# vaenyr/stable-diffusion-on-device

Measured on AMD Instinct MI355X. Metric: images/sec + per-UNet-step ms, SD v1.4 512x512 20-step PLMS, 1/2/4/8 MI355X, higher is better.
Workload: dtype f16; 1 GPU; SD v1.4 txt2img 512x512, 20-step PLMS (21 UNet evals, batch 2 = cond+uncond per image), CLIP encode + VAE decode + uint8, guidance 7.5; images_per_gpu=1, global_batch=1, parallelism=dp1 (image shards, 1 RCCL broadcast), hip_graph=True, trajectory_graph=True, decode_overlaps_next_sampling=False

## Files before the change

include/sdod_engine.h:

```cpp
#ifndef SDOD_ENGINE_H
#define SDOD_ENGINE_H

#include <stddef.h>
#include <stdint.h>

#ifndef SDOD_API
#define SDOD_API
#endif

#ifdef __cplusplus
extern "C" {
#endif

enum sdod_graph_kind { SDOD_GRAPH_UNET = 0, SDOD_GRAPH_VAE_DECODER = 1, SDOD_GRAPH_TEXT_ENCODER = 2, SDOD_GRAPH_TEMB = 3,
                       SDOD_GRAPH_VAE_ENCODER = 4, SDOD_GRAPH_VAE_ENCODER_MASKED = 5, SDOD_GRAPH_ADAPTER = 6, SDOD_GRAPH_UPSCALER = 7,
                       SDOD_GRAPH_CONTROLNET = 8, SDOD_GRAPH_CONTROL_HINT = 9, SDOD_GRAPH_IMAGE_ENCODER = 10, SDOD_GRAPH_IMAGE_PROJ = 11 };

typedef struct sdod_model_config {
    int latent_channels;
    int latent_h;
    int latent_w;
    int model_channels;
    int context_dim;
    int context_len;
    int num_heads;
    int head_dim;
    int vocab_size;
    int text_layers;
    int text_heads;
    int vae_channels;
    int linear_proj;
    int text_arch;
    int weight_quant;
    int concat_channels;
} sdod_model_config;

SDOD_API void sdod_model_config_sd14(sdod_model_config* cfg);
SDOD_API void sdod_model_config_sd21(sdod_model_config* cfg);

SDOD_API int sdod_graph_create(void** graph, int kind, const sdod_model_config* cfg, int batch);
typedef struct sdod_adapter_config {
    int adapter_reps;
    int adapter_hint_channels;
    int adapter_res_blocks;
} sdod_adapter_config;
SDOD_API int sdod_graph_create_ex(void** graph, int kind, const sdod_model_config* cfg, const sdod_adapter_config* adapter, int batch);
SDOD_API int sdod_graph_create_wrap(void** graph, int kind, const sdod_model_config* cfg, const sdod_adapter_config* adapter, int wrap,
                                    int batch);
typedef struct sdod_upscaler_config {
    int num_blocks;
    int in_h;
    int in_w;
} sdod_upscaler_config;
SDOD_API int sdod_graph_create_upscaler(void** graph, const sdod_upscaler_config* cfg, int batch);
typedef struct sdod_control_config {
    int control_inputs;
    int control_temb;
} sdod_control_config;
SDOD_API int sdod_graph_create_control(void** graph, int kind, const sdod_model_config* cfg, const sdod_control_config* control, int batch);
typedef struct sdod_region_config {
    int regions;
} sdod_region_config;
SDOD_API int sdod_graph_create_regions(void** graph, int kind, const sdod_model_config* cfg, const sdod_region_config* regions, int batch);
typedef struct sdod_ip_config {
    int ip_tokens;
} sdod_ip_config;
SDOD_API int sdod_graph_create_ip(void** graph, int kind, const sdod_model_config* cfg, const sdod_ip_config* ip, int batch);
typedef struct sdod_vision_config {
    int image_size;
    int patch;
    int width;
    int layers;
    int heads;
    int mlp_dim;
    int proj_dim;
    int quick_gelu;
} sdod_vision_config;
SDOD_API int sdod_graph_create_vision(void** graph, int kind, const sdod_model_config* cfg, const sdod_vision_config* vision, const sdod_ip_config* ip,
                                      int batch);
SDOD_API int sdod_graph_bind_output(void* graph, int index, void* device_ptr, size_t bytes);
SDOD_API int sdod_graph_destroy(void* graph);

SDOD_API int sdod_graph_num_params(void* graph);
SDOD_API int sdod_graph_param_info(void* graph, int index, const char** name, int* ndim, int64_t shape[4]);
SDOD_API int sdod_graph_set_param(void* graph, const char* name, const void* data, int dtype, const int64_t* shape, int ndim);
SDOD_API int sdod_graph_param_device(void* graph, const char* name, void** device_ptr, size_t* bytes);
SDOD_API int sdod_graph_load_file(void* graph, const char* path, const char* prefix);
SDOD_API int sdod_graph_finalize(void* graph);
SDOD_API int sdod_graph_io(void* graph, int is_output, int index, void** device_ptr, size_t* bytes);
enum sdod_exec_flags { SDOD_EXEC_HIP_GRAPH = 1, SDOD_EXEC_STATIC_UNCHANGED = 2 };
SDOD_API int sdod_graph_execute(void* graph, void* stream, int flags);
SDOD_API int sdod_graph_check(void* graph);
SDOD_API int sdod_graph_num_ops(void* graph);
SDOD_API int sdod_graph_op_info(void* graph, int index, const char** label, double* flops, double* bytes);
SDOD_API int sdod_graph_op_detail(void* graph, int index, const char** detail);
SDOD_API int sdod_graph_profile(void* graph, void* stream, int iters, float* ms_out, int n);
SDOD_API int sdod_graph_stats(void* graph, size_t* weight_bytes, size_t* arena_bytes, int* num_launches, double* flops);
SDOD_API int sdod_graph_tune_info(void* graph, int* from_table, int* tuned_in_process, char* table_path, int cap);

SDOD_API int sdod_graph_keep_base(void* graph);
SDOD_API int sdod_graph_base_bytes(void* graph, size_t* bytes);
typedef struct {
    const char* name;
    const void* up;
    const void* down;
    int dtype;
    int rank;
    float scale;
} sdod_lora_entry;
SDOD_API int sdod_graph_set_loras(void* graph, const sdod_lora_entry* entries, int count, void* stream);

SDOD_API int sdod_graph_enable_freeu(void* graph);
SDOD_API int sdod_graph_freeu_input(void* graph, int* index);

#ifdef __cplusplus
}
#endif
#endif
```

include/sdod_hip.h:

```cpp
#ifndef SDOD_HIP_H
#define SDOD_HIP_H

#include <stddef.h>
#include <stdint.h>

#ifndef SDOD_API
#define SDOD_API
#endif

#ifdef __cplusplus
extern "C" {
#endif

enum sdod_act { SDOD_ACT_NONE = 0, SDOD_ACT_SILU = 1, SDOD_ACT_GELU = 2, SDOD_ACT_QUICK_GELU = 3, SDOD_ACT_RELU = 4 };
enum sdod_dtype { SDOD_F16 = 0, SDOD_F32 = 1, SDOD_U8Q = 2, SDOD_BF16 = 3  };
enum sdod_a_mode { SDOD_A_ROWS = 0, SDOD_A_CONV3X3 = 1  };

typedef struct sdod_gemm_desc {
    const void* a;
    const void* a2;
    const void* w;
    const void* bias;
    const void* row_bias;
    const void* residual;
// ... 19 lines not shown
    const void* t0;
    const void* t1;
    int tc0, tc1;
    const void* bias2;
    int ln;
    const void* ln_s;
    float ln_eps;
    int phase;
    int wq;
    const void* w_scale;
    const void* w_off;
    void* fix_counters;
    int xcd_panels;
    int w_img_stride;
    int vec_img_stride;
    int softmax_cols;
    int pad_mode;
} sdod_gemm_desc;

SDOD_API int sdod_gemm_f16(const sdod_gemm_desc* d, void* stream);
SDOD_API int sdod_gemm_region_f16(const sdod_gemm_desc* d, const void* region_w, int regions, void* stream);
SDOD_API int sdod_gemm_fixup(const sdod_gemm_desc* d);
SDOD_API size_t sdod_gemm_fixup_counters(void);
SDOD_API size_t sdod_gemm_workspace_bytes(const sdod_gemm_desc* d);
SDOD_API int sdod_gemm_plan(const sdod_gemm_desc* d, int* tile, int* splits);
SDOD_API int sdod_gemm_halo_ok(const sdod_gemm_desc* d, int tile);
SDOD_API int sdod_gemm_panel_ok(const sdod_gemm_desc* d, int tile);
SDOD_API int sdod_gemm_xcd_panels(const sdod_gemm_desc* d);
SDOD_API int sdod_gemm_num_tiles(void);
SDOD_API int sdod_gemm_tile_shape(int tile, int* bm, int* bn, int* lds_dma);
SDOD_API int sdod_gemm_tile_info(int tile, int out[7]);
SDOD_API int sdod_gemm_time(const sdod_gemm_desc* d, void* stream, int iters, float* ms_avg);
SDOD_API int sdod_gemm_time_cold(const sdod_gemm_desc* d, void* stream, int iters, void* scratch, size_t scratch_bytes, float* ms_avg,
                                float* ms_min );

SDOD_API size_t sdod_group_norm_workspace_bytes(int n, int groups);
SDOD_API int sdod_group_norm_layout(int n, int groups, size_t* sync_off, size_t* partial_off, size_t* stats_off, size_t* shift_off,
                                    size_t* end_off);
SDOD_API int sdod_group_norm_status(void);
SDOD_API int sdod_group_norm_clear_error(void);
SDOD_API int sdod_group_norm_launches(int hw, int c, int groups, int dtype);
SDOD_API int sdod_group_norm_path(int n, int hw, int c0, int c1, int groups, int dtype);
SDOD_API int sdod_group_norm_nhwc(const void* x, const void* x2, void* y, const float* weight, const float* bias,
                                  int n, int hw, int c0, int c1, int groups, float eps, int silu, int dtype,
                                  void* workspace, void* stream);

SDOD_API size_t sdod_group_norm_nchw_workspace_bytes(int n, int groups);
SDOD_API int sdod_group_norm_nchw(const void* x, void* y, const float* weight, const float* bias, int n, int c, long long spatial,
                                  int groups, float eps, int silu, int dtype, void* workspace, void* stream);

typedef struct sdod_gn_reduce {
    const void* partial;
    int splits;
    size_t slab_floats;
    const void* bias;
    const void* bias2;
    const void* row_bias;
    int ld_row_bias;
    const void* residual;
    int ldr;
    void* x_out;
    float alpha;
    int act;
    int M, N;
} sdod_gn_reduce;
SDOD_API int sdod_gemm_reduce_info(const sdod_gemm_desc* d, sdod_gn_reduce* out);
SDOD_API int sdod_group_norm_reduce_ok(int hw, int c0, int c1, int groups);
SDOD_API int sdod_group_norm_reduce_nhwc(const sdod_gn_reduce* red, const void* x2, void* y, const float* weight,
                                         const float* bias, int n, int hw, int c0, int c1, int groups, float eps, int silu,
                                         void* stream);

SDOD_API int sdod_ln_fold_f16(void* w, int n, int k, int ldw, const float* gamma, const float* beta, const float* bias_in,
                              float* s_out, float* t_out, void* stream);
SDOD_API int sdod_compose_linear_f16(const void* p, int ldp, const void* w, int ldw, void* c, int ldc, int n_out, int n_mid, int k,
                                     const float* bias_w, const float* bias_p, float* bias_out, void* stream);
SDOD_API int sdod_lora_merge_f16(void* w, int n, int k, int ldw, const void* up, const void* down, int rank, float scale,
                                 int conv_cin, int geglu, void* stream);
SDOD_API int sdod_layer_norm_f16(const void* x, void* y, const float* weight, const float* bias, int m, int c,
                                 float eps, void* stream);

SDOD_API int sdod_attention_f16(const void* q, const void* k, const void* v, void* out, int batch, int heads,
                                int lq, int lk, int d, int ldq, int ldk, int ldv, int ldo, float scale, int causal,
                                void* stream);
SDOD_API int sdod_attention_head_dim_ok(int d);

SDOD_API int sdod_xattn_fold_f16(const void* kv, int ld_kv, int k_off, int v_off, int n_img, int L, const void* wq, int ldq,
                                 const void* sq, const void* tq, const void* wo, int ldwo, int heads, int d, float scale, void* w1,
                                 void* s1, void* t1, void* w2, void* stream);
SDOD_API int sdod_xattn_fold_ok(int heads, int d, int l_keys, int rows_per_image);

SDOD_API int sdod_xattn_fold_regions_f16(const void* kv, int ld_kv, int k_off, int v_off, int n_img, int regions, int L, const void* wq,
                                         int ldq, const void* sq, const void* tq, const void* wo, int ldwo, int heads, int d, float scale,
                                         void* w1, void* s1, void* t1, void* w2, void* stream);

SDOD_API int sdod_xattn_fold_ip_f16(const void* kv, int ld_kv, int k_off, int v_off, const void* kv_ip, int ld_ip, int k_off_ip, int v_off_ip,
                                    int n_img, int L, int T, const void* wq, int ldq, const void* sq, const void* tq, const void* wo, int ldwo,
                                    int heads, int d, float scale, void* w1, void* s1, void* t1, void* w2, void* stream);

SDOD_API int sdod_softmax_rows_f16(const void* x, void* y, int m, int n, void* stream);

SDOD_API int sdod_geglu_f16(const void* x, void* y, int m, int c, void* stream);
SDOD_API int sdod_act_f16(const void* x, void* y, size_t n, int act, void* stream);
SDOD_API int sdod_add_f16(const void* a, const void* b, void* y, size_t n, void* stream);
SDOD_API int sdod_region_weights_f32(const uint8_t* masks, int regions, int h, int w, float* w1, float* w2, float* w4, float* w8, void* stream);
SDOD_API int sdod_region_blend_f16(const void* a, size_t region_stride, const float* w, void* out, int rows, int rows_per_img, int c, int regions,
                                   void* stream);
SDOD_API int sdod_ip_weights_f32(const uint8_t* mask, float scale, int h, int w, float* w1, float* w2, float* w4, float* w8, void* stream);
SDOD_API int sdod_patch_embed_u8_f16(const uint8_t* img, void* out, int n, int image_size, int patch, int kpad, const float* mean3, const float* std3,
                                     void* stream);
SDOD_API int sdod_vit_tokens_f16(const void* patches, const void* class_embedding, const void* position_embedding, const float* ln_weight,
                                 const float* ln_bias, void* out, int n, int num_patches, int width, float eps, void* stream);
SDOD_API int sdod_concat_channels_f16(const void* a, const void* b, void* y, size_t rows, int c0, int c1, void* stream);
SDOD_API int sdod_pixel_unshuffle_u8_f16(const uint8_t* img, void* y, int n, int h, int w, int ch, int factor, void* stream);
SDOD_API int sdod_avg_pool2_f16(const void* x, void* y, int n, int h, int w, int c, void* stream);
SDOD_API int sdod_adapter_stage_f16(const void* src, void* dst, size_t count, float weight, void* stream);
SDOD_API int sdod_add_feature_f16(void* h, const void* f, size_t per_copy, int reps, void* stream);
#define SDOD_CONTROL_MAX_SEGS 16
typedef struct sdod_control_seg {
    void* h;
    const void* r;
    size_t count;
} sdod_control_seg;
SDOD_API int sdod_add_control_f16(const sdod_control_seg* segs, int count, const float* scales, void* stream);
#define SDOD_FREEU_PARAMS 8
SDOD_API int sdod_freeu_f16(void* h, void* skip, int n, int height, int width, int c, const float* params, int stage, float* scratch,
                            int phases, void* stream);
SDOD_API int sdod_im2col3x3_small_f16(const void* x, void* y, int n_img, int h, int w, int c, int kpad, void* stream);
SDOD_API int sdod_im2col3x3_small_wrap_f16(const void* x, void* y, int n_img, int h, int w, int c, int kpad, int wrap, void* stream);
SDOD_API int sdod_latent_im2col_f16(const float* x, void* y, int n_img, int h, int w, int c, int kpad, float scale, void* stream);

SDOD_API int sdod_conv_in_f16(const float* x, const void* w, const float* bias, void* y, int n_img, int h, int wd, int c, int cout,
                              float scale, void* stream);
SDOD_API int sdod_conv_in_wrap_f16(const float* x, const void* w, const float* bias, void* y, int n_img, int h, int wd, int c, int cout,
                                   float scale, int wrap, void* stream);
SDOD_API int sdod_image_conv_in_f16(const uint8_t* img, const void* w, const float* bias, void* y, int n_img, int h, int wd, int cout,
                                    void* stream);
SDOD_API int sdod_conv_in_cat_f16(const float* x, const float* cond, const void* w, const float* bias, void* y, int n_img, int h, int wd,
                                  int c, int c_cond, int cout, void* stream);
SDOD_API int sdod_masked_image_conv_in_f16(const uint8_t* img, const uint8_t* mask, const void* w, const float* bias, void* y, int n_img,
                                           int h, int wd, int cout, void* stream);
SDOD_API int sdod_image_conv_in_unit_f16(const uint8_t* img, const void* w, const float* bias, void* y, void* y2, int ld2, int n_img, int h,
                                         int wd, int cout, void* stream);

typedef struct sdod_dense_conv_desc {
    const void* in;
    const void* w;
    const float* bias;
    void* out;
    const void* res1;
    const void* res2;
    int ld_in, ld_out, ld_res1, ld_res2;
    int out_col;
    int cin, cout;
    int n, h, w_in;
    int upsample;
    float alpha, slope, c1;
} sdod_dense_conv_desc;
SDOD_API int sdod_dense_conv3x3_f16(const sdod_dense_conv_desc* d, void* stream);
SDOD_API int sdod_dense_conv3x3_ok(const sdod_dense_conv_desc* d);

SDOD_API int sdod_inpaint_cond_f32(const float* moments, const uint8_t* mask_u8, const float* n1, float* cond, int n, int c, int h_lat,
                                   int w_lat, int factor, int reps, uint64_t seed, uint64_t image_index0, void* stream);
SDOD_API int sdod_encode_latent_f32(const float* moments, const float* n1, const float* n2, float* x, float* z0, int n, int c, int hw,
                                    float sqrt_at, float sqrt_one_minus_at, uint64_t seed, uint64_t image_index0, void* stream);
SDOD_API int sdod_latent_resize_f32(const float* src, float* dst, int n, int c, int h_in, int w_in, int h_out, int w_out, int mode, float a,
                                    float b, const float* noise, uint64_t seed, uint64_t image_index0, void* stream);
// ... 110 lines not shown
```

stable-diffusion-on-device_amd/csrc/attention.hip:

```cpp
#include "common.h"
#include "sdod_hip.h"
#include "host_util.h"

#include <climits>
#include <cmath>
#include <cstdlib>
#include <type_traits>

namespace {

struct AttnP {
    const f16* q;
    const f16* k;
    const f16* v;
    f16* out;
    int B, H, Lq, Lk;
    int ldq, ldk, ldv, ldo;
    float scale_log2;
    int causal;
};

typedef short short4v __attribute__((__vector_size__(4 * sizeof(short))));
typedef __attribute__((address_space(3))) short4v* lds_short4_ptr;

constexpr int odd16(int dv) {
    int s = (dv + 15) / 16;
    if ((s & 1) == 0) s += 1;
    return s * 16;
}

template <int D, int QT>
constexpr int attn_min_waves() { return (D == 40 || (D == 80 && QT == 1)) ? 3 : 1; }

template <int N, int I = 0, class F>
SDOD_DEVICE void static_for(F&& f) {
    if constexpr (I < N) {
        f(std::integral_constant<int, I>{});
        static_for<N, I + 1>(f);
    }
}

template <int D, int QT, bool TR, int KVS = 1>
__global__ __launch_bounds__(256 * KVS, (attn_min_waves<D, QT>())) void attn_kernel(const AttnP p) {
    constexpr int DP = ((D + 31) / 32) * 32;
    constexpr int KSTEPS = DP / 32;
    constexpr int DV = ((D + 15) / 16) * 16;
    constexpr int NDT = DV / 16;
    constexpr int KSTR = DP + 8;
    constexpr int VSTR = odd16(DV);
    constexpr int KT = 64;
    constexpr int DC = D / 8;
    constexpr int LD_IT = (KT * DC + 255) / 256;
    constexpr int STAGE = KT * (KSTR + VSTR);
    constexpr bool SUM_BY_MFMA = DV > D;
    constexpr bool DEFER = DP > D;
    constexpr int KS_M = D / 32, G_M = (D % 32) / 8;
    constexpr float THR = 8.0f;
    static_assert(D % 8 == 0, "head dim must be a multiple of 8");

    extern __shared__ __attribute__((aligned(16))) char smem_raw[];
    const int grp = KVS > 1 ? (int)(threadIdx.x >> 8) : 0;
    f16* smem = reinterpret_cast<f16*>(smem_raw) + (size_t)grp * 2 * STAGE;

    const int tid = threadIdx.x & 255;
    const int lane = tid & 63;
    const int wave = tid >> 6;
    const int g = lane >> 4;
    const int li = lane & 15;
    const int nqb = (p.Lq + 64 * QT - 1) / (64 * QT);
    const int lid = xcd_remap(blockIdx.x, nqb * p.H * p.B);
    const int bh = lid / nqb;
    const int b = bh / p.H, h = bh - b * p.H;
    const int q_block = (lid - bh * nqb) * (64 * QT);

    const f16* kbase = p.k + (size_t)b * p.Lk * p.ldk + h * D;
    const f16* vbase = p.v + (size_t)b * p.Lk * p.ldv + h * D;

    {
        constexpr int KPADC = (DP - D) / 8, VPADC = (DV - D) / 8;
        for (int st = 0; st < 2; ++st) {
            f16* sK = smem + st * STAGE;
            f16* sV = sK + KT * KSTR;
            if (KPADC > 0)
                for (int idx = tid; idx < KT * KPADC; idx += 256) {
                    const int row = idx / (KPADC > 0 ? KPADC : 1), ch = idx - row * KPADC;
                    f16x8 pad = zero8();
                    if (DEFER && ch == 0) pad[0] = (f16)-1.0f;
                    *reinterpret_cast<f16x8*>(sK + row * KSTR + D + ch * 8) = pad;
                }
            if (VPADC > 0)
                for (int idx = tid; idx < KT * VPADC; idx += 256) {
                    const int row = idx / (VPADC > 0 ? VPADC : 1), ch = idx - row * VPADC;
                    f16x8 pad = zero8();
                    if (ch == 0) pad[0] = (f16)1.0f;
                    *reinterpret_cast<f16x8*>(sV + row * VSTR + D + ch * 8) = pad;
                }
        }
    }

    f16x8 qf[QT][KSTEPS];
    int qrow[QT];
#pragma unroll
// ... 236 lines not shown
    };

    if (grp < NT) {
        load_tile(grp);
        store_tile(0);
    }
    __syncthreads();
    const int NTG = (NT + KVS - 1) / KVS;
    int thr = INT_MIN;
    for (int it = 0; it < NTG; ++it) {
        const int t = it * KVS + grp;
        const int cur = it & 1;
        const bool has_next = t + KVS < NT;
        const f16* sK = smem + cur * STAGE;
        const f16* sV = sK + KT * KSTR;
        if (t >= NT) {
            __syncthreads();
            continue;
        }
        f16x8 kf[HOLD ? KSTEPS : 1][4];
        f16x8 vfr[HOLD ? 2 : 1][HOLD ? NDT : 1];
        read_k(sK, kf);
        read_v(sV, vfr);
        f32x4 s[QT][4];
        qk(sK, kf, s);
        if (has_next && !(abl & 1)) load_tile(t + KVS);
        static_for<QT>([&](auto a_c) { softmax_pv(a_c, t, thr, s[decltype(a_c)::value], vfr, sV); });
        thr = __builtin_bit_cast(int, THR);
        asm volatile("" : "+s"(thr));
        if (has_next) store_tile(cur ^ 1);
        __syncthreads();
    }

    if constexpr (KVS > 1) {
        static_assert(KVS == 2, "the merge below handles two groups");
        float* mrg = reinterpret_cast<float*>(smem_raw);
        constexpr int NV = QT * (2 + NDT * 4);
        static_assert((size_t)NV * 256 * sizeof(float) <= (size_t)KVS * 2 * STAGE * sizeof(f16), "merge buffer fits the staging LDS");
        if (grp == 1) {
#pragma unroll
            for (int a = 0; a < QT; ++a) {
                mrg[(a * (2 + NDT * 4) + 0) * 256 + tid] = m_run[a];
                mrg[(a * (2 + NDT * 4) + 1) * 256 + tid] = l_run[a];
#pragma unroll
                for (int dt = 0; dt < NDT; ++dt)
#pragma unroll
                    for (int r = 0; r < 4; ++r) mrg[(a * (2 + NDT * 4) + 2 + dt * 4 + r) * 256 + tid] = o[a][dt][r];
            }
        }
        __syncthreads();
        if (grp == 1) return;
#pragma unroll
        for (int a = 0; a < QT; ++a) {
            const float m1 = mrg[(a * (2 + NDT * 4) + 0) * 256 + tid], l1 = mrg[(a * (2 + NDT * 4) + 1) * 256 + tid];
            const float m = fmaxf(m_run[a], m1);
            const float a0 = __builtin_amdgcn_exp2f(m_run[a] - m), a1 = __builtin_amdgcn_exp2f(m1 - m);
            l_run[a] = l_run[a] * a0 + l1 * a1;
#pragma unroll
            for (int dt = 0; dt < NDT; ++dt)
#pragma unroll
                for (int r = 0; r < 4; ++r) o[a][dt][r] = o[a][dt][r] * a0 + mrg[(a * (2 + NDT * 4) + 2 + dt * 4 + r) * 256 + tid] * a1;
            m_run[a] = m;
        }
    }
#pragma unroll
    for (int a = 0; a < QT; ++a) {
        float l;
        if (SUM_BY_MFMA) {
            l = __shfl(o[a][D / 16][D % 4], ((D % 16) / 4) * 16 + li);
        } else {
            l = quad_rows_sum(l_run[a]);
        }
        const float inv = l > 0.f ? 1.0f / l : 0.f;
        if (qrow[a] < p.Lq) {
            f16* op = p.out + ((size_t)b * p.Lq + qrow[a]) * p.ldo + h * D;
#pragma unroll
            for (int dt = 0; dt < NDT; ++dt) {
                const int dv0 = dt * 16 + g * 4;
                if (dv0 < D) {
                    f16x4 hv;
#pragma unroll
                    for (int r = 0; r < 4; ++r) hv[r] = (f16)(o[a][dt][r] * inv);
                    *reinterpret_cast<f16x4*>(op + dv0) = hv;
                }
            }
        }
    }
}

template <int D, int QT, bool TR, int KVS = 1>
hipError_t attn_launch(const AttnP& p, hipStream_t st) {
    constexpr int DP = ((D + 31) / 32) * 32;
    constexpr int DV = ((D + 15) / 16) * 16;
    constexpr size_t smem = (size_t)KVS * 2 * 64 * (DP + 8 + odd16(DV)) * sizeof(f16);
    static_assert(smem <= 160 * 1024, "LDS");
    static std::atomic<unsigned long long> attr_devs{0};
    if (sdod::first_use_on_device(attr_devs)) {
        hipError_t e = hipFuncSetAttribute(reinterpret_cast<const void*>(&attn_kernel<D, QT, TR, KVS>),
                                           hipFuncAttributeMaxDynamicSharedMemorySize, (int)smem);
        if (e != hipSuccess) return e;
    }
    dim3 grid(((p.Lq + 64 * QT - 1) / (64 * QT)) * p.H * p.B);
    SDOD_LAUNCH((attn_kernel<D, QT, TR, KVS>), grid, dim3(256 * KVS), smem, st, p);
    return hipGetLastError();
}

template <int D>
hipError_t attn_dispatch(const AttnP& p, bool big, bool tr, hipStream_t st) {
    if (tr) return big ? attn_launch<D, 2, true>(p, st) : attn_launch<D, 1, true>(p, st);
    return big ? attn_launch<D, 2, false>(p, st) : attn_launch<D, 1, false>(p, st);
}

struct FoldP {
    const f16* kv; int ld_kv, k_off, v_off, L, n_img;
    const f16* wq; int ldq;
    const float* sq; const float* tq;
    const f16* wo; int ldwo;
    int heads, d, C;
    float alpha;
    f16* w1; float* s1; float* t1; f16* w2;
    int tiles_c;
    int n_w;
    int regions;
    const f16* kv2; int ld_kv2, k_off2, v_off2, L2;
};
constexpr int kFoldKMax = 160;
struct FoldSeg { const f16* k; const f16* v; int ld, L; };
template <bool TWO_SRC>
__device__ __forceinline__ FoldSeg fold_segment(const FoldP& p, int seg) {
    if constexpr (!TWO_SRC) {
        const f16* base = p.kv + (long long)seg * p.L * p.ld_kv;
        return FoldSeg{base + p.k_off, base + p.v_off, p.ld_kv, p.L};
    }
    const int b = seg >> 1;
    if (seg & 1) {
        const f16* base = p.kv2 + (long long)b * p.L2 * p.ld_kv2;
        return FoldSeg{base + p.k_off2, base + p.v_off2, p.ld_kv2, p.L2};
    }
    const f16* base = p.kv + (long long)b * p.L * p.ld_kv;
    return FoldSeg{base + p.k_off, base + p.v_off, p.ld_kv, p.L};
}
template <bool TWO_SRC>
__global__ __launch_bounds__(256) void xattn_fold_kernel(const FoldP p) {
    __shared__ __attribute__((aligned(16))) f16 sa[80][kFoldKMax + 8], sb[80][kFoldKMax + 8];
    const int tid = threadIdx.x, lane = tid & 63, wave = tid >> 6;
    const int NK = p.heads * 80, d = p.d;
    int item = blockIdx.x;
    if (item >= 2 * p.n_w) {
        const int idx = (item - 2 * p.n_w) * 256 + tid;
        if (idx >= p.n_img * NK) return;
        const int j = idx % 80, bh = idx / 80, h = bh % p.heads, img = bh / p.heads;
        const FoldSeg sg = fold_segment<TWO_SRC>(p, img);
        if (j >= sg.L) {
            p.s1[idx] = 0.f;
            p.t1[idx] = -30000.f;
            return;
        }
        const f16* kr = sg.k + (long long)j * sg.ld + h * d;
        float a = 0.f, b = 0.f;
        for (int dd = 0; dd < d; ++dd) {
            const float kval = (float)kr[dd];
            a = fmaf(kval, p.sq[h * d + dd], a);
            b = fmaf(kval, p.tq[h * d + dd], b);
        }
        p.s1[idx] = p.alpha * a;
        p.t1[idx] = p.alpha * b;
        return;
    }
    const bool second = item >= p.n_w;
    if (second) item -= p.n_w;
    const int tc = item % p.tiles_c, bh = item / p.tiles_c, h = bh % p.heads, img = bh / p.heads;
    const int KP = (d + 31) & ~31, kc = KP / 8;
    const FoldSeg sg = fold_segment<TWO_SRC>(p, img);
    auto stage_rows = [&](f16 (*dst)[kFoldKMax + 8], const f16* base, long long row_stride, int valid_rows) {
        for (int idx = tid; idx < 80 * kc; idx += 256) {
            const int r = idx / kc, ch = idx - r * kc;
            const f16x8 v = (r < valid_rows && ch * 8 < d) ? ldg8(base + (long long)r * row_stride + ch * 8) : zero8();
            *reinterpret_cast<f16x8*>(&dst[r][ch * 8]) = v;
        }
    };
    if (!second) {
        stage_rows(sa, sg.k + h * d, sg.ld, sg.L);
        for (int idx = tid; idx < KP * 10; idx += 256) {
            const int k = idx / 10, ch = idx - k * 10;
            const f16x8 v = k < d ? ldg8(p.wq + (long long)(h * d + k) * p.ldq + tc * 80 + ch * 8) : zero8();
#pragma unroll
            for (int e = 0; e < 8; ++e) sb[ch * 8 + e][k] = v[e];
        }
    } else {
        stage_rows(sa, p.wo + (long long)(tc * 80) * p.ldwo + h * d, p.ldwo, 80);
        stage_rows(sb, sg.v + h * d, sg.ld, sg.L);
    }
    __syncthreads();
    const int fr = lane & 15, fg = lane >> 4;
    for (int rb = wave; rb < 5; rb += 4) {
        f32x4 acc[5];
#pragma unroll
        for (int j = 0; j < 5; ++j) acc[j] = f32x4{0.f, 0.f, 0.f, 0.f};
        for (int ks = 0; ks < KP / 32; ++ks) {
            const f16x8 fa = *reinterpret_cast<const f16x8*>(&sa[rb * 16 + fr][ks * 32 + fg * 8]);
#pragma unroll
            for (int j = 0; j < 5; ++j) {
                const f16x8 fb = *reinterpret_cast<const f16x8*>(&sb[j * 16 + fr][ks * 32 + fg * 8]);
                acc[j] = mfma16(fb, fa, acc[j]);
            }
        }
        const int m = rb * 16 + fr;
        const int wimg = img / p.regions, reg = img - wimg * p.regions;
        f16* row = second ? p.w2 + ((long long)wimg * p.C + tc * 80 + m) * ((long long)p.regions * NK) + reg * NK + h * 80
                          : p.w1 + ((long long)(img * p.heads + h) * 80 + m) * p.C + tc * 80;
        const float al = second ? 1.0f : p.alpha;
#pragma unroll
        for (int j = 0; j < 5; ++j) {
            f16x4 o;
#pragma unroll
            for (int r = 0; r < 4; ++r) o[r] = (f16)(al * acc[j][r]);
            *reinterpret_cast<f16x4*>(row + j * 16 + fg * 4) = o;
        }
    }
}

}

extern "C" int sdod_attention_head_dim_ok(int d) { return d == 40 || d == 64 || d == 80 || d == 160 ? 1 : 0; }

extern "C" int sdod_xattn_fold_ok(int heads, int d, int l_keys, int rows_per_image) {
    if (heads <= 0 || d <= 0 || d > kFoldKMax || d % 8 != 0 || l_keys <= 0 || l_keys > 80) return 0;
    const long long C = (long long)heads * d, NK = (long long)heads * 80;
    if (C % 80 != 0) return 0;
    if (rows_per_image == 0) return 1;
    return rows_per_image > 0 && rows_per_image % 32 == 0 && NK % 320 == 0 && C % 64 == 0 ? 1 : 0;
}

extern "C" int sdod_attention_f16(const void* q, const void* k, const void* v, void* out, int batch, int heads, int lq,
                                  int lk, int d, int ldq, int ldk, int ldv, int ldo, float scale, int causal,
                                  void* stream) {
    SDOD_TRY
    SDOD_REQUIRE(q && k && v && out, "null pointer");
    SDOD_REQUIRE(batch > 0 && heads > 0 && lq > 0 && lk > 0, "bad shape");
    SDOD_REQUIRE(sdod_attention_head_dim_ok(d), "head dim must be one of 40, 64, 80, 160");
    SDOD_REQUIRE(ldq % 8 == 0 && ldk % 8 == 0 && ldv % 8 == 0 && ldo % 4 == 0, "row strides must keep 16-byte alignment");
    SDOD_REQUIRE(ldq >= heads * d && ldk >= heads * d && ldv >= heads * d && ldo >= heads * d, "row stride < heads*d");
    SDOD_REQUIRE((((uintptr_t)q | (uintptr_t)k | (uintptr_t)v) & 15) == 0 && ((uintptr_t)out & 7) == 0, "misaligned pointer");
    SDOD_REQUIRE(std::isfinite(scale) && scale > 0.f, "scale must be finite and > 0");
    AttnP p{};
    p.q = (const f16*)q; p.k = (const f16*)k; p.v = (const f16*)v; p.out = (f16*)out;
    p.B = batch; p.H = heads; p.Lq = lq; p.Lk = lk;
    p.ldq = ldq; p.ldk = ldk; p.ldv = ldv; p.ldo = ldo;
    p.scale_log2 = scale * 1.4426950408889634f;
    p.causal = causal;
    const bool no_tr = std::getenv("SDOD_ATTN_NO_TR") != nullptr;
    const bool tr = !no_tr;
    bool big = lq >= 2048 && d != 160;
    if (const char* e = std::getenv("SDOD_ATTN_QT")) big = e[0] == '2' && d != 160;
    hipStream_t st = (hipStream_t)stream;
    hipError_t e;
    switch (d) {
    case 40: e = attn_dispatch<40>(p, big, tr, st); break;
    case 64: e = attn_dispatch<64>(p, big, tr, st); break;
    case 80: {
        static const bool kvs_off = [] { const char* e2 = std::getenv("SDOD_ATTN_KVS"); return e2 && e2[0] == '0'; }();
        const long long wgs = (long long)((lq + 63) / 64) * heads * batch;
        if (!big && tr && !kvs_off && !causal && wgs <= 512 && lk >= 256) e = attn_launch<80, 1, true, 2>(p, st);
        else e = attn_dispatch<80>(p, big, tr, st);
        break;
    }
    default: e = attn_dispatch<160>(p, false, tr, st); break;
    }
    SDOD_HIP_CHECK(e);
    return 0;
    SDOD_CATCH
}

namespace {
struct FoldSrc2 { const void* kv; int ld, k_off, v_off, L; };
int xattn_fold_launch(const void* kv, int ld_kv, int k_off, int v_off, int n_img, int regions, int L, const void* wq, int ldq, const void* sq,
                      const void* tq, const void* wo, int ldwo, int heads, int d, float scale, void* w1, void* s1, void* t1, void* w2,
                      void* stream, const FoldSrc2& ip = FoldSrc2{nullptr, 0, 0, 0, 0}) {
    SDOD_TRY
    SDOD_REQUIRE(regions >= 1 && regions <= 4, "regions must be in [1, 4]");
    if (ip.kv) {
        SDOD_REQUIRE(regions == 2, "two sources are two segments per image");
        SDOD_REQUIRE(ip.L >= 1 && ip.L <= 16, "image tokens must be in [1, 16]");
        SDOD_REQUIRE(ip.ld % 8 == 0 && ip.k_off % 8 == 0 && ip.v_off % 8 == 0 && ip.k_off >= 0 && ip.v_off >= 0 && ((uintptr_t)ip.kv & 15) == 0,
                     "operands must keep 16-byte alignment");
        SDOD_REQUIRE(heads > 0 && d > 0 && (long long)ip.k_off + (long long)heads * d <= ip.ld && (long long)ip.v_off + (long long)heads * d <= ip.ld,
                     "image K / V offsets + heads * d must fit the image row stride");
    }
    SDOD_REQUIRE(n_img <= (1 << 20), "bad shape (too many images)");
    n_img *= regions;
    SDOD_REQUIRE(kv && wq && sq && tq && wo && w1 && s1 && t1 && w2, "null pointer");
    SDOD_REQUIRE(n_img > 0 && sdod_xattn_fold_ok(heads, d, L, 0), "bad shape (d <= 160, d % 8 == 0, L <= 80, heads * d a multiple of 80)");
    SDOD_REQUIRE((long long)heads * d <= (1 << 24), "bad shape (heads * d too large)");
    const int C = heads * d, NK = heads * 80;
    SDOD_REQUIRE(ldq >= C && ldwo >= C && ld_kv >= C, "row strides >= heads * d");
    SDOD_REQUIRE(ld_kv % 8 == 0 && k_off % 8 == 0 && v_off % 8 == 0 && ldq % 8 == 0 && ldwo % 8 == 0 &&
                     (((uintptr_t)kv | (uintptr_t)wq | (uintptr_t)wo | (uintptr_t)w1 | (uintptr_t)w2) & 15) == 0,
                 "operands must keep 16-byte alignment");
    FoldP p{};
    p.kv = (const f16*)kv; p.ld_kv = ld_kv; p.k_off = k_off; p.v_off = v_off; p.L = L; p.n_img = n_img;
    p.wq = (const f16*)wq; p.ldq = ldq; p.sq = (const float*)sq; p.tq = (const float*)tq;
    p.wo = (const f16*)wo; p.ldwo = ldwo;
    p.heads = heads; p.d = d; p.C = C;
    p.alpha = scale * 1.4426950408889634f;
    p.w1 = (f16*)w1; p.s1 = (float*)s1; p.t1 = (float*)t1; p.w2 = (f16*)w2;
    p.tiles_c = C / 80;
    p.n_w = n_img * heads * p.tiles_c;
    p.regions = regions;
    p.kv2 = (const f16*)ip.kv; p.ld_kv2 = ip.ld; p.k_off2 = ip.k_off; p.v_off2 = ip.v_off; p.L2 = ip.L;
    const int blocks = 2 * p.n_w + (n_img * NK + 255) / 256;
    if (ip.kv) SDOD_LAUNCH(xattn_fold_kernel<true>, dim3(blocks), dim3(256), 0, (hipStream_t)stream, p);
    else SDOD_LAUNCH(xattn_fold_kernel<false>, dim3(blocks), dim3(256), 0, (hipStream_t)stream, p);
    SDOD_HIP_CHECK(hipGetLastError());
    return 0;
    SDOD_CATCH
}
}

extern "C" int sdod_xattn_fold_f16(const void* kv, int ld_kv, int k_off, int v_off, int n_img, int L, const void* wq, int ldq,
                                   const void* sq, const void* tq, const void* wo, int ldwo, int heads, int d, float scale, void* w1,
                                   void* s1, void* t1, void* w2, void* stream) {
    return xattn_fold_launch(kv, ld_kv, k_off, v_off, n_img, 1, L, wq, ldq, sq, tq, wo, ldwo, heads, d, scale, w1, s1, t1, w2, stream);
}

extern "C" int sdod_xattn_fold_regions_f16(const void* kv, int ld_kv, int k_off, int v_off, int n_img, int regions, int L, const void* wq,
                                           int ldq, const void* sq, const void* tq, const void* wo, int ldwo, int heads, int d, float scale,
                                           void* w1, void* s1, void* t1, void* w2, void* stream) {
    return xattn_fold_launch(kv, ld_kv, k_off, v_off, n_img, regions, L, wq, ldq, sq, tq, wo, ldwo, heads, d, scale, w1, s1, t1, w2, stream);
}

extern "C" int sdod_xattn_fold_ip_f16(const void* kv, int ld_kv, int k_off, int v_off, const void* kv_ip, int ld_ip, int k_off_ip, int v_off_ip,
                                      int n_img, int L, int T, const void* wq, int ldq, const void* sq, const void* tq, const void* wo, int ldwo,
                                      int heads, int d, float scale, void* w1, void* s1, void* t1, void* w2, void* stream) {
    SDOD_TRY
    SDOD_REQUIRE(kv_ip, "null pointer");
    SDOD_CATCH
    return xattn_fold_launch(kv, ld_kv, k_off, v_off, n_img, 2, L, wq, ldq, sq, tq, wo, ldwo, heads, d, scale, w1, s1, t1, w2, stream,
                             FoldSrc2{kv_ip, ld_ip, k_off_ip, v_off_ip, T});
}
```

stable-diffusion-on-device_amd/csrc/engine.h:

```cpp
#pragma once
#include <hip/hip_runtime.h>

#include <cstdint>
#include <functional>
#include <map>
#include <string>
#include <unordered_map>
#include <vector>

#include "host_util.h"
#include "sdod_engine.h"
#include "sdod_hip.h"

namespace sdod {

typedef _Float16 f16;

inline void check_rc(int rc) {
    if (rc != 0) throw Error(rc, get_last_error());
}

enum ParamKind {
    PK_CONV3,
    PK_CONV3_SMALL,
    PK_CONV1,
    PK_LINEAR,
    PK_EMBED,
    PK_VEC,
    PK_MAT_F32,
    PK_LINEAR_GEGLU,
    PK_VEC_GEGLU,
};

inline int small_k(int64_t cin) { return 9 * cin <= 64 ? 64 : 128; }

struct Param {
    std::string name;
    std::vector<int64_t> shape;
    ParamKind kind;
    int group = -1;
    int ld = 0;
    int col_off = 0;
    int owner = -1;
    size_t dev_bytes = 0;
    char* dev = nullptr;
    bool set = false;
    bool quant = false;
    size_t qrow = 0;
};

struct Act {
    f16* p = nullptr;
    int n = 0, h = 0, w = 0, c = 0;
    int rows() const { return n * h * w; }
    size_t numel() const { return (size_t)rows() * c; }
};

struct IoSlot {
    void* ptr = nullptr;
    size_t bytes = 0;
    bool owned = true;
};

class Graph {
public:
    Graph(int kind, const sdod_model_config& cfg, int batch, const sdod_adapter_config& acfg = sdod_adapter_config{0, 0, 0}, int wrap = 0,
          const sdod_upscaler_config& ucfg = sdod_upscaler_config{0, 0, 0}, const sdod_control_config* ccfg = nullptr, int regions = 0,
          int ip_tokens = 0, const sdod_vision_config* vcfg = nullptr);
    ~Graph();
    Graph(const Graph&) = delete;

    int num_params() const { return (int)params_.size(); }
    const Param& param(int i) const { return params_.at(i); }
    void set_param(const std::string& name, const void* data, int dtype, const int64_t* shape, int ndim);
    void load_file(const std::string& path, const std::string& prefix);
    void finalize();
    void keep_base();
    size_t base_bytes() const { return base_copy_ ? weight_bytes_ : 0; }
    void set_loras(const sdod_lora_entry* entries, int count, hipStream_t st);
    void enable_freeu();
    int freeu_input() const { return freeu_ ? freeu_input_ : -1; }
    void execute(hipStream_t st, bool use_hip_graph, bool skip_static = false);
    void check_health() const;
    IoSlot io(bool output, int index) const;
    void bind_output(int index, void* ptr, size_t bytes);
    void stats(size_t* wbytes, size_t* abytes, int* launches, double* flops) const;

private:
    enum Mode { DECLARE, DRY, REAL };
    int kind_;
    sdod_model_config cfg_;
    sdod_adapter_config acfg_;
    sdod_upscaler_config ucfg_;
    sdod_control_config ccfg_{0, 0};
    int regions_ = 0;
    const float* region_w_[4] = {};
    sdod_vision_config vcfg_{0, 0, 0, 0, 0, 0, 0, 0};
    int ip_tokens_ = 0;
    const float* ip_w_[4] = {};
    f16* ip_kv_all_ = nullptr;
    bool freeu_ = false;
    int freeu_input_ = -1;
    void freeu_site(const Act& h, const Act& skip, const float* params, int stage);
    bool has_kv() const { return kind_ == SDOD_GRAPH_UNET || kind_ == SDOD_GRAPH_CONTROLNET; }
    int batch_;
    int wrap_ = 0;
    Mode mode_ = DECLARE;
    bool finalized_ = false;

    std::vector<Param> params_;
    std::unordered_map<std::string, int> pindex_;
    std::vector<std::vector<int>> groups_;
    std::unordered_map<std::string, int> gindex_;
    char* weight_base_ = nullptr;
    size_t weight_bytes_ = 0;
    float* qscale_ = nullptr;
    float* qoff_ = nullptr;
    size_t qrows_ = 0;
    bool quant_mode() const { return cfg_.weight_quant != 0 && (kind_ == SDOD_GRAPH_UNET || kind_ == SDOD_GRAPH_TEMB); }
    static constexpr int kQuantAutoMaxRows = 128;
    bool quant_decl_ = false;
    void quant_rows(int rows) { quant_decl_ = quant_mode() && (cfg_.weight_quant == 1 || rows <= kQuantAutoMaxRows); }
    void quant_global() { quant_decl_ = quant_mode(); }
    const float* qscale_of(int w) const { return params_[w].quant ? qscale_ + params_[w].qrow : nullptr; }
    const float* qoff_of(int w) const { return params_[w].quant ? qoff_ + params_[w].qrow : nullptr; }
    int P(const std::string& name, std::vector<int64_t> shape, ParamKind kind, const std::string& group = "");
    int Pc(const std::string& name, std::vector<int64_t> shape, ParamKind kind, int ld, int col_off, int owner);
    template <typename T>
    const T* W(int idx) const { return reinterpret_cast<const T*>(params_[idx].dev); }
    void allocate_weights();

    char* arena_base_ = nullptr;
    size_t arena_cap_ = 0, arena_high_ = 0;
    std::map<size_t, size_t> free_;
    std::map<size_t, size_t> used_;
    void arena_reset();
    f16* alloc(size_t halves);
    void release(const void* p);
    Act act(int n, int h, int w, int c);
    void release(const Act& a) { release(a.p); }

    char* ws_ = nullptr;
    size_t ws_bytes_ = 0, ws_need_ = 0;
    char* gn_ws_ = nullptr;
    size_t gn_ws_bytes_ = 0, gn_ws_need_ = 0;

    std::vector<IoSlot> inputs_, outputs_;
    void* io_alloc(std::vector<IoSlot>& v, size_t bytes);
    std::vector<size_t> out_bytes_;
    std::map<int, void*> bound_out_;

    struct Op {
        std::function<void(hipStream_t)> fn;
        std::string label;
        double flops = 0;
        double bytes = 0;
        std::string detail;
        const void* pf_ptr = nullptr;
        size_t pf_bytes = 0;
    };
    std::vector<Op> ops_;
    std::vector<Op> static_ops_;
    bool to_static_ = false;
    double flops_ = 0;
    hipGraphExec_t graph_exec_ = nullptr;
    hipGraph_t hip_graph_ = nullptr;
    hipStream_t capture_stream_ = nullptr;
    unsigned* fix_counters_ = nullptr;
    hipStream_t side_stream_ = nullptr;
    std::vector<hipEvent_t> pf_events_;
    void run_ops(hipStream_t st);
    int eager_runs_ = 0;
    int tune_hits_ = 0, tune_misses_ = 0;

    void build();
    void build_unet();
    void build_vae();
    void build_vae_encoder(bool masked);
    void build_clip();
    Act clip_block(const std::string& pfx, bool oc, Act x, int heads, int inter, bool causal, int mlp_act);
    void build_image_encoder();
    void build_image_proj();
    void build_temb();
    void build_adapter();
    void build_upscaler();
    void build_controlnet();
    void build_control_hint();

    struct GemmOpt {
        int bias = -1;
        const float* bias_raw = nullptr;
        f16* out = nullptr;
        const f16* row_bias = nullptr;
        int ld_row_bias = 0, rows_per_img = 0;
        const f16* residual = nullptr;
        int act = 0;
        float alpha = 1.0f;
        bool bias_on_m = false;
        int lda = 0, ldo = 0;
        int ldr = 0;
        bool geglu = false;
        const Act* tail0 = nullptr;
        const Act* tail1 = nullptr;
        int bias2 = -1;
        int ln_w = -1, ln_b = -1;
        const float* wq_scale = nullptr;
        const float* wq_off = nullptr;
        const float* ln_s_raw = nullptr;
        int w_img_stride = 0, vec_img_stride = 0;
        int softmax_cols = 0;
        const float* region_w = nullptr;
        int regions = 0;
        int pad_mode = 0;
        int split_k = 0;
    };
    struct LnVecs { float* s; float* t; };
    LnVecs ln_fold_vectors(f16* w, int N, int K, int ldw, int ln_w, int ln_b, const float* bias);
    struct FoldJob {
        f16* w; int n, k, ldw;
        const float *gamma, *beta, *bias_in;
        float *s, *t;
    };
    std::vector<FoldJob> fold_jobs_;
    struct ComposeJob {
        f16* c; const f16* p; int ld, n_out, n_mid, k;
        const float *bias_w, *bias_p;
        float* bias_out;
    };
    std::vector<ComposeJob> compose_jobs_;
    void run_folds(hipStream_t st);
    bool keep_base_ = false;
    char* base_copy_ = nullptr;
    bool static_stale_ = false;
    std::vector<void*> derived_;
    void emit_gemm(sdod_gemm_desc d, const float* region_w = nullptr, int regions = 0);
    void linear(const f16* x, int rows, int K, int w, int N, f16* out, const GemmOpt& o);
    void linear_raw(const f16* x, int rows, int K, const f16* w, int ldw, int N, f16* out, const GemmOpt& o);
    Act conv(const Act& x, const Act* x2, int w, int cout, int ksize, int stride, bool upsample, const GemmOpt& o);
    Act group_norm(const Act& x, const Act* x2, int gw, int gb, float eps, bool silu);
    Act layer_norm(const Act& x, int lw, int lb, float eps);
    void dense_conv(sdod_dense_conv_desc d, int w, int bias);
    void attention(const f16* q, const f16* k, const f16* v, f16* out, int B, int heads, int lq, int lk, int d, int ldq,
                   int ldk, int ldv, int ldo, bool causal);

    Act res_block(const std::string& pfx, const Act& x, const Act* x2, int cout, const f16* emb_all, int emb_ld, int& emb_off);
    std::vector<Op>& sink() { return to_static_ ? static_ops_ : ops_; }
    struct PendingReduce {
        bool active = false;
        sdod_gemm_desc d{};
        double bytes = 0;
        std::string detail;
    } pending_;
    void flush_pending();
    std::vector<const void*> parked_;
    void release_after_consumer(const Act& a) { parked_.push_back(a.p); }
    void drain_parked() {
        for (const void* p : parked_) release(p);
        parked_.clear();
    }
    void settle() {
        flush_pending();
        drain_parked();
    }
    struct HeadGeom { int heads, d; };
    HeadGeom head_geometry(int C) const;
    void check_head_geometry() const;
    Act spatial_transformer(const std::string& pfx, const Act& x, const Act& ctx);
    Act unet_conv_in(const float* x_in, const float* cond_in);
    Act unet_encoder(Act h, const Act& ctx, const f16* emb_all, int emb_ld, int& emb_off, const f16* const* feat_in, std::vector<Act>* hs,
                     const std::function<void(int, const Act&)>& on_skip);
    size_t control_residual_numel(int k) const;
    void kv_all_gemm(const f16* ctx_in);
    void ip_kv_all_gemm(const f16* ip_ctx_in);
    std::vector<std::pair<std::string, int>> temb_blocks() const;
    Act vae_res_block(const std::string& pfx, const Act& x, int cout);
    Act vae_attn_block(const std::string& pfx, const Act& x);
    void vae_res_step(const std::string& pfx, Act& h, int cout);
    void vae_mid(const std::string& pfx, Act& h, int ch);
    int emb_total_ = 0;
    int kv_total_ = 0;
    f16* kv_all_ = nullptr;
    int kv_off_ = 0;
    std::vector<std::pair<std::string, int>> unet_res_blocks() const;
    const char* group_base(const std::string& group) const;
    int group_first(const std::string& group) const;
    void emit(std::function<void(hipStream_t)> fn, std::string label = "elementwise", double flops = 0, double bytes = 0, std::string detail = "") {
        settle();
        if (mode_ != REAL) return;
        flops_ += flops;
        sink().push_back(Op{std::move(fn), std::move(label), flops, bytes, std::move(detail)});
    }

public:
    int tune_hits() const { return tune_hits_; }
    int tune_misses() const { return tune_misses_; }
    int num_ops() const { return (int)ops_.size(); }
    const Op& op(int i) const { return ops_.at(i); }
    void profile(hipStream_t st, int iters, float* ms, int n);
};

}
```

stable-diffusion-on-device_amd/csrc/engine.hip:

```cpp
#include "engine.h"

#include <cstdio>

#include <dlfcn.h>
#include <fcntl.h>
#include <sys/mman.h>
#include <sys/stat.h>
#include <unistd.h>

#include <algorithm>
#include <cstdlib>
#include <cstring>
#include <map>
#include <mutex>
#include <thread>

namespace sdod {

static inline size_t align_up(size_t v, size_t a) { return (v + a - 1) / a * a; }

template <typename F>
static void parallel_for(int64_t n, F&& fn) {
    int nt = (int)std::min<int64_t>(n, std::max(1u, std::min(16u, std::thread::hardware_concurrency())));
    if (nt <= 1) {
        fn(0, n);
        return;
    }
    std::vector<std::thread> th;
    const int64_t per = (n + nt - 1) / nt;
    for (int t = 0; t < nt; ++t) {
        const int64_t b = t * per, e = std::min(n, b + per);
        if (b < e) th.emplace_back([=, &fn]() { fn(b, e); });
    }
    for (auto& t : th) t.join();
}

Graph::Graph(int kind, const sdod_model_config& cfg, int batch, const sdod_adapter_config& acfg, int wrap, const sdod_upscaler_config& ucfg,
             const sdod_control_config* ccfg, int regions, int ip_tokens, const sdod_vision_config* vcfg)
    : kind_(kind), cfg_(cfg), acfg_(acfg), ucfg_(ucfg), regions_(regions), ip_tokens_(ip_tokens), batch_(batch), wrap_(wrap) {
    SDOD_REQUIRE(ip_tokens == 0 || ((kind == SDOD_GRAPH_UNET || kind == SDOD_GRAPH_IMAGE_PROJ) && ip_tokens >= 1 && ip_tokens <= 16 && regions == 0),
                 "ip_tokens: the UNET and IMAGE_PROJ graphs only, 1 .. 16, not with regions");
    const bool vision_kind = kind == SDOD_GRAPH_IMAGE_ENCODER || kind == SDOD_GRAPH_IMAGE_PROJ;
    SDOD_REQUIRE(vision_kind == (vcfg != nullptr), "the IMAGE_ENCODER and IMAGE_PROJ graphs, and only they, are created by sdod_graph_create_vision");
    if (vcfg) {
        vcfg_ = *vcfg;
        cfg_.weight_quant = 0;
        SDOD_REQUIRE(vcfg_.proj_dim >= 64 && vcfg_.proj_dim <= 4096 && vcfg_.proj_dim % 64 == 0, "proj_dim must be a multiple of 64 in [64, 4096]");
        if (kind == SDOD_GRAPH_IMAGE_ENCODER) {
            SDOD_REQUIRE(vcfg_.patch >= 1 && vcfg_.patch <= 64 && vcfg_.image_size >= vcfg_.patch && vcfg_.image_size <= 1024 && vcfg_.image_size % vcfg_.patch == 0,
                         "image_size must be a multiple of patch (patch <= 64, image_size <= 1024)");
            SDOD_REQUIRE(vcfg_.width >= 64 && vcfg_.width <= 3072 && vcfg_.width % 64 == 0 && vcfg_.mlp_dim >= 64 && vcfg_.mlp_dim % 64 == 0 && vcfg_.mlp_dim <= 16384,
                         "width and mlp_dim must be multiples of 64 (width <= 3072, mlp_dim <= 16384)");
            SDOD_REQUIRE(vcfg_.layers >= 1 && vcfg_.layers <= 64 && vcfg_.heads >= 1 && vcfg_.width % vcfg_.heads == 0 &&
                             (vcfg_.width / vcfg_.heads == 64 || vcfg_.width / vcfg_.heads == 80),
                         "layers in [1, 64]; the head dim width / heads must be 64 or 80");
            SDOD_REQUIRE(vcfg_.quick_gelu == 0 || vcfg_.quick_gelu == 1, "quick_gelu must be 0 or 1");
        } else {
            SDOD_REQUIRE(ip_tokens >= 1, "the IMAGE_PROJ graph needs ip_tokens");
        }
    }
    SDOD_REQUIRE(regions == 0 || (kind == SDOD_GRAPH_UNET && regions >= 2 && regions <= 4), "regions: the UNET graph only, 2 .. 4");
    SDOD_REQUIRE(kind >= SDOD_GRAPH_UNET && kind <= SDOD_GRAPH_IMAGE_PROJ, "unknown graph kind");
    const bool control_kind = kind == SDOD_GRAPH_CONTROLNET || kind == SDOD_GRAPH_CONTROL_HINT;
    SDOD_REQUIRE(!control_kind || ccfg, "the CONTROLNET and CONTROL_HINT graphs are created by sdod_graph_create_control");
    if (ccfg) {
        ccfg_ = *ccfg;
        SDOD_REQUIRE((ccfg_.control_inputs == 0 || ccfg_.control_inputs == 1) && (ccfg_.control_temb == 0 || ccfg_.control_temb == 1),
                     "control_inputs and control_temb must be 0 or 1");
        SDOD_REQUIRE(ccfg_.control_inputs == 0 || kind == SDOD_GRAPH_UNET, "control_inputs applies to the UNET graph only");
        SDOD_REQUIRE(ccfg_.control_temb == 0 || kind == SDOD_GRAPH_TEMB, "control_temb applies to the TEMB graph only");
        if (control_kind || ccfg_.control_temb) {
            SDOD_REQUIRE(cfg.concat_channels == 0 && cfg.weight_quant == 0, "a control graph takes no concat_channels and no weight_quant");
            SDOD_REQUIRE(kind != SDOD_GRAPH_CONTROLNET || batch % 2 == 0, "the CONTROLNET graph needs an even batch (the two guidance halves)");
        }
    }
    if (kind == SDOD_GRAPH_UPSCALER) {
        SDOD_REQUIRE(ucfg.num_blocks != 0 || ucfg.in_h != 0 || ucfg.in_w != 0, "the UPSCALER graph is created by sdod_graph_create_upscaler");
        SDOD_REQUIRE(ucfg.num_blocks >= 1 && ucfg.num_blocks <= 23, "num_blocks must be in [1, 23]");
        SDOD_REQUIRE(ucfg.in_h >= 8 && ucfg.in_h <= 1024 && ucfg.in_h % 8 == 0 && ucfg.in_w >= 8 && ucfg.in_w <= 1024 && ucfg.in_w % 8 == 0,
                     "in_h and in_w must be multiples of 8 in [8, 1024]");
        cfg_.weight_quant = 0;
    } else {
        SDOD_REQUIRE(ucfg.num_blocks == 0 && ucfg.in_h == 0 && ucfg.in_w == 0, "an upscaler configuration needs kind SDOD_GRAPH_UPSCALER");
    }
    SDOD_REQUIRE(batch > 0 && batch <= 64, "batch must be in [1, 64]");
    SDOD_REQUIRE(cfg.model_channels > 0 && cfg.model_channels % 64 == 0, "model_channels must be a multiple of 64");
    SDOD_REQUIRE(cfg.context_dim % 64 == 0, "context_dim must be a multiple of 64");
    if (kind == SDOD_GRAPH_UNET || kind == SDOD_GRAPH_CONTROLNET) check_head_geometry();
    SDOD_REQUIRE(cfg.context_len >= 1 && cfg.context_len <= 4096, "context_len must be in [1, 4096]");
    SDOD_REQUIRE(cfg.concat_channels >= 0, "concat_channels must not be negative");
    SDOD_REQUIRE(acfg.adapter_reps >= 0 && acfg.adapter_reps <= 2, "adapter_reps must be 0, 1 or 2");
    SDOD_REQUIRE(wrap >= 0 && wrap <= 3, "wrap must be 0 .. 3 (bit 0 = x, bit 1 = y)");
    if (wrap != 0)
        SDOD_REQUIRE((kind == SDOD_GRAPH_UNET || kind == SDOD_GRAPH_VAE_DECODER) && cfg.concat_channels == 0,
                     "wrap applies to the UNET (without concat_channels) and VAE_DECODER graphs only");
    if (kind == SDOD_GRAPH_UNET && acfg.adapter_reps > 0)
        SDOD_REQUIRE(batch % acfg.adapter_reps == 0, "adapter_reps must divide the batch");
    if (kind == SDOD_GRAPH_ADAPTER) {
        SDOD_REQUIRE(acfg.adapter_hint_channels == 1 || acfg.adapter_hint_channels == 3, "adapter_hint_channels must be 1 or 3");
        SDOD_REQUIRE(acfg.adapter_res_blocks >= 0 && acfg.adapter_res_blocks <= 8, "adapter_res_blocks must be in [1, 8] (0 = 2)");
        cfg_.weight_quant = 0;
    }
    mode_ = DECLARE;
    arena_reset();
    build();
}

Graph::~Graph() {
    if (graph_exec_) (void)hipGraphExecDestroy(graph_exec_);
    if (capture_stream_) (void)hipStreamDestroy(capture_stream_);
    if (side_stream_) (void)hipStreamDestroy(side_stream_);
    (void)hipFree(fix_counters_);
    for (hipEvent_t e : pf_events_) (void)hipEventDestroy(e);
    if (hip_graph_) (void)hipGraphDestroy(hip_graph_);
    for (auto& s : inputs_) (void)hipFree(s.ptr);
    for (auto& s : outputs_)
        if (s.owned) (void)hipFree(s.ptr);
    (void)hipFree(weight_base_);
    (void)hipFree(base_copy_);
    (void)hipFree(qscale_);
    (void)hipFree(qoff_);
    (void)hipFree(arena_base_);
    (void)hipFree(ws_);
    (void)hipFree(gn_ws_);
    (void)hipFree(kv_all_);
    (void)hipFree(ip_kv_all_);
    for (void* d : derived_) (void)hipFree(d);
}

static size_t param_dev_bytes(const Param& p) {
    const auto& s = p.shape;
    if (p.quant) return (size_t)s[0] * s[1] * (p.kind == PK_CONV3 ? 9 : 1);
    switch (p.kind) {
    case PK_CONV3: return (size_t)s[0] * s[1] * 9 * sizeof(f16);
    case PK_CONV3_SMALL: return (size_t)s[0] * small_k(s[1]) * sizeof(f16);
    case PK_CONV1:
    case PK_LINEAR:
    case PK_LINEAR_GEGLU:
    case PK_EMBED: return (size_t)s[0] * s[1] * sizeof(f16);
    case PK_VEC:
    case PK_VEC_GEGLU: return (size_t)s[0] * sizeof(float);
    case PK_MAT_F32: {
        size_t n = 1;
        for (auto d : s) n *= (size_t)d;
        return n * sizeof(float);
    }
    }
    return 0;
}

int Graph::P(const std::string& name, std::vector<int64_t> shape, ParamKind kind, const std::string& group) {
    if (mode_ != DECLARE) {
        auto it = pindex_.find(name);
        if (it == pindex_.end()) throw Error(INTERNAL_ERROR, "parameter not declared: " + name);
        return it->second;
    }
    if (pindex_.count(name)) throw Error(INTERNAL_ERROR, "duplicate parameter: " + name);
    Param p;
    p.name = name;
    p.shape = std::move(shape);
    p.kind = kind;
    p.quant = quant_decl_ && (kind == PK_CONV3 || kind == PK_CONV1 || kind == PK_LINEAR || kind == PK_LINEAR_GEGLU);
    p.dev_bytes = param_dev_bytes(p);
    if (!group.empty()) {
        auto it = gindex_.find(group);
        if (it == gindex_.end()) {
            gindex_[group] = (int)groups_.size();
            groups_.emplace_back();
            it = gindex_.find(group);
        }
        p.group = it->second;
// ... 432 lines not shown
            for (int i = 0; i < ShapeKey::kFields; ++i) k.v[i] = (int)val[i];
            v = (int)val[ShapeKey::kFields];
        } else if (n == 13) {
            for (int i = 0; i < 12; ++i) k.v[i] = (int)val[i];
            k.v[12] = k.v[13] = 0;
            if (k.v[0] == SDOD_A_CONV3X3 && k.v[9] > 0) {
                const int ups = k.v[7] ? 1 : 0, stride = k.v[6] > 0 ? k.v[6] : 1;
                const int ho = (k.v[9] << ups) / stride;
                k.v[12] = k.v[9];
                k.v[13] = ho > 0 ? k.v[1] / (ho * ho) : 0;
            }
            v = (int)val[12];
        } else {
            continue;
        }
        const int tile = v % 1000, split = v / 1000;
        if (!(tile >= 1 && tile <= sdod_gemm_num_tiles() && split >= 1 && split <= 64)) continue;
        if (keep_existing) c.emplace(k, TuneEntry{v, true});
        else c[k] = TuneEntry{v, true};
    }
    std::fclose(f);
}
TuneCache& tune_cache() {
    static TuneCache c;
    std::lock_guard<std::mutex> lk(c.mu);
    if (!c.loaded) {
        c.loaded = true;
        const std::string shipped = shipped_tune_path();
        if (!shipped.empty()) tune_cache_read(shipped.c_str(), c.map);
        if (!shipped.empty()) tune_cache_read(control_tune_path().c_str(), c.map, true);
        if (!shipped.empty()) tune_cache_read(regions_tune_path().c_str(), c.map, true);
        if (!shipped.empty()) tune_cache_read(ip_tune_path().c_str(), c.map, true);
        if (const char* path = tune_cache_path()) tune_cache_read(path, c.map);
    }
    return c;
}
void tune_cache_append(const ShapeKey& k, int v) {
    const char* path = tune_cache_path();
    if (!path) return;
    if (FILE* f = std::fopen(path, "a")) {
        for (int i = 0; i < ShapeKey::kFields; ++i) std::fprintf(f, "%d ", k.v[i]);
        std::fprintf(f, "%d\n", v);
        std::fclose(f);
    }
}
bool autotune_enabled() {
    const char* e = std::getenv("SDOD_AUTOTUNE");
    return !(e && e[0] == '0');
}
bool autotune_cold() {
    const char* e = std::getenv("SDOD_AUTOTUNE");
    return !(e && e[0] == 'h');
}
constexpr size_t kSweepBytes = (size_t)384 << 20;
void*& tune_scratch() {
    static void* p = nullptr;
    return p;
}
ShapeKey key_of(const sdod_gemm_desc& d) {
    return ShapeKey{{d.a_mode, d.M, d.N, d.K, d.c0, d.c1, d.stride, d.upsample, d.ksize, d.h_in,
                     (d.residual ? 1 : 0) + (d.geglu ? 2 : 0) + 4 * d.tc0 + 16384 * d.tc1 + (d.ln ? (1 << 30) : 0) + (d.wq ? (1 << 29) : 0) + (d.softmax_cols ? (1 << 28) : 0) + (d.w_img_stride ? (1 << 27) : 0) +
                         (d.pad_mode == 1 ? (1 << 26) : 0) , d.lda,
                     d.a_mode == SDOD_A_CONV3X3 ? d.w_in : 0, d.a_mode == SDOD_A_CONV3X3 ? d.n_img : 0}};
}
bool pick_runs(const sdod_gemm_desc& d, int v) {
    sdod_gemm_desc c = d;
    c.tile = v % 1000;
    c.split_k = v / 1000;
    int info[7] = {0};
    if (sdod_gemm_tile_info(c.tile, info) != 0) return false;
    if (info[5] == 2) return sdod_gemm_halo_ok(&c, c.tile) != 0;
    if (info[5] == 3) return sdod_gemm_panel_ok(&c, c.tile) != 0;
    return true;
}
}

void Graph::flush_pending() {
    if (!pending_.active) return;
    pending_.active = false;
    const sdod_gemm_desc d2 = pending_.d;
    sink().push_back(Op{[d2](hipStream_t st) { check_rc(sdod_gemm_f16(&d2, st)); }, "splitk_reduce", 0.0, pending_.bytes, pending_.detail});
}

void Graph::emit_gemm(sdod_gemm_desc d, const float* region_w, int regions) {
    settle();
    if (mode_ == DECLARE) return;
    const bool tune = autotune_enabled() && (d.N > 16 || (d.a_mode == SDOD_A_CONV3X3 && d.ksize != 1 && d.N % 4 == 0));
    if (tune) {
        for (int t : kCandidates) {
            sdod_gemm_desc c = d;
            c.tile = t;
            c.split_k = 0;
            int tt = 0, sp = 1;
            (void)sdod_gemm_plan(&c, &tt, &sp);
            c.split_k = sp > 1 ? std::min(64, sp * 2) : 1;
            if (c.split_k > 1 && d.N % 4 == 0) ws_need_ = std::max(ws_need_, sdod_gemm_workspace_bytes(&c));
        }
    }
    ws_need_ = std::max(ws_need_, sdod_gemm_workspace_bytes(&d));
    if (mode_ != REAL) return;
    if (tune) {
        d.workspace = ws_;
        d.workspace_bytes = ws_bytes_;
        d.fix_counters = std::getenv("SDOD_GEMM_FIXUP") && std::getenv("SDOD_GEMM_FIXUP")[0] == '1' ? fix_counters_ : nullptr;
        const ShapeKey key = key_of(d);
        TuneCache& tc = tune_cache();
        int pick = 0;
        bool from_file = false;
        {
            std::lock_guard<std::mutex> lk(tc.mu);
            auto it = tc.map.find(key);
            if (it != tc.map.end() && pick_runs(d, it->second.v)) {
                pick = it->second.v;
                from_file = it->second.from_file;
            }
        }
        if (pick && from_file) ++tune_hits_;
        else ++tune_misses_;
        if (!pick) {
            int best = 0;
            float best_ms = 1e30f;
            const int KT = d.K / 64;
            for (int t : kCandidates) {
                sdod_gemm_desc h = d;
                h.tile = t;
                h.split_k = 0;
                int tt = 0, sp = 1;
                (void)sdod_gemm_plan(&h, &tt, &sp);
                if (tt != t) continue;
                int tried[4] = {sp, 1, sp / 2, sp > 1 ? sp * 2 : 0};
                for (int k = 0; k < 4; ++k) {
                    const int want = tried[k];
                    bool dup = want < 1 || want > 64 || (want > 1 && KT / want < 2) || (want > 1 && d.N % 4 != 0);
                    for (int j = 0; j < k && !dup; ++j) dup = tried[j] == want;
                    if (dup) continue;
                    sdod_gemm_desc c = d;
                    c.tile = t;
                    c.split_k = want;
                    if (sdod_gemm_workspace_bytes(&c) > ws_bytes_) continue;
                    float ms = 0.f;
                    if (autotune_cold()) {
                        if (!tune_scratch()) {
                            SDOD_HIP_CHECK(hipMalloc(&tune_scratch(), kSweepBytes));
                            SDOD_HIP_CHECK(hipMemset(tune_scratch(), 0, kSweepBytes));
                        }
                        float avg = 0.f;
                        if (sdod_gemm_time_cold(&c, nullptr, 4, tune_scratch(), kSweepBytes, &avg, &ms) != 0) continue;
                    } else if (sdod_gemm_time(&c, nullptr, 4, &ms) != 0) {
                        continue;
                    }
                    if (ms < best_ms) {
                        best_ms = ms;
                        best = t + 1000 * want;
                    }
                }
            }
            {
                std::lock_guard<std::mutex> lk(tc.mu);
                tc.map[key] = TuneEntry{best, false};
                tune_cache_append(key, best);
            }
            pick = best;
        }
        d.tile = pick % 1000;
        d.split_k = pick / 1000;
    }
    const double fl = 2.0 * d.M * d.N * d.K;
    flops_ += fl;
    d.workspace = ws_;
    d.workspace_bytes = ws_bytes_;
    d.fix_counters = fix_counters_;
    int tile = 0, splits = 1;
    (void)sdod_gemm_plan(&d, &tile, &splits);
    std::string label = "gemm_t" + std::to_string(tile);
    double a_bytes = d.a_mode == SDOD_A_ROWS ? (double)d.M * d.K * 2
                                             : (double)d.n_img * d.h_in * d.w_in * (d.c0 + d.c1) * 2;
    double by = a_bytes + (double)d.N * d.K * 2 + (double)d.M * d.N * 2 * (d.residual ? 2 : 1);
    std::string detail = (d.a_mode == SDOD_A_ROWS ? std::string("rows") : "conv" + std::to_string(d.ksize) + (d.upsample ? "u" : "") +
                                                                          (d.stride == 2 ? "s2" : "") + (d.c1 ? "+cat" : "")) +
                         " M" + std::to_string(d.M) + " N" + std::to_string(d.N) + " K" + std::to_string(d.K) + " x" + std::to_string(splits);
    static const bool fixup_on = [] { const char* e = std::getenv("SDOD_GEMM_FIXUP"); return e && e[0] == '1'; }();
    if (!fixup_on) d.fix_counters = nullptr;
    static const bool fuse_reduce_gn = [] { const char* e = std::getenv("SDOD_GN_REDUCE"); return e && e[0] == '1'; }();
    if (regions > 0) {
        if (splits > 1) throw Error(INTERNAL_ERROR, "a region-weighted GEMM planned split-K");
        sink().push_back(Op{[d, region_w, regions](hipStream_t st) { check_rc(sdod_gemm_region_f16(&d, region_w, regions, st)); }, label, fl, by, detail});
        return;
    }
    if (splits > 1 && !fuse_reduce_gn && sdod_gemm_fixup(&d)) {
        const double part = (double)splits * d.M * d.N * 4;
        sink().push_back(Op{[d](hipStream_t st) { check_rc(sdod_gemm_f16(&d, st)); }, label, fl, by + part, detail});
        return;
    }
    if (splits > 1) {
        sdod_gemm_desc d1 = d, d2 = d;
        d1.phase = 1;
        d2.phase = 2;
        const double part = (double)splits * d.M * d.N * 4;
        sink().push_back(Op{[d1](hipStream_t st) { check_rc(sdod_gemm_f16(&d1, st)); }, label, fl, by + part, detail});
        if ((size_t)d.N * d.ldw * (d.wq ? 1 : 2) >= kPrefetchMinBytes) {
            sink().back().pf_ptr = d.w;
            sink().back().pf_bytes = (size_t)d.N * d.ldw * (d.wq ? 1 : 2);
        }
        pending_.active = true;
        pending_.d = d2;
        pending_.bytes = part + (double)d.M * d.N * 2 * (d.residual ? 2 : 1);
        pending_.detail = detail;
        static const bool fuse_reduce = [] { const char* e = std::getenv("SDOD_GN_REDUCE"); return e && e[0] == '1'; }();
        if (to_static_ || !fuse_reduce) flush_pending();
        return;
    }
    sink().push_back(Op{[d](hipStream_t st) { check_rc(sdod_gemm_f16(&d, st)); }, label, fl, by, detail});
    if ((size_t)d.N * d.ldw * (d.wq ? 1 : 2) >= kPrefetchMinBytes) {
        sink().back().pf_ptr = d.w;
        sink().back().pf_bytes = (size_t)d.N * d.ldw * (d.wq ? 1 : 2);
    }
}

void Graph::linear_raw(const f16* x, int rows, int K, const f16* w, int ldw, int N, f16* out, const GemmOpt& o) {
    sdod_gemm_desc d{};
    d.a = x; d.w = w; d.out = out;
    d.M = rows; d.N = N; d.K = K;
    d.lda = o.lda ? o.lda : K;
    d.ldw = ldw;
    d.ldo = o.ldo ? o.ldo : N;
    d.a_mode = SDOD_A_ROWS;
    if (o.bias >= 0) d.bias = params_[o.bias].dev;
    if (o.bias_raw) d.bias = o.bias_raw;
    d.bias_on_m = o.bias_on_m ? 1 : 0;
    d.row_bias = o.row_bias; d.ld_row_bias = o.ld_row_bias; d.rows_per_img = o.rows_per_img;
    d.residual = o.residual; d.ldr = o.ldr ? o.ldr : d.ldo;
    d.act = o.act; d.alpha = o.alpha;
    if (o.geglu) {
        d.geglu = 1;
        if (!o.ldo) d.ldo = N / 2;
        d.ldr = d.ldo;
    }
    if (o.wq_scale) {
        d.wq = 1;
        d.w_scale = o.wq_scale;
        d.w_off = o.wq_off;
    }
    if (o.ln_w >= 0) {
        if (d.wq) throw Error(INTERNAL_ERROR, "LayerNorm fold with uint8 weights");
        d.ln = 1;
        d.ln_eps = 1e-5f;
        if (mode_ == REAL) {
            const LnVecs v = ln_fold_vectors(const_cast<f16*>(w), N, K, ldw, o.ln_w, o.ln_b, reinterpret_cast<const float*>(d.bias));
            d.ln_s = v.s;
            d.bias = v.t;
        } else {
            d.ln_s = d.w;
            d.bias = d.w;
        }
    }
    if (o.ln_s_raw) {
        d.ln = 1;
        d.ln_eps = 1e-5f;
        d.ln_s = o.ln_s_raw;
    }
    d.w_img_stride = o.w_img_stride; d.vec_img_stride = o.vec_img_stride; d.softmax_cols = o.softmax_cols;
    emit_gemm(d, o.region_w, o.regions);
}

Graph::LnVecs Graph::ln_fold_vectors(f16* w, int N, int K, int ldw, int ln_w, int ln_b, const float* bias) {
    float *sv = nullptr, *tv = nullptr;
    SDOD_HIP_CHECK(hipMalloc((void**)&sv, (size_t)N * sizeof(float)));
    SDOD_HIP_CHECK(hipMalloc((void**)&tv, (size_t)N * sizeof(float)));
    derived_.push_back(sv);
    derived_.push_back(tv);
    fold_jobs_.push_back(FoldJob{w, N, K, ldw, W<float>(ln_w), W<float>(ln_b), bias, sv, tv});
    return LnVecs{sv, tv};
}

void Graph::linear(const f16* x, int rows, int K, int w, int N, f16* out, const GemmOpt& o) {
    const Param& p = params_[w];
    const int ldw = p.ld > 0 ? p.ld : p.kind == PK_CONV3_SMALL ? small_k(p.shape[1]) : (int)(p.kind == PK_CONV3 ? p.shape[1] * 9 : p.shape[1]);
    if (p.quant) {
        GemmOpt oq = o;
        oq.wq_scale = qscale_of(w);
        oq.wq_off = qoff_of(w);
        linear_raw(x, rows, K, reinterpret_cast<const f16*>(p.dev), ldw, N, out, oq);
        return;
    }
    linear_raw(x, rows, K, reinterpret_cast<const f16*>(p.dev), ldw, N, out, o);
}

Act Graph::conv(const Act& x, const Act* x2, int w, int cout, int ksize, int stride, bool upsample, const GemmOpt& o) {
    const int ups = upsample ? 1 : 0;
    const int hup = x.h << ups, wup = x.w << ups;
    const int pad_mode = o.pad_mode == 0 && ksize == 3 && wrap_ != 0 ? (wrap_ == 3 ? 2 : wrap_ == 1 ? 3 : 4) : o.pad_mode;
    const int pad_sum = pad_mode == 1 ? 1 : 2 * (ksize / 2);
    const int ho = (hup + pad_sum - ksize) / stride + 1, wo = (wup + pad_sum - ksize) / stride + 1;
    Act y;
    y.n = x.n; y.h = ho; y.w = wo; y.c = cout;
    y.p = o.out ? o.out : alloc(y.numel());
    sdod_gemm_desc d{};
    d.a = x.p; d.a2 = x2 ? x2->p : nullptr;
    d.w = params_[w].dev; d.out = y.p;
    const int cin = x.c + (x2 ? x2->c : 0);
    d.M = y.rows(); d.N = cout; d.K = ksize * ksize * cin;
    if (o.tail0) {
        d.k_tail = d.K;
        d.t0 = o.tail0->p; d.tc0 = o.tail0->c;
        d.t1 = o.tail1 ? o.tail1->p : nullptr; d.tc1 = o.tail1 ? o.tail1->c : 0;
        d.K += d.tc0 + d.tc1;
        if (o.bias2 >= 0) d.bias2 = params_[o.bias2].dev;
    }
    d.ldw = params_[w].ld > 0 ? params_[w].ld : d.K; d.ldo = cout;
    d.a_mode = SDOD_A_CONV3X3;
    d.n_img = x.n; d.h_in = x.h; d.w_in = x.w; d.c0 = x.c; d.c1 = x2 ? x2->c : 0;
    d.stride = stride; d.upsample = ups; d.ksize = ksize; d.pad_mode = pad_mode;
    if (o.bias >= 0) d.bias = params_[o.bias].dev;
    else if (o.bias_raw) d.bias = o.bias_raw;
    d.row_bias = o.row_bias; d.ld_row_bias = o.ld_row_bias; d.rows_per_img = o.rows_per_img;
    d.residual = o.residual; d.ldr = cout;
    d.act = o.act; d.alpha = o.alpha;
    d.split_k = o.split_k;
    if (params_[w].quant) {
        if (o.tail0) throw Error(INTERNAL_ERROR, "tail segment with uint8 weights");
        d.wq = 1;
        d.w_scale = qscale_of(w);
        d.w_off = qoff_of(w);
    }
    emit_gemm(d);
    return y;
}

Act Graph::group_norm(const Act& x, const Act* x2, int gw, int gb, float eps, bool silu) {
    Act y = act(x.n, x.h, x.w, x.c + (x2 ? x2->c : 0));
    if (mode_ != DECLARE) gn_ws_need_ = std::max(gn_ws_need_, sdod_group_norm_workspace_bytes(x.n, 32));
    if (mode_ == REAL) {
        const void* xp = x.p; const void* x2p = x2 ? x2->p : nullptr; void* yp = y.p;
        const float* wp = W<float>(gw); const float* bp = W<float>(gb);
        const int n = x.n, hw = x.h * x.w, c0 = x.c, c1 = x2 ? x2->c : 0, si = silu ? 1 : 0;
        const std::string shape = "n" + std::to_string(n) + " hw" + std::to_string(hw) + " c" + std::to_string(c0 + c1);
        if (pending_.active && pending_.d.out == x.p && pending_.d.M == x.rows() && pending_.d.N == c0 &&
            (!pending_.d.row_bias || pending_.d.rows_per_img == hw) && sdod_group_norm_reduce_ok(hw, c0, c1, 32)) {
            sdod_gn_reduce red{};
            check_rc(sdod_gemm_reduce_info(&pending_.d, &red));
            pending_.active = false;
            ops_.push_back(Op{[=](hipStream_t st) {
                check_rc(sdod_group_norm_reduce_nhwc(&red, x2p, yp, wp, bp, n, hw, c0, c1, 32, eps, si, st));
            }, "gn_group_red", 0, pending_.bytes + 2.0 * n * hw * (c0 + c1) * 2, shape + " x" + std::to_string(red.splits)});
        } else {
            flush_pending();
            void* ws = gn_ws_;
            ops_.push_back(Op{[=](hipStream_t st) {
                check_rc(sdod_group_norm_nhwc(xp, x2p, yp, wp, bp, n, hw, c0, c1, 32, eps, si, SDOD_F16, ws, st));
            }, [&] {
                switch (sdod_group_norm_path(n, hw, c0, c1, 32, SDOD_F16)) {
                case 0: return "gn_grid";
                case 1: return "gn_group";
                case 2: return "gn_small";
                default: return "gn_stats_apply";
                }
            }(), 0, 2.0 * n * hw * (c0 + c1) * 2, shape});
        }
    }
    drain_parked();
    return y;
}

Act Graph::layer_norm(const Act& x, int lw, int lb, float eps) {
    Act y = act(x.n, x.h, x.w, x.c);
    const void* xp = x.p; void* yp = y.p;
    const float* wp = W<float>(lw); const float* bp = W<float>(lb);
    const int m = x.rows(), c = x.c;
    emit([=](hipStream_t st) { check_rc(sdod_layer_norm_f16(xp, yp, wp, bp, m, c, eps, st)); }, "layer_norm", 0, 2.0 * m * c * 2,
         "m" + std::to_string(m) + " c" + std::to_string(c));
    return y;
}

void Graph::attention(const f16* q, const f16* k, const f16* v, f16* out, int B, int heads, int lq, int lk, int d, int ldq,
                      int ldk, int ldv, int ldo, bool causal) {
    const float scale = 1.0f / sqrtf((float)d);
    const int ca = causal ? 1 : 0;
    emit([=](hipStream_t st) { check_rc(sdod_attention_f16(q, k, v, out, B, heads, lq, lk, d, ldq, ldk, ldv, ldo, scale, ca, st)); },
         "attn_d" + std::to_string(d), 4.0 * B * heads * (double)lq * lk * d, 2.0 * B * heads * d * (2.0 * lq + 2.0 * lk),
         "B" + std::to_string(B) + " h" + std::to_string(heads) + " lq" + std::to_string(lq) + " lk" + std::to_string(lk));
}

void Graph::build() {
    quant_global();
    switch (kind_) {
    case SDOD_GRAPH_UNET: build_unet(); break;
    case SDOD_GRAPH_VAE_DECODER: build_vae(); break;
    case SDOD_GRAPH_TEXT_ENCODER: build_clip(); break;
    case SDOD_GRAPH_VAE_ENCODER: build_vae_encoder(false); break;
    case SDOD_GRAPH_VAE_ENCODER_MASKED: build_vae_encoder(true); break;
    case SDOD_GRAPH_ADAPTER: build_adapter(); break;
    case SDOD_GRAPH_UPSCALER: build_upscaler(); break;
    case SDOD_GRAPH_IMAGE_ENCODER: build_image_encoder(); break;
    case SDOD_GRAPH_IMAGE_PROJ: build_image_proj(); break;
    case SDOD_GRAPH_CONTROLNET: build_controlnet(); break;
    case SDOD_GRAPH_CONTROL_HINT: build_control_hint(); break;
    default: build_temb(); break;
    }
    settle();
}

void Graph::finalize() {
    allocate_weights();
    SDOD_REQUIRE(!finalized_, "graph already finalized");
    std::string missing;
    int nmiss = 0;
    for (auto& p : params_)
        if (!p.set) {
            if (nmiss < 5) missing += (nmiss ? ", " : "") + p.name;
            ++nmiss;
        }
    SDOD_REQUIRE(nmiss == 0, std::to_string(nmiss) + " parameter(s) not set: " + missing + (nmiss > 5 ? ", ..." : ""));
    mode_ = DRY;
    arena_reset();
    ws_need_ = gn_ws_need_ = 0;
    build();
    arena_cap_ = align_up(arena_high_, 256) + 256;
    ws_bytes_ = align_up(ws_need_, 256) + 256;
    gn_ws_bytes_ = align_up(gn_ws_need_, 256) + 256;
    SDOD_HIP_CHECK(hipMalloc((void**)&arena_base_, arena_cap_));
    SDOD_HIP_CHECK(hipMalloc((void**)&ws_, ws_bytes_));
    SDOD_HIP_CHECK(hipMalloc((void**)&gn_ws_, gn_ws_bytes_));
    SDOD_HIP_CHECK(hipMemset(gn_ws_, 0, gn_ws_bytes_));
    SDOD_HIP_CHECK(hipMalloc((void**)&fix_counters_, sdod_gemm_fixup_counters() * sizeof(unsigned)));
    SDOD_HIP_CHECK(hipMemset(fix_counters_, 0, sdod_gemm_fixup_counters() * sizeof(unsigned)));
    if (has_kv() && kv_total_ > 0)
        SDOD_HIP_CHECK(hipMalloc((void**)&kv_all_, (size_t)batch_ * cfg_.context_len * kv_total_ * sizeof(f16)));
    if (ip_tokens_ > 0 && kv_total_ > 0)
        SDOD_HIP_CHECK(hipMalloc((void**)&ip_kv_all_, (size_t)batch_ * ip_tokens_ * kv_total_ * sizeof(f16)));
    mode_ = REAL;
    arena_reset();
    ops_.clear();
    static_ops_.clear();
    fold_jobs_.clear();
    compose_jobs_.clear();
    flops_ = 0;
    build();
    if (keep_base_) {
        SDOD_HIP_CHECK(hipMalloc((void**)&base_copy_, weight_bytes_));
        SDOD_HIP_CHECK(hipMemcpy(base_copy_, weight_base_, weight_bytes_, hipMemcpyDeviceToDevice));
    }
    run_folds(nullptr);
    SDOD_HIP_CHECK(hipDeviceSynchronize());
    if (tune_scratch()) {
        (void)hipFree(tune_scratch());
        tune_scratch() = nullptr;
    }
    finalized_ = true;
}

void Graph::run_folds(hipStream_t st) {
    for (const FoldJob& j : fold_jobs_)
        check_rc(sdod_ln_fold_f16(j.w, j.n, j.k, j.ldw, j.gamma, j.beta, j.bias_in, j.s, j.t, st));
    for (const ComposeJob& j : compose_jobs_) {
        f16* tmp = nullptr;
        SDOD_HIP_CHECK(hipMalloc((void**)&tmp, (size_t)j.n_mid * j.k * sizeof(f16)));
        int rc = 0;
        hipError_t e = hipMemcpy2DAsync(tmp, (size_t)j.k * sizeof(f16), j.c, (size_t)j.ld * sizeof(f16), (size_t)j.k * sizeof(f16), (size_t)j.n_mid,
                                        hipMemcpyDeviceToDevice, st);
        if (e == hipSuccess) rc = sdod_compose_linear_f16(j.p, j.ld, tmp, j.k, j.c, j.ld, j.n_out, j.n_mid, j.k, j.bias_w, j.bias_p, j.bias_out, st);
        const hipError_t e2 = hipStreamSynchronize(st);
        (void)hipFree(tmp);
        SDOD_HIP_CHECK(e);
        SDOD_HIP_CHECK(e2);
        check_rc(rc);
    }
}

void Graph::keep_base() {
    SDOD_REQUIRE(!finalized_, "keep_base() must be called before finalize()");
    keep_base_ = true;
}

void Graph::enable_freeu() {
    SDOD_REQUIRE(kind_ == SDOD_GRAPH_UNET, "FreeU applies to the UNET graph only");
    SDOD_REQUIRE(!finalized_, "enable_freeu() must be called before finalize()");
    SDOD_REQUIRE(cfg_.latent_h <= 2048 && cfg_.latent_w <= 2048, "FreeU needs latent_h and latent_w <= 2048 (sdod_freeu_f16 takes sides up to 1024)");
    freeu_ = true;
}

void Graph::set_loras(const sdod_lora_entry* entries, int count, hipStream_t st) {
    SDOD_REQUIRE(count >= 0 && (count == 0 || entries != nullptr), "bad entry list");
    SDOD_REQUIRE(finalized_, "graph not finalized");
    SDOD_REQUIRE(base_copy_ != nullptr, "the graph was finalized without keep_base(): merge on the host and rebuild it");
    SDOD_REQUIRE(cfg_.weight_quant == 0, "LoRA adapters need fp16 weights (weight_quant = 0): integer codes cannot take a delta");
    struct Merge {
        f16* w;
        int n, k, ldw, cin, geglu, rank;
        size_t up_off, down_off;
        float scale;
    };
    std::vector<Merge> merges;
    size_t halves = 0;
    for (int i = 0; i < count; ++i) {
        const sdod_lora_entry& e = entries[i];
        SDOD_REQUIRE(e.name != nullptr, "entry " + std::to_string(i) + ": null name");
        const std::string name = e.name;
        auto it = pindex_.find(name);
        SDOD_REQUIRE(it != pindex_.end(), "unknown parameter '" + name + "'");
        const Param& p = params_[it->second];
        SDOD_REQUIRE(p.kind == PK_LINEAR || p.kind == PK_CONV1 || p.kind == PK_LINEAR_GEGLU || p.kind == PK_CONV3,
                     "'" + name + "' is not a LoRA target (3x3 / 1x1 convolution, Linear or GEGLU projection weights only)");
        SDOD_REQUIRE(!p.quant, "'" + name + "' is kept as uint8 codes");
        SDOD_REQUIRE(e.dtype == SDOD_F16 || e.dtype == SDOD_F32, "'" + name + "': dtype must be SDOD_F16 or SDOD_F32");
        SDOD_REQUIRE(e.up != nullptr && e.down != nullptr, "'" + name + "': null factor");
        SDOD_REQUIRE(e.rank >= 1 && e.rank <= 128, "'" + name + "': rank must be in [1, 128]");
        Merge m{};
        m.w = reinterpret_cast<f16*>(p.dev);
        m.n = (int)p.shape[0];
        m.cin = p.kind == PK_CONV3 ? (int)p.shape[1] : 0;
        m.k = p.kind == PK_CONV3 ? 9 * (int)p.shape[1] : (int)p.shape[1];
        m.ldw = p.ld > 0 ? p.ld : m.k;
        m.geglu = p.kind == PK_LINEAR_GEGLU ? 1 : 0;
        m.rank = e.rank;
        m.scale = e.scale;
        m.up_off = halves;
        halves += align_up((size_t)m.n * m.rank, 8);
        m.down_off = halves;
        halves += align_up((size_t)m.rank * m.k, 8);
        try {
            lora_merge_require(m.w, m.n, m.k, m.ldw, e.up, e.down, m.rank, m.scale, m.cin, m.geglu);
        } catch (const Error& err) {
            throw Error(err.code, "'" + name + "': " + err.what());
        }
        merges.push_back(m);
    }
    std::vector<f16> host(halves, (f16)0.0f);
    for (int i = 0; i < count; ++i) {
        const Merge& m = merges[i];
        auto put = [&](const void* src, size_t off, size_t cnt) {
            f16* dst = host.data() + off;
            if (entries[i].dtype == SDOD_F16) std::memcpy(dst, src, cnt * sizeof(f16));
            else
                for (size_t j = 0; j < cnt; ++j) dst[j] = (f16) static_cast<const float*>(src)[j];
        };
        put(entries[i].up, m.up_off, (size_t)m.n * m.rank);
        put(entries[i].down, m.down_off, (size_t)m.rank * m.k);
    }
    struct Staging {
        f16* p = nullptr;
        ~Staging() { (void)hipFree(p); }
    } dev;
    if (halves) {
        SDOD_HIP_CHECK(hipMalloc((void**)&dev.p, halves * sizeof(f16)));
        SDOD_HIP_CHECK(hipMemcpy(dev.p, host.data(), halves * sizeof(f16), hipMemcpyHostToDevice));
    }
    SDOD_HIP_CHECK(hipMemcpyAsync(weight_base_, base_copy_, weight_bytes_, hipMemcpyDeviceToDevice, st));
    static_stale_ = true;
    for (const Merge& m : merges)
        check_rc(sdod_lora_merge_f16(m.w, m.n, m.k, m.ldw, dev.p + m.up_off, dev.p + m.down_off, m.rank, m.scale, m.cin, m.geglu, st));
    run_folds(st);
    SDOD_HIP_CHECK(hipStreamSynchronize(st));
}

namespace {
constexpr int kPrefetchLookahead = 3;
bool prefetch_enabled() {
    static const bool on = [] { const char* e = std::getenv("SDOD_PREFETCH"); return e && e[0] == '1'; }();
    return on;
// ... 140 lines not shown
    cfg->text_layers = 12;
    cfg->text_heads = 12;
    cfg->vae_channels = 128;
    cfg->linear_proj = 0;
    cfg->text_arch = 0;
    cfg->concat_channels = 0;
}

extern "C" void sdod_model_config_sd21(sdod_model_config* cfg) {
    if (!cfg) return;
    sdod_model_config_sd14(cfg);
    cfg->latent_h = cfg->latent_w = 96;
    cfg->context_dim = 1024;
    cfg->num_heads = 0;
    cfg->head_dim = 64;
    cfg->linear_proj = 1;
    cfg->text_arch = 1;
    cfg->text_layers = 23;
    cfg->text_heads = 16;
}

extern "C" int sdod_graph_create(void** graph, int kind, const sdod_model_config* cfg, int batch) {
    SDOD_TRY
    SDOD_REQUIRE(graph != nullptr && cfg != nullptr, "null argument");
    *graph = nullptr;
    *graph = new Graph(kind, *cfg, batch);
    return 0;
    SDOD_CATCH
}

extern "C" int sdod_graph_create_ex(void** graph, int kind, const sdod_model_config* cfg, const sdod_adapter_config* adapter, int batch) {
    SDOD_TRY
    SDOD_REQUIRE(graph != nullptr && cfg != nullptr, "null argument");
    *graph = nullptr;
    *graph = new Graph(kind, *cfg, batch, adapter ? *adapter : sdod_adapter_config{0, 0, 0});
    return 0;
    SDOD_CATCH
}

extern "C" int sdod_graph_create_wrap(void** graph, int kind, const sdod_model_config* cfg, const sdod_adapter_config* adapter, int wrap,
                                      int batch) {
    SDOD_TRY
    SDOD_REQUIRE(graph != nullptr && cfg != nullptr, "null argument");
    *graph = nullptr;
    *graph = new Graph(kind, *cfg, batch, adapter ? *adapter : sdod_adapter_config{0, 0, 0}, wrap);
    return 0;
    SDOD_CATCH
}

extern "C" int sdod_graph_create_upscaler(void** graph, const sdod_upscaler_config* ucfg, int batch) {
    SDOD_TRY
    SDOD_REQUIRE(graph != nullptr, "null argument");
    *graph = nullptr;
    SDOD_REQUIRE(ucfg != nullptr, "null upscaler configuration");
    sdod_model_config cfg{};
    sdod_model_config_sd14(&cfg);
    *graph = new Graph(SDOD_GRAPH_UPSCALER, cfg, batch, sdod_adapter_config{0, 0, 0}, 0, *ucfg);
    return 0;
    SDOD_CATCH
}

extern "C" int sdod_graph_create_control(void** graph, int kind, const sdod_model_config* cfg, const sdod_control_config* control, int batch) {
    SDOD_TRY
    SDOD_REQUIRE(graph && cfg, "null argument");
    SDOD_REQUIRE(kind != SDOD_GRAPH_UPSCALER && kind != SDOD_GRAPH_ADAPTER, "this kind has a create function of its own");
    const sdod_control_config none{0, 0};
    *graph = new Graph(kind, *cfg, batch, sdod_adapter_config{0, 0, 0}, 0, sdod_upscaler_config{0, 0, 0}, control ? control : &none);
    return 0;
    SDOD_CATCH
}

extern "C" int sdod_graph_create_regions(void** graph, int kind, const sdod_model_config* cfg, const sdod_region_config* regions, int batch) {
    SDOD_TRY
    SDOD_REQUIRE(graph && cfg, "null argument");
    *graph = nullptr;
    SDOD_REQUIRE(regions != nullptr && kind == SDOD_GRAPH_UNET, "regional prompts: a region configuration and kind SDOD_GRAPH_UNET");
    SDOD_REQUIRE(regions->regions >= 2 && regions->regions <= 4, "regions must be in [2, 4]");
    SDOD_REQUIRE(cfg->context_len == 77 * regions->regions, "regional prompts: context_len must be 77 * regions");
    *graph = new Graph(kind, *cfg, batch, sdod_adapter_config{0, 0, 0}, 0, sdod_upscaler_config{0, 0, 0}, nullptr, regions->regions);
    return 0;
    SDOD_CATCH
}

extern "C" int sdod_graph_create_ip(void** graph, int kind, const sdod_model_config* cfg, const sdod_ip_config* ip, int batch) {
    SDOD_TRY
    SDOD_REQUIRE(graph && cfg, "null argument");
    *graph = nullptr;
    SDOD_REQUIRE(kind != SDOD_GRAPH_UPSCALER && kind != SDOD_GRAPH_ADAPTER && kind != SDOD_GRAPH_CONTROLNET && kind != SDOD_GRAPH_CONTROL_HINT,
                 "this graph kind has a create function of its own");
    const int T = ip ? ip->ip_tokens : 0;
    if (T != 0) {
        SDOD_REQUIRE(kind == SDOD_GRAPH_UNET, "image prompts: kind SDOD_GRAPH_UNET");
        SDOD_REQUIRE(T >= 1 && T <= 16, "ip_tokens must be in [1, 16]");
        SDOD_REQUIRE(cfg->weight_quant == 0 && cfg->concat_channels == 0, "image prompts take no weight_quant and no concat_channels");
        SDOD_REQUIRE(cfg->context_len <= 80, "image prompts: context_len must be <= 80");
    }
    *graph = new Graph(kind, *cfg, batch, sdod_adapter_config{0, 0, 0}, 0, sdod_upscaler_config{0, 0, 0}, nullptr, 0, T);
    return 0;
    SDOD_CATCH
}

extern "C" int sdod_graph_create_vision(void** graph, int kind, const sdod_model_config* cfg, const sdod_vision_config* vision, const sdod_ip_config* ip,
                                        int batch) {
    SDOD_TRY
    SDOD_REQUIRE(graph, "null argument");
    *graph = nullptr;
    SDOD_REQUIRE(vision && (kind == SDOD_GRAPH_IMAGE_ENCODER || kind == SDOD_GRAPH_IMAGE_PROJ),
                 "a vision configuration and kind SDOD_GRAPH_IMAGE_ENCODER or SDOD_GRAPH_IMAGE_PROJ");
    SDOD_REQUIRE(kind == SDOD_GRAPH_IMAGE_ENCODER || (cfg && ip), "the IMAGE_PROJ graph needs the model configuration (context_dim) and ip_tokens");
    sdod_model_config base;
    sdod_model_config_sd14(&base);
    if (cfg) base = *cfg;
    *graph = new Graph(kind, base, batch, sdod_adapter_config{0, 0, 0}, 0, sdod_upscaler_config{0, 0, 0}, nullptr, 0,
                       kind == SDOD_GRAPH_IMAGE_PROJ ? ip->ip_tokens : 0, vision);
    return 0;
    SDOD_CATCH
}

extern "C" int sdod_graph_bind_output(void* graph, int index, void* device_ptr, size_t bytes) {
    SDOD_TRY
    SDOD_REQUIRE(graph, "null argument");
    static_cast<Graph*>(graph)->bind_output(index, device_ptr, bytes);
    return 0;
    SDOD_CATCH
}

extern "C" int sdod_graph_destroy(void* graph) {
    SDOD_TRY
    delete static_cast<Graph*>(graph);
    return 0;
    SDOD_CATCH
}

extern "C" int sdod_graph_num_params(void* graph) { return graph ? static_cast<Graph*>(graph)->num_params() : 0; }

extern "C" int sdod_graph_param_info(void* graph, int index, const char** name, int* ndim, int64_t shape[4]) {
    SDOD_TRY
    SDOD_REQUIRE(graph != nullptr, "null graph");
    auto* g = static_cast<Graph*>(graph);
    SDOD_REQUIRE(index >= 0 && index < g->num_params(), "parameter index out of range");
    const sdod::Param& p = g->param(index);
    if (name) *name = p.name.c_str();
    if (ndim) *ndim = (int)p.shape.size();
    if (shape)
        for (size_t i = 0; i < 4; ++i) shape[i] = i < p.shape.size() ? p.shape[i] : 1;
    return 0;
    SDOD_CATCH
}

extern "C" int sdod_graph_set_param(void* graph, const char* name, const void* data, int dtype, const int64_t* shape, int ndim) {
    SDOD_TRY
    SDOD_REQUIRE(graph && name && shape, "null argument");
    static_cast<Graph*>(graph)->set_param(name, data, dtype, shape, ndim);
    return 0;
    SDOD_CATCH
}

extern "C" int sdod_graph_load_file(void* graph, const char* path, const char* prefix) {
    SDOD_TRY
    SDOD_REQUIRE(graph && path, "null argument");
    static_cast<Graph*>(graph)->load_file(path, prefix ? prefix : "");
    return 0;
    SDOD_CATCH
}

extern "C" int sdod_graph_finalize(void* graph) {
// ... 147 lines not shown
```

stable-diffusion-on-device_amd/csrc/graphs.hip:

```cpp
#include "engine.h"

namespace sdod {

static const int kChMult[4] = {1, 2, 4, 4};

int Graph::group_first(const std::string& group) const {
    auto it = gindex_.find(group);
    if (it == gindex_.end()) throw Error(INTERNAL_ERROR, "unknown parameter group " + group);
    return groups_[it->second].front();
}

const char* Graph::group_base(const std::string& group) const {
    auto it = gindex_.find(group);
    if (it == gindex_.end()) throw Error(INTERNAL_ERROR, "unknown parameter group " + group);
    return params_[groups_[it->second].front()].dev;
}

Act Graph::res_block(const std::string& pfx, const Act& x, const Act* x2, int cout, const f16* emb_all, int emb_ld, int& emb_off) {
    const int cin = x.c + (x2 ? x2->c : 0);
    quant_rows(x.rows());
    const int n1w = P(pfx + ".in_layers.0.weight", {cin}, PK_VEC), n1b = P(pfx + ".in_layers.0.bias", {cin}, PK_VEC);
    const int c1w = P(pfx + ".in_layers.2.weight", {cout, cin, 3, 3}, PK_CONV3), c1b = P(pfx + ".in_layers.2.bias", {cout}, PK_VEC);
    const int n2w = P(pfx + ".out_layers.0.weight", {cout}, PK_VEC), n2b = P(pfx + ".out_layers.0.bias", {cout}, PK_VEC);
    int c2w, skw = -1, skb = -1;
// ... 54 lines not shown
    HeadGeom g;
    if (nh > 0) {
        SDOD_REQUIRE(C % nh == 0, "num_heads must divide the channels of every transformer" + at);
        g.heads = nh;
        g.d = C / nh;
        SDOD_REQUIRE(sdod_attention_head_dim_ok(g.d), "num_heads gives head dim " + std::to_string(g.d) + ", which no attention kernel takes (40, 64, 80, 160)" + at);
    } else {
        SDOD_REQUIRE(hd > 0, "head_dim must be positive when num_heads is 0 (one of num_heads / head_dim decides the head geometry)");
        SDOD_REQUIRE(C % hd == 0, "head_dim must divide the channels of every transformer" + at);
        SDOD_REQUIRE(sdod_attention_head_dim_ok(hd), "head_dim must be one the attention kernel takes (40, 64, 80, 160)");
        g.heads = C / hd;
        g.d = hd;
    }
    return g;
}

void Graph::check_head_geometry() const {
    for (int m : {1, 2, 4}) (void)head_geometry(m * cfg_.model_channels);
}

Act Graph::spatial_transformer(const std::string& pfx, const Act& x, const Act& ctx) {
    const int C = x.c, cd = ctx.c;
    const HeadGeom hg = head_geometry(C);
    const int heads = hg.heads, d = hg.d;
    const int rows = x.rows(), L = x.h * x.w, B = x.n;
    const std::string tb = pfx + ".transformer_blocks.0";
    quant_rows(rows);
    const bool quant_block = quant_decl_;
    const int nw = P(pfx + ".norm.weight", {C}, PK_VEC), nb = P(pfx + ".norm.bias", {C}, PK_VEC);
    const bool lin = cfg_.linear_proj != 0;
    const int piw = lin ? P(pfx + ".proj_in.weight", {C, C}, PK_LINEAR) : P(pfx + ".proj_in.weight", {C, C, 1, 1}, PK_CONV1);
    const int pib = P(pfx + ".proj_in.bias", {C}, PK_VEC);
    const int l1w = P(tb + ".norm1.weight", {C}, PK_VEC), l1b = P(tb + ".norm1.bias", {C}, PK_VEC);
    const std::string gq = tb + ".attn1.qkv";
    P(tb + ".attn1.to_q.weight", {C, C}, PK_LINEAR, gq);
    P(tb + ".attn1.to_k.weight", {C, C}, PK_LINEAR, gq);
    P(tb + ".attn1.to_v.weight", {C, C}, PK_LINEAR, gq);
    const int o1w = P(tb + ".attn1.to_out.0.weight", {C, C}, PK_LINEAR), o1b = P(tb + ".attn1.to_out.0.bias", {C}, PK_VEC);
    const int l2w = P(tb + ".norm2.weight", {C}, PK_VEC), l2b = P(tb + ".norm2.bias", {C}, PK_VEC);
    const int q2w = P(tb + ".attn2.to_q.weight", {C, C}, PK_LINEAR);
    quant_global();
    P(tb + ".attn2.to_k.weight", {C, cd}, PK_LINEAR, "attn2_kv_all");
    P(tb + ".attn2.to_v.weight", {C, cd}, PK_LINEAR, "attn2_kv_all");
    if (ip_tokens_ > 0) {
        P(tb + ".attn2.to_k_ip.weight", {C, cd}, PK_LINEAR, "attn2_kv_ip_all");
        P(tb + ".attn2.to_v_ip.weight", {C, cd}, PK_LINEAR, "attn2_kv_ip_all");
    }
    quant_decl_ = quant_block;
    const int my_kv = kv_off_;
    kv_off_ += 2 * C;
    const int o2w = P(tb + ".attn2.to_out.0.weight", {C, C}, PK_LINEAR), o2b = P(tb + ".attn2.to_out.0.bias", {C}, PK_VEC);
    const int l3w = P(tb + ".norm3.weight", {C}, PK_VEC), l3b = P(tb + ".norm3.bias", {C}, PK_VEC);
    const int f1w = P(tb + ".ff.net.0.proj.weight", {8 * C, C}, PK_LINEAR_GEGLU), f1b = P(tb + ".ff.net.0.proj.bias", {8 * C}, PK_VEC_GEGLU);
    static const bool compose_on = [] { const char* e = std::getenv("SDOD_COMPOSE"); return !(e && e[0] == '0'); }();
    const bool compose = compose_on && !quant_block;
    int f2w, pow_;
    if (compose) {
        f2w = Pc(tb + ".ff.net.2.weight", {C, 4 * C}, PK_LINEAR, 5 * C, 0, -1);
        pow_ = lin ? Pc(pfx + ".proj_out.weight", {C, C}, PK_LINEAR, 5 * C, 4 * C, f2w)
                   : Pc(pfx + ".proj_out.weight", {C, C, 1, 1}, PK_CONV1, 5 * C, 4 * C, f2w);
    } else {
        f2w = P(tb + ".ff.net.2.weight", {C, 4 * C}, PK_LINEAR);
        pow_ = lin ? P(pfx + ".proj_out.weight", {C, C}, PK_LINEAR) : P(pfx + ".proj_out.weight", {C, C, 1, 1}, PK_CONV1);
    }
    const int f2b = P(tb + ".ff.net.2.bias", {C}, PK_VEC);
    const int pob = P(pfx + ".proj_out.bias", {C}, PK_VEC);
    if (mode_ == DECLARE) return act(x.n, x.h, x.w, C);

    Act g = group_norm(x, nullptr, nw, nb, 1e-6f, false);
    Act t0 = act(B, 1, L, C);
    { GemmOpt o; o.bias = pib; linear(g.p, rows, C, piw, C, t0.p, o); }
    release(g);
    const bool fold = !quant_block;
    auto behind_ln = [&](const Act& src, int lw, int lb, GemmOpt o, auto gemm) {
        if (fold) {
            o.ln_w = lw; o.ln_b = lb;
            gemm(src.p, o);
        } else {
            Act nrm = layer_norm(src, lw, lb, 1e-5f);
            gemm(nrm.p, o);
            release(nrm);
        }
    };
    f16* qkv = alloc((size_t)rows * 3 * C);
    { GemmOpt o; o.wq_scale = qscale_of(group_first(gq)); o.wq_off = qoff_of(group_first(gq));
      behind_ln(t0, l1w, l1b, o, [&](const f16* a, const GemmOpt& og) {
          linear_raw(a, rows, C, reinterpret_cast<const f16*>(group_base(gq)), C, 3 * C, qkv, og); }); }
    f16* a1 = alloc((size_t)rows * C);
    attention(qkv, qkv + C, qkv + 2 * C, a1, B, heads, L, L, d, 3 * C, 3 * C, 3 * C, C, false);
    release(qkv);
    Act t1 = act(B, 1, L, C);
    { GemmOpt o; o.bias = o1b; o.residual = t0.p; linear(a1, rows, C, o1w, C, t1.p, o); }
    release(a1); release(t0);
    static const bool xfold_on = [] { const char* e = std::getenv("SDOD_XATTN_FOLD"); return !(e && e[0] == '0'); }();
    const int IPT = ip_tokens_;
    const int RG = IPT > 0 ? 2 : regions_, NR = RG > 0 ? RG : 1;
    const int Lkeys = IPT > 0 ? ctx.w : ctx.w / NR;
    const float* rgw = nullptr;
    if (RG > 0) {
        int lvl = 0;
        while (lvl < 4 && (cfg_.latent_h >> lvl) != x.h) ++lvl;
        if (lvl == 4 || (cfg_.latent_w >> lvl) != x.w) throw Error(INTERNAL_ERROR, "regional prompts: a transformer off the four UNet levels");
        rgw = IPT > 0 ? ip_w_[lvl] : region_w_[lvl];
    }
    const int NK = heads * 80;
    const bool xfold = xfold_on && fold && sdod_xattn_fold_ok(heads, d, Lkeys, L) != 0;
    struct { f16* a; int K; const f16* w; GemmOpt o; } xo;
    xo.o.bias = o2b; xo.o.residual = t1.p;
    if (xfold) {
        f16 *w1 = nullptr, *w2 = nullptr;
        float *s1 = nullptr, *t1v = nullptr;
        f16* wq = reinterpret_cast<f16*>(params_[q2w].dev);
        const f16* wo = reinterpret_cast<const f16*>(params_[o2w].dev);
        if (mode_ == REAL) {
            SDOD_HIP_CHECK(hipMalloc((void**)&w1, (size_t)B * NR * NK * C * sizeof(f16)));
            SDOD_HIP_CHECK(hipMalloc((void**)&w2, (size_t)B * NR * NK * C * sizeof(f16)));
            SDOD_HIP_CHECK(hipMalloc((void**)&s1, (size_t)B * NR * NK * sizeof(float)));
            SDOD_HIP_CHECK(hipMalloc((void**)&t1v, (size_t)B * NR * NK * sizeof(float)));
            derived_.push_back(w1); derived_.push_back(w2); derived_.push_back(s1); derived_.push_back(t1v);
            const LnVecs qv = ln_fold_vectors(wq, C, C, C, l2w, l2b, nullptr);
            const f16* kvp = kv_all_;
            const int ldkv = kv_total_, koff = my_kv, Lk = Lkeys, hh = heads, dd = d;
            const float scale = 1.0f / sqrtf((float)d);
            to_static_ = true;
            const f16* ipkv = ip_kv_all_;
            if (IPT > 0)
                sink().push_back(Op{[=](hipStream_t st) {
                    check_rc(sdod_xattn_fold_ip_f16(kvp, ldkv, koff, koff + C, ipkv, ldkv, koff, koff + C, B, Lk, IPT, wq, C, qv.s, qv.t, wo, C, hh, dd, scale,
                                                    w1, s1, t1v, w2, st));
                }, "xattn_fold", 4.0 * B * RG * NK * (double)C * d, 4.0 * B * RG * NK * C * 2,
                   "C" + std::to_string(C) + " d" + std::to_string(d) + " ip" + std::to_string(IPT)});
            else if (RG > 0)
                sink().push_back(Op{[=](hipStream_t st) {
                    check_rc(sdod_xattn_fold_regions_f16(kvp, ldkv, koff, koff + C, B, RG, Lk, wq, C, qv.s, qv.t, wo, C, hh, dd, scale, w1, s1, t1v, w2, st));
                }, "xattn_fold", 4.0 * B * RG * NK * (double)C * d, 4.0 * B * RG * NK * C * 2,
                   "C" + std::to_string(C) + " d" + std::to_string(d) + " regions" + std::to_string(RG)});
            else
            sink().push_back(Op{[=](hipStream_t st) {
                check_rc(sdod_xattn_fold_f16(kvp, ldkv, koff, koff + C, B, Lk, wq, C, qv.s, qv.t, wo, C, hh, dd, scale, w1, s1, t1v, w2, st));
            }, "xattn_fold", 4.0 * B * NK * (double)C * d, 4.0 * B * NK * C * 2, "C" + std::to_string(C) + " d" + std::to_string(d)});
            to_static_ = false;
        }
        const f16* w1p = mode_ == REAL ? w1 : wq;
        const f16* w2p = mode_ == REAL ? w2 : wq;
        const int NKR = NR * NK;
        f16* pb = alloc((size_t)rows * NKR);
        { GemmOpt o; o.ln_s_raw = mode_ == REAL ? s1 : reinterpret_cast<const float*>(wq); o.bias_raw = mode_ == REAL ? t1v : reinterpret_cast<const float*>(wq);
          o.w_img_stride = NKR * C; o.vec_img_stride = NKR; o.softmax_cols = 80; o.rows_per_img = L;
          o.region_w = rgw; o.regions = RG;
          linear_raw(t1.p, rows, C, w1p, C, NKR, pb, o); }
        xo.a = pb; xo.K = NKR; xo.w = w2p;
        xo.o.w_img_stride = C * NKR; xo.o.rows_per_img = L;
    } else if (RG > 0) {
        f16* q2 = alloc((size_t)rows * C);
        behind_ln(t1, l2w, l2b, GemmOpt{}, [&](const f16* a, const GemmOpt& og) { linear(a, rows, C, q2w, C, q2, og); });
        f16* ar = alloc((size_t)RG * rows * C);
        for (int b = 0; b < B; ++b)
            for (int r = 0; r < RG; ++r) {
                const bool img_seg = IPT > 0 && r == 1;
                const f16* kv = img_seg     ? ip_kv_all_ + (size_t)b * IPT * kv_total_ + my_kv
                                : IPT > 0   ? kv_all_ + (size_t)b * Lkeys * kv_total_ + my_kv
                                            : kv_all_ + (size_t)(b * RG + r) * Lkeys * kv_total_ + my_kv;
                attention(q2 + (size_t)b * L * C, kv, kv + C, ar + ((size_t)r * rows + (size_t)b * L) * C, 1, heads, L, img_seg ? IPT : Lkeys, d, C, kv_total_,
                          kv_total_, C, false);
            }
        release(q2);
        { const int rr = rows, LL = L, CC2 = C;
          emit([=](hipStream_t st) { check_rc(sdod_region_blend_f16(ar, (size_t)rr * CC2, rgw, ar, rr, LL, CC2, RG, st)); }, "region_blend", 2.0 * RG * rows * C,
               (double)(RG + 1) * rows * C * 2, "rows" + std::to_string(rows) + " C" + std::to_string(C) + " regions" + std::to_string(RG)); }
        xo.a = ar; xo.K = C; xo.w = W<f16>(o2w);
    } else {
        f16* q2 = alloc((size_t)rows * C);
// ... 882 lines not shown
```

stable-diffusion-on-device_amd/sdod/amd/_lib.py:

```python
import ctypes
import os

_HERE = os.path.dirname(os.path.abspath(__file__))
LIB_DIR = os.path.normpath(os.path.join(_HERE, '..', '..', 'lib'))

_cache = {}


def load(name):
    if name in _cache:
        return _cache[name]
    path = os.path.join(LIB_DIR, os.environ.get('SDOD_LIBSDOD', name) if name == 'libsdod.so' else name)
    if not os.path.exists(path):
        raise ImportError(
            f'{path} not found: build the MI355X extension first '
            f'(python -c "import __graft_entry__ as g; g.build()" or make -C stable-diffusion-on-device_amd). '
            f'There is no CPU fallback for the HIP path.')
    lib = ctypes.CDLL(path, mode=ctypes.RTLD_GLOBAL)
    _cache[name] = lib
    return lib


class SdodError(RuntimeError):
    def __init__(self, code, msg):
# ... 37 lines not shown
                                              'known_sa', 'known_s1a')]


class KStepArgs(ctypes.Structure):
    _fields_ = [(k, ctypes.c_void_p) for k in ('eps_nhwc', 'x', 'den_prev', 'noise', 'x_stage', 'temb_row', 'temb_dst')] + \
               [('seed', ctypes.c_uint64), ('image_index0', ctypes.c_uint64)] + \
               [(k, ctypes.c_int) for k in ('n', 'c', 'hw', 'uncond_first', 'mode', 'noise_level', 'stage_reps', 'temb_width', 'temb_reps')] + \
               [(k, ctypes.c_float) for k in ('guidance', 'd0', 'd1', 'a', 'b', 'cprev', 'u', 'stage_scale')]


PANO_MAX_AXIS = 32


class KStepWindowsArgs(ctypes.Structure):
    _fields_ = [(k, ctypes.c_void_p) for k in ('eps', 'x', 'den_prev', 'noise', 'wgt', 'wsum', 'x_stage', 'temb_row', 'temb_dst')] + \
               [('seed', ctypes.c_uint64), ('image_index0', ctypes.c_uint64)] + \
               [(k, ctypes.c_int) for k in ('c', 'H', 'W', 'wh', 'ww', 'ny', 'nx', 'wrap_x', 'n', 'chunks', 'mode', 'noise_level',
                                            'temb_width', 'temb_reps')] + \
               [('oy', ctypes.c_int * PANO_MAX_AXIS), ('ox', ctypes.c_int * PANO_MAX_AXIS)] + \
               [(k, ctypes.c_float) for k in ('guidance', 'd0', 'd1', 'a', 'b', 'cprev', 'u', 'stage_scale')]


class GemmDesc(ctypes.Structure):
    _fields_ = [
        ('a', c_void_p), ('a2', c_void_p), ('w', c_void_p), ('bias', c_void_p), ('row_bias', c_void_p),
        ('residual', c_void_p), ('out', c_void_p), ('workspace', c_void_p), ('workspace_bytes', c_size_t),
        ('M', c_int), ('N', c_int), ('K', c_int),
        ('lda', c_int), ('ldw', c_int), ('ldo', c_int), ('ldr', c_int),
        ('a_mode', c_int),
        ('n_img', c_int), ('h_in', c_int), ('w_in', c_int), ('c0', c_int), ('c1', c_int),
        ('stride', c_int), ('upsample', c_int), ('ksize', c_int), ('rows_per_img', c_int), ('ld_row_bias', c_int),
        ('act', c_int), ('alpha', c_float), ('bias_on_m', c_int), ('split_k', c_int), ('tile', c_int),
        ('geglu', c_int), ('k_tail', c_int), ('t0', c_void_p), ('t1', c_void_p), ('tc0', c_int), ('tc1', c_int),
        ('bias2', c_void_p), ('ln', c_int), ('ln_s', c_void_p), ('ln_eps', c_float), ('phase', c_int),
        ('wq', c_int), ('w_scale', c_void_p), ('w_off', c_void_p), ('fix_counters', c_void_p), ('xcd_panels', c_int),
        ('w_img_stride', c_int), ('vec_img_stride', c_int), ('softmax_cols', c_int), ('pad_mode', c_int),
    ]


class DenseConvDesc(ctypes.Structure):
    _fields_ = [(k, c_void_p) for k in ('inp', 'w', 'bias', 'out', 'res1', 'res2')] + \
               [(k, c_int) for k in ('ld_in', 'ld_out', 'ld_res1', 'ld_res2', 'out_col', 'cin', 'cout', 'n', 'h', 'w_in', 'upsample')] + \
               [(k, c_float) for k in ('alpha', 'slope', 'c1')]


class ControlSeg(ctypes.Structure):
    _fields_ = [('h', c_void_p), ('r', c_void_p), ('count', c_size_t)]


def _declare(lib):
    P = c_void_p
    sig = {
        'sdod_gemm_f16': (c_int, [ctypes.POINTER(GemmDesc), P]),
        'sdod_gemm_region_f16': (c_int, [ctypes.POINTER(GemmDesc), P, c_int, P]),
        'sdod_gemm_fixup': (c_int, [P]),
        'sdod_gemm_fixup_counters': (c_size_t, []),
        'sdod_gemm_workspace_bytes': (c_size_t, [ctypes.POINTER(GemmDesc)]),
        'sdod_gemm_plan': (c_int, [ctypes.POINTER(GemmDesc), ctypes.POINTER(c_int), ctypes.POINTER(c_int)]),
        'sdod_gemm_halo_ok': (c_int, [ctypes.POINTER(GemmDesc), c_int]),
        'sdod_gemm_panel_ok': (c_int, [ctypes.POINTER(GemmDesc), c_int]),
        'sdod_gemm_xcd_panels': (c_int, [ctypes.POINTER(GemmDesc)]),
        'sdod_gemm_time': (c_int, [ctypes.POINTER(GemmDesc), P, c_int, ctypes.POINTER(c_float)]),
        'sdod_gemm_time_cold': (c_int, [ctypes.POINTER(GemmDesc), P, c_int, P, c_size_t, ctypes.POINTER(c_float), ctypes.POINTER(c_float)]),
        'sdod_gemm_num_tiles': (c_int, []),
        'sdod_gemm_tile_info': (c_int, [c_int, ctypes.POINTER(c_int)]),
        'sdod_gemm_tile_shape': (c_int, [c_int, ctypes.POINTER(c_int), ctypes.POINTER(c_int), ctypes.POINTER(c_int)]),
        'sdod_gemm_reduce_info': (c_int, [ctypes.POINTER(GemmDesc), P]),
        'sdod_group_norm_reduce_ok': (c_int, [c_int, c_int, c_int, c_int]),
        'sdod_group_norm_reduce_nhwc': (c_int, [P, P, P, P, P, c_int, c_int, c_int, c_int, c_int, c_float, c_int, P]),
        'sdod_group_norm_launches': (c_int, [c_int, c_int, c_int, c_int]),
        'sdod_group_norm_workspace_bytes': (c_size_t, [c_int, c_int]),
        'sdod_group_norm_layout': (c_int, [c_int, c_int] + [ctypes.POINTER(c_size_t)] * 5),
        'sdod_group_norm_status': (c_int, []),
        'sdod_group_norm_clear_error': (c_int, []),
        'sdod_group_norm_path': (c_int, [c_int, c_int, c_int, c_int, c_int, c_int]),
        'sdod_group_norm_nchw_workspace_bytes': (c_size_t, [c_int, c_int]),
        'sdod_group_norm_nchw': (c_int, [P, P, P, P, c_int, c_int, ctypes.c_longlong, c_int, c_float, c_int, c_int, P, P]),
        'sdod_group_norm_nhwc': (c_int, [P, P, P, P, P, c_int, c_int, c_int, c_int, c_int, c_float, c_int, c_int, P, P]),
        'sdod_layer_norm_f16': (c_int, [P, P, P, P, c_int, c_int, c_float, P]),
        'sdod_ln_fold_f16': (c_int, [P, c_int, c_int, c_int, P, P, P, P, P, P]),
        'sdod_compose_linear_f16': (c_int, [P, c_int, P, c_int, P, c_int, c_int, c_int, c_int, P, P, P, P]),
        'sdod_lora_merge_f16': (c_int, [P, c_int, c_int, c_int, P, P, c_int, c_float, c_int, c_int, P]),
        'sdod_attention_f16': (c_int, [P, P, P, P, c_int, c_int, c_int, c_int, c_int, c_int, c_int, c_int, c_int, c_float, c_int, P]),
        'sdod_attention_head_dim_ok': (c_int, [c_int]),
        'sdod_xattn_fold_ok': (c_int, [c_int, c_int, c_int, c_int]),
        'sdod_xattn_fold_f16': (c_int, [P, c_int, c_int, c_int, c_int, c_int, P, c_int, P, P, P, c_int, c_int, c_int, c_float, P, P, P, P, P]),
        'sdod_xattn_fold_regions_f16': (c_int, [P, c_int, c_int, c_int, c_int, c_int, c_int, P, c_int, P, P, P, c_int, c_int, c_int, c_float, P, P, P, P, P]),
        'sdod_region_weights_f32': (c_int, [P, c_int, c_int, c_int, P, P, P, P, P]),
        'sdod_xattn_fold_ip_f16': (c_int, [P, c_int, c_int, c_int, P, c_int, c_int, c_int, c_int, c_int, c_int, P, c_int, P, P, P, c_int, c_int, c_int, c_float,
                                           P, P, P, P, P]),
        'sdod_ip_weights_f32': (c_int, [P, c_float, c_int, c_int, P, P, P, P, P]),
        'sdod_patch_embed_u8_f16': (c_int, [P, P, c_int, c_int, c_int, c_int, P, P, P]),
        'sdod_vit_tokens_f16': (c_int, [P, P, P, P, P, P, c_int, c_int, c_int, c_float, P]),
        'sdod_region_blend_f16': (c_int, [P, c_size_t, P, P, c_int, c_int, c_int, c_int, P]),
        'sdod_softmax_rows_f16': (c_int, [P, P, c_int, c_int, P]),
        'sdod_geglu_f16': (c_int, [P, P, c_int, c_int, P]),
        'sdod_act_f16': (c_int, [P, P, c_size_t, c_int, P]),
        'sdod_add_f16': (c_int, [P, P, P, c_size_t, P]),
        'sdod_concat_channels_f16': (c_int, [P, P, P, c_size_t, c_int, c_int, P]),
        'sdod_pixel_unshuffle_u8_f16': (c_int, [P, P, c_int, c_int, c_int, c_int, c_int, P]),
        'sdod_avg_pool2_f16': (c_int, [P, P, c_int, c_int, c_int, c_int, P]),
        'sdod_adapter_stage_f16': (c_int, [P, P, c_size_t, c_float, P]),
        'sdod_add_feature_f16': (c_int, [P, P, c_size_t, c_int, P]),
        'sdod_add_control_f16': (c_int, [ctypes.POINTER(ControlSeg), c_int, P, P]),
        'sdod_freeu_f16': (c_int, [P, P, c_int, c_int, c_int, c_int, P, c_int, P, c_int, P]),
        'sdod_im2col3x3_small_f16': (c_int, [P, P, c_int, c_int, c_int, c_int, c_int, P]),
        'sdod_im2col3x3_small_wrap_f16': (c_int, [P, P, c_int, c_int, c_int, c_int, c_int, c_int, P]),
        'sdod_latent_im2col_f16': (c_int, [P, P, c_int, c_int, c_int, c_int, c_int, c_float, P]),
        'sdod_conv_in_f16': (c_int, [P, P, P, P, c_int, c_int, c_int, c_int, c_int, c_float, P]),
        'sdod_conv_in_wrap_f16': (c_int, [P, P, P, P, c_int, c_int, c_int, c_int, c_int, c_float, c_int, P]),
        'sdod_image_conv_in_f16': (c_int, [P, P, P, P, c_int, c_int, c_int, c_int, P]),
        'sdod_image_conv_in_unit_f16': (c_int, [P, P, P, P, P, c_int, c_int, c_int, c_int, c_int, P]),
        'sdod_dense_conv3x3_f16': (c_int, [ctypes.POINTER(DenseConvDesc), P]),
        'sdod_dense_conv3x3_ok': (c_int, [ctypes.POINTER(DenseConvDesc)]),
        'sdod_conv_in_cat_f16': (c_int, [P, P, P, P, P, c_int, c_int, c_int, c_int, c_int, c_int, P]),
        'sdod_masked_image_conv_in_f16': (c_int, [P, P, P, P, P, c_int, c_int, c_int, c_int, P]),
        'sdod_inpaint_cond_f32': (c_int, [P, P, P, P, c_int, c_int, c_int, c_int, c_int, c_int, ctypes.c_uint64, ctypes.c_uint64, P]),
        'sdod_encode_latent_f32': (c_int, [P, P, P, P, P, c_int, c_int, c_int, c_float, c_float, ctypes.c_uint64, ctypes.c_uint64, P]),
        'sdod_latent_resize_f32': (c_int, [P, P, c_int, c_int, c_int, c_int, c_int, c_int, c_int, c_float, c_float, P, ctypes.c_uint64, ctypes.c_uint64, P]),
        'sdod_latent_resize_taps': (c_int, [c_int, c_int, c_int, P, P]),
        'sdod_plms_update': (c_int, [ctypes.POINTER(PlmsUpdateArgs), P]),
        'sdod_dpm_step': (c_int, [ctypes.POINTER(DpmStepArgs), P]),
        'sdod_ddim_inpaint_step': (c_int, [ctypes.POINTER(DdimInpaintStepArgs), P]),
        'sdod_k_step': (c_int, [ctypes.POINTER(KStepArgs), P]),
        'sdod_k_step_windows': (c_int, [ctypes.POINTER(KStepWindowsArgs), P]),
        'sdod_mask_to_latent_f32': (c_int, [P, P, c_int, c_int, c_int, c_int, P]),
        'sdod_image_composite_u8': (c_int, [P, P, P, P, c_int, c_size_t, c_float, c_float, c_int, P]),
        'sdod_nchw_f32_to_nhwc_f16': (c_int, [P, P, c_int, c_int, c_int, c_float, P]),
        'sdod_nhwc_f16_to_nchw_f32': (c_int, [P, P, c_int, c_int, c_int, P]),
        'sdod_latent_prep_f16': (c_int, [P, P, P, P, c_int, c_int, c_int, c_float, P]),
        'sdod_embedding_f16': (c_int, [P, P, P, P, c_int, c_int, c_int, P]),
        'sdod_context_assemble_f16': (c_int, [P, P, P, c_int, c_int, c_int, c_int, P]),
        'sdod_timestep_features_f16': (c_int, [P, P, c_int, c_int, P]),
        'sdod_stage_unet_inputs': (c_int, [P, P, c_size_t, c_int, P, P, c_size_t, c_int, P]),
        'sdod_randn_f32': (c_int, [P, P, c_size_t, ctypes.c_uint64, ctypes.c_uint64, P]),
        'sdod_cfg_combine': (c_int, [P, P, c_int, c_int, c_int, c_float, c_int, c_int, P]),
        'sdod_dpm_update': (c_int, [P, P, P, c_size_t, c_int, c_float, c_float, c_float, c_float, c_float, P]),
        'sdod_ddim_step_f32': (c_int, [P, P, c_size_t, c_float, c_float, c_float, c_float, P]),
        'sdod_lincomb4_f32': (c_int, [P, P, P, P, P, c_float, c_float, c_float, c_float, c_float, c_size_t, P]),
        'sdod_image_to_u8': (c_int, [P, P, c_size_t, c_float, c_float, c_int, P]),
        'sdod_hip_last_error': (c_char_p, []),
        'sdod_hip_device_info': (c_int, [ctypes.POINTER(c_int), ctypes.POINTER(c_size_t), c_char_p, c_int]),
    }
    for name, (res, args) in sig.items():
        fn = getattr(lib, name)
        fn.restype = res
        fn.argtypes = args


HIP_SYMBOLS = [
    'sdod_gemm_f16', 'sdod_gemm_fixup', 'sdod_gemm_fixup_counters', 'sdod_gemm_workspace_bytes', 'sdod_gemm_plan', 'sdod_gemm_halo_ok', 'sdod_gemm_panel_ok', 'sdod_gemm_xcd_panels', 'sdod_gemm_num_tiles', 'sdod_gemm_tile_shape', 'sdod_gemm_tile_info', 'sdod_gemm_time', 'sdod_gemm_time_cold', 'sdod_group_norm_workspace_bytes', 'sdod_group_norm_layout', 'sdod_group_norm_status', 'sdod_group_norm_clear_error', 'sdod_l2_prefetch', 'sdod_group_norm_launches', 'sdod_group_norm_path', 'sdod_group_norm_nhwc', 'sdod_group_norm_nchw', 'sdod_group_norm_nchw_workspace_bytes', 'sdod_gemm_reduce_info', 'sdod_group_norm_reduce_ok', 'sdod_group_norm_reduce_nhwc',
    'sdod_layer_norm_f16', 'sdod_ln_fold_f16', 'sdod_compose_linear_f16', 'sdod_lora_merge_f16', 'sdod_attention_f16', 'sdod_xattn_fold_f16', 'sdod_softmax_rows_f16', 'sdod_geglu_f16', 'sdod_act_f16',
    'sdod_add_f16', 'sdod_concat_channels_f16', 'sdod_pixel_unshuffle_u8_f16', 'sdod_avg_pool2_f16', 'sdod_adapter_stage_f16', 'sdod_add_feature_f16', 'sdod_im2col3x3_small_f16', 'sdod_im2col3x3_small_wrap_f16', 'sdod_latent_im2col_f16', 'sdod_conv_in_f16', 'sdod_conv_in_wrap_f16', 'sdod_image_conv_in_f16', 'sdod_conv_in_cat_f16', 'sdod_masked_image_conv_in_f16', 'sdod_inpaint_cond_f32', 'sdod_encode_latent_f32', 'sdod_latent_resize_f32', 'sdod_latent_resize_taps', 'sdod_plms_update', 'sdod_dpm_step', 'sdod_ddim_inpaint_step', 'sdod_k_step', 'sdod_mask_to_latent_f32', 'sdod_image_composite_u8', 'sdod_nchw_f32_to_nhwc_f16',
    'sdod_nhwc_f16_to_nchw_f32', 'sdod_latent_prep_f16', 'sdod_embedding_f16', 'sdod_context_assemble_f16', 'sdod_timestep_features_f16', 'sdod_cfg_combine', 'sdod_stage_unet_inputs', 'sdod_randn_f32',
    'sdod_dpm_update', 'sdod_ddim_step_f32', 'sdod_lincomb4_f32', 'sdod_image_to_u8', 'sdod_hip_last_error',
    'sdod_hip_device_info', 'sdod_image_conv_in_unit_f16', 'sdod_dense_conv3x3_f16', 'sdod_dense_conv3x3_ok',
    'sdod_add_control_f16',
    'sdod_gemm_region_f16', 'sdod_xattn_fold_regions_f16', 'sdod_region_weights_f32', 'sdod_region_blend_f16',
    'sdod_xattn_fold_ip_f16', 'sdod_ip_weights_f32', 'sdod_patch_embed_u8_f16', 'sdod_vit_tokens_f16',
    'sdod_attention_head_dim_ok', 'sdod_xattn_fold_ok',
    'sdod_k_step_windows',
    'sdod_freeu_f16',
]


def check(code):
    if code != 0:
        msg = hip().sdod_hip_last_error()
        raise SdodError(code, msg.decode() if msg else 'unknown error')
```

stable-diffusion-on-device_amd/sdod/amd/engine.py:

```python
import contextlib
import ctypes

import numpy as np
import torch

from . import _lib
from ._lib import check

UNET, VAE_DECODER, TEXT_ENCODER, TEMB, VAE_ENCODER, VAE_ENCODER_MASKED, ADAPTER, UPSCALER, CONTROLNET, CONTROL_HINT = 0, 1, 2, 3, 4, 5, 6, 7, 8, 9
IMAGE_ENCODER, IMAGE_PROJ = 10, 11


class ModelConfig(ctypes.Structure):
    _fields_ = [(n, ctypes.c_int) for n in (
        'latent_channels', 'latent_h', 'latent_w', 'model_channels', 'context_dim', 'context_len', 'num_heads',
        'head_dim', 'vocab_size', 'text_layers', 'text_heads', 'vae_channels', 'linear_proj', 'text_arch', 'weight_quant',
        'concat_channels')]
    adapter_reps = 0
    adapter_hint_channels = 0
    adapter_res_blocks = 0
    tiling = 0
    control_inputs = 0
    control_temb = 0
    regions = 0
    ip_tokens = 0
    freeu = 0
    _ADAPTER_FIELDS = ('adapter_reps', 'adapter_hint_channels', 'adapter_res_blocks', 'tiling', 'control_inputs', 'control_temb', 'regions',
                       'ip_tokens', 'freeu')

    @classmethod
    def from_buffer_copy(cls, source, offset=0):
        out = type(ctypes.Structure).from_buffer_copy(cls, source, offset)
        for n in cls._ADAPTER_FIELDS:
            v = int(getattr(source, n, 0))
            if v:
                setattr(out, n, v)
        return out


class AdapterConfig(ctypes.Structure):
    _fields_ = [(n, ctypes.c_int) for n in ('adapter_reps', 'adapter_hint_channels', 'adapter_res_blocks')]


class ControlConfig(ctypes.Structure):
    _fields_ = [(n, ctypes.c_int) for n in ('control_inputs', 'control_temb')]


class RegionConfig(ctypes.Structure):
    _fields_ = [('regions', ctypes.c_int)]


class IpConfig(ctypes.Structure):
    _fields_ = [('ip_tokens', ctypes.c_int)]


class VisionConfig(ctypes.Structure):
    _fields_ = [(n, ctypes.c_int) for n in ('image_size', 'patch', 'width', 'layers', 'heads', 'mlp_dim', 'proj_dim', 'quick_gelu')]


def vit_h14_config():
    return VisionConfig(224, 14, 1280, 32, 16, 5120, 1024, 0)


class UpscalerConfig(ctypes.Structure):
    _fields_ = [(n, ctypes.c_int) for n in ('num_blocks', 'in_h', 'in_w')]


TILING_WRAP = {False: 0, True: 3, 'xy': 3, 'x': 1, 'y': 2}


def tiling_wrap(tiling):
    if isinstance(tiling, (bool, str)) and tiling in TILING_WRAP:
        return TILING_WRAP[tiling]
    raise ValueError(f"tiling must be False, True, 'xy', 'x' or 'y', not {tiling!r}")


def copy_config(cfg):
    return ModelConfig.from_buffer_copy(cfg)


class LoraEntry(ctypes.Structure):
    _fields_ = [('name', ctypes.c_char_p), ('up', ctypes.c_void_p), ('down', ctypes.c_void_p), ('dtype', ctypes.c_int),
                ('rank', ctypes.c_int), ('scale', ctypes.c_float)]


ENGINE_SYMBOLS = [
    'sdod_model_config_sd14', 'sdod_model_config_sd21', 'sdod_graph_create', 'sdod_graph_create_ex', 'sdod_graph_create_wrap', 'sdod_graph_destroy', 'sdod_graph_num_params', 'sdod_graph_param_info',
    'sdod_graph_set_param', 'sdod_graph_param_device', 'sdod_graph_load_file', 'sdod_graph_finalize', 'sdod_graph_io', 'sdod_graph_execute', 'sdod_graph_check',
    'sdod_graph_stats', 'sdod_graph_tune_info', 'sdod_graph_num_ops', 'sdod_graph_op_info', 'sdod_graph_op_detail', 'sdod_graph_profile',
    'sdod_graph_keep_base', 'sdod_graph_base_bytes', 'sdod_graph_set_loras', 'sdod_graph_create_upscaler',
    'sdod_graph_create_control', 'sdod_graph_bind_output', 'sdod_graph_create_regions',
    'sdod_graph_create_ip', 'sdod_graph_create_vision',
    'sdod_graph_enable_freeu', 'sdod_graph_freeu_input',
]


def _engine():
    lib = _lib.hip()
    if not getattr(lib, '_sdod_engine_typed', False):
        P, I = ctypes.c_void_p, ctypes.c_int
        lib.sdod_model_config_sd14.argtypes = [ctypes.POINTER(ModelConfig)]
        lib.sdod_model_config_sd14.restype = None
        lib.sdod_model_config_sd21.argtypes = [ctypes.POINTER(ModelConfig)]
        lib.sdod_model_config_sd21.restype = None
        lib.sdod_graph_create.argtypes = [ctypes.POINTER(P), I, ctypes.POINTER(ModelConfig), I]
        lib.sdod_graph_create_ex.argtypes = [ctypes.POINTER(P), I, ctypes.POINTER(ModelConfig), ctypes.POINTER(AdapterConfig), I]
        lib.sdod_graph_create_wrap.argtypes = [ctypes.POINTER(P), I, ctypes.POINTER(ModelConfig), ctypes.POINTER(AdapterConfig), I, I]
        lib.sdod_graph_create_upscaler.argtypes = [ctypes.POINTER(P), ctypes.POINTER(UpscalerConfig), I]
        lib.sdod_graph_create_control.argtypes = [ctypes.POINTER(P), I, ctypes.POINTER(ModelConfig), ctypes.POINTER(ControlConfig), I]
        lib.sdod_graph_create_regions.argtypes = [ctypes.POINTER(P), I, ctypes.POINTER(ModelConfig), ctypes.POINTER(RegionConfig), I]
        lib.sdod_graph_create_ip.argtypes = [ctypes.POINTER(P), I, ctypes.POINTER(ModelConfig), ctypes.POINTER(IpConfig), I]
        lib.sdod_graph_create_vision.argtypes = [ctypes.POINTER(P), I, ctypes.POINTER(ModelConfig), ctypes.POINTER(VisionConfig), ctypes.POINTER(IpConfig), I]
        lib.sdod_graph_bind_output.argtypes = [P, I, P, ctypes.c_size_t]
        lib.sdod_graph_destroy.argtypes = [P]
        lib.sdod_graph_num_params.argtypes = [P]
        lib.sdod_graph_param_info.argtypes = [P, I, ctypes.POINTER(ctypes.c_char_p), ctypes.POINTER(I), ctypes.POINTER(ctypes.c_int64)]
        lib.sdod_graph_set_param.argtypes = [P, ctypes.c_char_p, P, I, ctypes.POINTER(ctypes.c_int64), I]
        lib.sdod_graph_load_file.argtypes = [P, ctypes.c_char_p, ctypes.c_char_p]
        lib.sdod_graph_param_device.argtypes = [P, ctypes.c_char_p, ctypes.POINTER(P), ctypes.POINTER(ctypes.c_size_t)]
        lib.sdod_graph_finalize.argtypes = [P]
        lib.sdod_graph_io.argtypes = [P, I, I, ctypes.POINTER(P), ctypes.POINTER(ctypes.c_size_t)]
        lib.sdod_graph_execute.argtypes = [P, P, I]
        lib.sdod_graph_check.argtypes = [P]
        lib.sdod_graph_stats.argtypes = [P, ctypes.POINTER(ctypes.c_size_t), ctypes.POINTER(ctypes.c_size_t), ctypes.POINTER(I),
                                         ctypes.POINTER(ctypes.c_double)]
        lib.sdod_graph_tune_info.argtypes = [P, ctypes.POINTER(I), ctypes.POINTER(I), ctypes.c_char_p, I]
        lib.sdod_graph_num_ops.argtypes = [P]
        lib.sdod_graph_op_info.argtypes = [P, I, ctypes.POINTER(ctypes.c_char_p), ctypes.POINTER(ctypes.c_double), ctypes.POINTER(ctypes.c_double)]
        lib.sdod_graph_profile.argtypes = [P, P, I, P, I]
        lib.sdod_graph_op_detail.argtypes = [P, I, ctypes.POINTER(ctypes.c_char_p)]
        lib.sdod_graph_keep_base.argtypes = [P]
        lib.sdod_graph_base_bytes.argtypes = [P, ctypes.POINTER(ctypes.c_size_t)]
        lib.sdod_graph_set_loras.argtypes = [P, ctypes.POINTER(LoraEntry), I, P]
        lib.sdod_graph_enable_freeu.argtypes = [P]
        lib.sdod_graph_freeu_input.argtypes = [P, ctypes.POINTER(I)]
        lib._sdod_engine_typed = True
    return lib


def sd14_config(latent_h=64, latent_w=64, concat_channels=0, adapter_reps=0, adapter_hint_channels=0, adapter_res_blocks=0):
    cfg = ModelConfig()
    _engine().sdod_model_config_sd14(ctypes.byref(cfg))
    cfg.latent_h, cfg.latent_w, cfg.concat_channels = latent_h, latent_w, concat_channels
    cfg.adapter_reps, cfg.adapter_hint_channels, cfg.adapter_res_blocks = int(adapter_reps), int(adapter_hint_channels), int(adapter_res_blocks)
    return cfg


def sd21_config(latent_h=96, latent_w=96, concat_channels=0):
    cfg = ModelConfig()
    _engine().sdod_model_config_sd21(ctypes.byref(cfg))
    cfg.latent_h, cfg.latent_w, cfg.concat_channels = latent_h, latent_w, concat_channels
    return cfg


class _DevView:

    def __init__(self, ptr, shape, typestr):
        self.__cuda_array_interface__ = {'shape': tuple(shape), 'typestr': typestr, 'data': (int(ptr), False), 'version': 2}


def device_view(ptr, shape, dtype, device):
    typestr = {torch.float16: '<f2', torch.float32: '<f4', torch.int32: '<i4', torch.uint8: '|u1'}[dtype]
    return torch.as_tensor(_DevView(ptr, shape, typestr), device=device)


class Graph:

    def __init__(self, kind, cfg, batch, device='cuda:0', wrap=None):
        self._lib = _engine()
        self._h = ctypes.c_void_p()
        self.kind, self.cfg, self.batch = kind, cfg, batch
        self.device = torch.device(device)
        acfg = AdapterConfig(*(int(getattr(cfg, n, 0)) for n, _ in AdapterConfig._fields_))
        ccfg = ControlConfig(int(getattr(cfg, 'control_inputs', 0)) if kind == UNET else 0, int(getattr(cfg, 'control_temb', 0)) if kind == TEMB else 0)
        control = kind in (CONTROLNET, CONTROL_HINT) or ccfg.control_inputs or ccfg.control_temb
        if control and (wrap or any(getattr(acfg, n) for n, _ in AdapterConfig._fields_)):
            raise ValueError('a ControlNet graph, or a UNet with control inputs, takes neither tiling nor a T2I-Adapter configuration')
        regions = int(getattr(cfg, 'regions', 0)) if kind == UNET else 0
        if regions and (control or wrap or any(getattr(acfg, n) for n, _ in AdapterConfig._fields_)):
            raise ValueError('a UNet with regions takes no control inputs, no tiling and no T2I-Adapter configuration')
        ip_tokens = int(getattr(cfg, 'ip_tokens', 0)) if kind == UNET else 0
        if ip_tokens and (regions or control or wrap or any(getattr(acfg, n) for n, _ in AdapterConfig._fields_)):
            raise ValueError('a UNet with an image prompt takes no regions, no control inputs, no tiling and no T2I-Adapter configuration')
        with self._on_device():
            if kind in (IMAGE_ENCODER, IMAGE_PROJ):
                icfg = IpConfig(int(getattr(cfg, 'ip_tokens', 0)))
                check(self._lib.sdod_graph_create_vision(ctypes.byref(self._h), kind, ctypes.byref(cfg), ctypes.byref(cfg.vision), ctypes.byref(icfg), batch))
            elif ip_tokens:
                icfg = IpConfig(ip_tokens)
                check(self._lib.sdod_graph_create_ip(ctypes.byref(self._h), kind, ctypes.byref(cfg), ctypes.byref(icfg), batch))
            elif regions:
                rcfg = RegionConfig(regions)
                check(self._lib.sdod_graph_create_regions(ctypes.byref(self._h), kind, ctypes.byref(cfg), ctypes.byref(rcfg), batch))
            elif control:
                check(self._lib.sdod_graph_create_control(ctypes.byref(self._h), kind, ctypes.byref(cfg), ctypes.byref(ccfg), batch))
            elif kind == UPSCALER:
                check(self._lib.sdod_graph_create_upscaler(ctypes.byref(self._h), ctypes.byref(cfg), batch))
            elif wrap is not None:
                check(self._lib.sdod_graph_create_wrap(ctypes.byref(self._h), kind, ctypes.byref(cfg), ctypes.byref(acfg), int(wrap), batch))
            elif kind == ADAPTER or any(getattr(acfg, n) for n, _ in AdapterConfig._fields_):
                check(self._lib.sdod_graph_create_ex(ctypes.byref(self._h), kind, ctypes.byref(cfg), ctypes.byref(acfg), batch))
            else:
                check(self._lib.sdod_graph_create(ctypes.byref(self._h), kind, ctypes.byref(cfg), batch))
            if kind == UNET and int(getattr(cfg, 'freeu', 0)):
                self.enable_freeu()
        self.finalized = False

    def _on_device(self):
        return torch.cuda.device(self.device) if torch.cuda.is_available() else contextlib.nullcontext()

    def __del__(self):
        h = getattr(self, '_h', None)
        if h:
            self._lib.sdod_graph_destroy(h)
            self._h = None

    def param_table(self):
        out = []
        n = self._lib.sdod_graph_num_params(self._h)
        name = ctypes.c_char_p(); nd = ctypes.c_int(); shape = (ctypes.c_int64 * 4)()
        for i in range(n):
            check(self._lib.sdod_graph_param_info(self._h, i, ctypes.byref(name), ctypes.byref(nd), shape))
            out.append((name.value.decode(), tuple(shape[:nd.value])))
        return out

    def set_param(self, name, tensor):
        if hasattr(tensor, 'payload'):
            buf = tensor.payload()
            shape = (ctypes.c_int64 * max(len(tensor.shape), 1))(*tensor.shape)
            check(self._lib.sdod_graph_set_param(self._h, name.encode(), ctypes.cast(ctypes.c_char_p(buf), ctypes.c_void_p), 2, shape,
                                                 len(tensor.shape)))
            return
        t = tensor.detach().cpu().contiguous()
        if t.dtype not in (torch.float32, torch.float16):
            t = t.float()
        shape = (ctypes.c_int64 * max(t.dim(), 1))(*t.shape)
        check(self._lib.sdod_graph_set_param(self._h, name.encode(), ctypes.c_void_p(t.data_ptr()),
                                             1 if t.dtype == torch.float32 else 0, shape, t.dim()))

    def packed_param(self, name, dtype=torch.float16):
        p = ctypes.c_void_p(); n = ctypes.c_size_t()
        check(self._lib.sdod_graph_param_device(self._h, name.encode(), ctypes.byref(p), ctypes.byref(n)))
        return device_view(p.value, (n.value // torch.empty((), dtype=dtype).element_size(),), dtype, self.device)

    def load_state_dict(self, sd, prefix=''):
        with torch.cuda.device(self.device):
            for name, _ in self.param_table():
                key = prefix + name
                if key not in sd:
                    raise KeyError(f'missing parameter {key}')
                self.set_param(name, sd[key])

    def load_file(self, path, prefix=''):
        with self._on_device():
            check(self._lib.sdod_graph_load_file(self._h, path.encode(), prefix.encode()))

    def finalize(self):
        with torch.cuda.device(self.device):
            check(self._lib.sdod_graph_finalize(self._h))
        self.finalized = True
        return self

    def keep_base(self):
        check(self._lib.sdod_graph_keep_base(self._h))
        return self

    def enable_freeu(self):
        check(self._lib.sdod_graph_enable_freeu(self._h))
# ... 342 lines not shown
```

stable-diffusion-on-device_amd/sdod/amd/ops.py:

```python
import ctypes

import torch

from . import _lib
from ._lib import GemmDesc, check

ACT = {None: 0, 'none': 0, 'silu': 1, 'gelu': 2, 'quick_gelu': 3, 'relu': 4}


def _stream():
    return ctypes.c_void_p(torch.cuda.current_stream().cuda_stream)


def _p(t):
    return None if t is None else ctypes.c_void_p(t.data_ptr())


def _req(t, dtype=None, name='tensor'):
    if not t.is_cuda:
        raise ValueError(f'{name} must live on the GPU')
    if not t.is_contiguous():
        raise ValueError(f'{name} must be contiguous')
    if dtype is not None and t.dtype != dtype:
        raise ValueError(f'{name} must be {dtype}, got {t.dtype}')
# ... 253 lines not shown
    _req(up, torch.float16, 'up'); _req(down, torch.float16, 'down')
    if up.dim() != 2 or w.stride(-1) != 1:
        raise ValueError('up must be [n, rank] and the columns of w contiguous')
    n, rank = up.shape
    k = down.numel() // rank if rank else (down.shape[-1] if down.dim() > 1 else 0)
    if ld is None:
        ld = w.stride(0) if w.dim() == 2 and w.shape[0] > 1 else k
    check(lib.sdod_lora_merge_f16(_p(w), n, k, int(ld), _p(up), _p(down), rank, float(scale), int(conv_cin or 0), 1 if geglu else 0,
                                  _stream()))
    return w


def layer_norm(x, weight, bias, eps=1e-5, out=None):
    lib = _lib.hip()
    _req(x, torch.float16, 'x')
    c = x.shape[-1]; m = x.numel() // c
    if out is None:
        out = torch.empty_like(x)
    check(lib.sdod_layer_norm_f16(_p(x), _p(out), _p(weight), _p(bias), m, c, eps, _stream()))
    return out


def attention(q, k, v, heads, scale=None, causal=False, out=None):
    lib = _lib.hip()
    for t, nme in ((q, 'q'), (k, 'k'), (v, 'v')):
        _req(t, torch.float16, nme)
    b, lq, c = q.shape
    lk = k.shape[1]
    d = c // heads
    if scale is None:
        scale = d ** -0.5
    if out is None:
        out = torch.empty_like(q)
    check(lib.sdod_attention_f16(_p(q), _p(k), _p(v), _p(out), b, heads, lq, lk, d, q.shape[2], k.shape[2], v.shape[2],
                                 out.shape[2], scale, 1 if causal else 0, _stream()))
    return out


def xattn_fold(kv, k_off, v_off, n_img, L, wq, sq, tq, wo, heads, scale=None, regions=None):
    lib = _lib.hip()
    _req(kv, torch.float16, 'kv'); _req(wq, torch.float16, 'wq'); _req(wo, torch.float16, 'wo')
    _req(sq, torch.float32, 'sq'); _req(tq, torch.float32, 'tq')
    c = wq.shape[0]; d = c // heads
    if scale is None:
        scale = d ** -0.5
    nk = heads * 80 * (1 if regions is None else int(regions))
    w1 = torch.empty(n_img, nk, c, dtype=torch.float16, device=kv.device)
    w2 = torch.empty(n_img, c, nk, dtype=torch.float16, device=kv.device)
    s1 = torch.empty(n_img, nk, dtype=torch.float32, device=kv.device); t1 = torch.empty_like(s1)
    if regions is not None:
        check(lib.sdod_xattn_fold_regions_f16(_p(kv), kv.shape[-1], k_off, v_off, n_img, int(regions), L, _p(wq), wq.shape[1], _p(sq), _p(tq),
                                              _p(wo), wo.shape[1], heads, d, scale, _p(w1), _p(s1), _p(t1), _p(w2), _stream()))
        return w1, s1, t1, w2
    check(lib.sdod_xattn_fold_f16(_p(kv), kv.shape[-1], k_off, v_off, n_img, L, _p(wq), wq.shape[1], _p(sq), _p(tq), _p(wo), wo.shape[1],
                                  heads, d, scale, _p(w1), _p(s1), _p(t1), _p(w2), _stream()))
    return w1, s1, t1, w2


def xattn_fold_ip(kv, k_off, v_off, kv_ip, k_off_ip, v_off_ip, n_img, L, T, wq, sq, tq, wo, heads, scale=None):
    lib = _lib.hip()
    _req(kv, torch.float16, 'kv'); _req(kv_ip, torch.float16, 'kv_ip'); _req(wq, torch.float16, 'wq'); _req(wo, torch.float16, 'wo')
    _req(sq, torch.float32, 'sq'); _req(tq, torch.float32, 'tq')
    c = wq.shape[0]; d = c // heads
    if kv.shape[0] < n_img * L or kv_ip.shape[0] < n_img * T:
        raise ValueError(f'kv needs {n_img * L} rows and kv_ip {n_img * T}, got {kv.shape[0]} and {kv_ip.shape[0]}')
    if scale is None:
        scale = d ** -0.5
    nk = heads * 80 * 2
    w1 = torch.empty(n_img, nk, c, dtype=torch.float16, device=kv.device)
    w2 = torch.empty(n_img, c, nk, dtype=torch.float16, device=kv.device)
    s1 = torch.empty(n_img, nk, dtype=torch.float32, device=kv.device); t1 = torch.empty_like(s1)
    check(lib.sdod_xattn_fold_ip_f16(_p(kv), kv.shape[-1], k_off, v_off, _p(kv_ip), kv_ip.shape[-1], k_off_ip, v_off_ip, n_img, L, T,
                                     _p(wq), wq.shape[1], _p(sq), _p(tq), _p(wo), wo.shape[1], heads, d, scale, _p(w1), _p(s1), _p(t1), _p(w2),
                                     _stream()))
    return w1, s1, t1, w2


def attention_strided(q, k, v, out, batch, heads, lq, lk, d, ldq, ldk, ldv, ldo, scale, causal=False):
    lib = _lib.hip()
    check(lib.sdod_attention_f16(q, k, v, out, batch, heads, lq, lk, d, ldq, ldk, ldv, ldo, scale, 1 if causal else 0,
                                 _stream()))


def softmax_rows(x, out=None):
    if out is not None:
        _req_out(out, x, x.numel())
    _req(x, torch.float16, 'x')
    lib = _lib.hip()
    n = x.shape[-1]; m = x.numel() // n
    if out is None:
        out = torch.empty_like(x)
    check(lib.sdod_softmax_rows_f16(_p(x), _p(out), m, n, _stream()))
    return out


def geglu(x, out=None):
    if out is not None:
        _req_out(out, x, x.numel() // 2)
    _req(x, torch.float16, 'x')
    lib = _lib.hip()
    c = x.shape[-1] // 2; m = x.numel() // (2 * c)
    if out is None:
        out = torch.empty(x.shape[:-1] + (c,), dtype=torch.float16, device=x.device)
    check(lib.sdod_geglu_f16(_p(x), _p(out), m, c, _stream()))
    return out


def activation(x, act, out=None):
    if out is not None:
        _req_out(out, x, x.numel())
    _req(x, torch.float16, 'x')
    lib = _lib.hip()
    if out is None:
        out = torch.empty_like(x)
    check(lib.sdod_act_f16(_p(x), _p(out), x.numel(), ACT[act], _stream()))
    return out


def add(a, b, out=None):
    _req_out(b, a, a.numel(), 'b')
    if out is not None:
        _req_out(out, a, a.numel())
    _req(a, torch.float16, 'a')
    lib = _lib.hip()
    if out is None:
        out = torch.empty_like(a)
    check(lib.sdod_add_f16(_p(a), _p(b), _p(out), a.numel(), _stream()))
    return out


def pixel_unshuffle_u8(img_u8, factor=8, out=None):
    lib = _lib.hip()
    _req(img_u8, torch.uint8, 'img')
    n, ih, iw, ch = img_u8.shape
    h, w = ih // factor, iw // factor
    assert ih == h * factor and iw == w * factor, img_u8.shape
    if out is None:
        out = torch.empty((n, h, w, ch * factor * factor), dtype=torch.float16, device=img_u8.device)
    else:
        _req(out, torch.float16, 'out')
        assert out.numel() == img_u8.numel(), (out.shape, img_u8.shape)
    check(lib.sdod_pixel_unshuffle_u8_f16(_p(img_u8), _p(out), n, h, w, ch, factor, _stream()))
    return out


def avg_pool2(x, out=None):
    lib = _lib.hip()
    _req(x, torch.float16, 'x')
    n, h, w, c = x.shape
    if out is None:
        out = torch.empty((n, h // 2, w // 2, c), dtype=torch.float16, device=x.device)
    else:
        _req(out, torch.float16, 'out')
        assert out.numel() * 4 == x.numel(), (out.shape, x.shape)
    check(lib.sdod_avg_pool2_f16(_p(x), _p(out), n, h, w, c, _stream()))
    return out


def adapter_stage(src, dst, weight=1.0):
    lib = _lib.hip()
    _req(src, torch.float16, 'src'); _req(dst, torch.float16, 'dst')
    assert dst.numel() == src.numel(), (dst.shape, src.shape)
    check(lib.sdod_adapter_stage_f16(_p(src), _p(dst), src.numel(), float(weight), _stream()))
    return dst


# ... 612 lines not shown
```

stable-diffusion-on-device_amd/sdod/amd/pipeline.py:

```python
import os

import numpy as np
import torch

from . import engine as E
from . import ops
from . import prompts as PR
from . import regions as RG
from . import ip_adapter as IP
from . import freeu as FU
from . import upscale as UP
from . import panorama as PN
from .host import DpmSolver
from .samplers import K_SAMPLERS, K_SCHEDULES, PLMS_ORDERS, KSchedule, PlmsSchedule


class Txt2Img:
    inpaint_unet = False
    _cond_staged = False
    encoder = None
    masked_encoder = None
    _traj = None
    prompt_chunks = 1
    model = 'sd14'
# ... 17 lines not shown
    regions = 0
    canvas_hw = None
    canvas_wrap = False
    canvas_vae = None
    freeu = False
    _pano = None

    def __init__(self, state_dicts=None, models_dir=None, images_per_gpu=1, latent_hw=64, device='cuda:0', use_hip_graph=True,
                 tokenizer=None, with_text_encoder=True, model='sd14', with_vae=True, cfg_split=False, weight_quant=None,
                 with_vae_encoder=False, inpaint_unet=False, prompt_chunks=1, *, loras=False, hires_hw=None, adapter=False,
                 adapter_channels=3, tiling=False, upscaler=False, controlnet=False, regions=False, ip_adapter=False, canvas_hw=None,
                 canvas_wrap=False, freeu=False):
        self.freeu = FU.freeu_check_build(freeu)
        self.prompt_chunks = check_prompt_chunks(prompt_chunks)
        latent_h, latent_w = check_latent_hw(latent_hw)
        self.canvas_hw = PN.panorama_check_build(canvas_hw, canvas_wrap, (latent_h, latent_w), cfg_split, inpaint_unet, hires_hw, adapter,
                                                 controlnet, regions, ip_adapter, tiling, upscaler)
        self.canvas_wrap = bool(canvas_wrap)
        adapter_check_build(adapter, adapter_channels, cfg_split, hires_hw, inpaint_unet, model)
        control_check_build(controlnet, cfg_split, hires_hw, inpaint_unet, adapter, tiling, model)
        self.tiling = tiling_check_build(tiling, with_vae_encoder, inpaint_unet, hires_hw, adapter)
        quant_asked = bool(regions) and (weight_quant or (weight_quant is None and state_dicts is not None and any(
            hasattr(v, 'payload') and len(v.shape) >= 2 for v in state_dicts.get('unet', {}).values())))
        self.regions = RG.regions_check_build(regions, self.prompt_chunks, cfg_split, hires_hw, controlnet, adapter, tiling, inpaint_unet,
                                              model, quant_asked)
        quant_ip = bool(ip_adapter) and (weight_quant or (weight_quant is None and state_dicts is not None and any(
            hasattr(v, 'payload') and len(v.shape) >= 2 for v in state_dicts.get('unet', {}).values())))
        if IP.ip_check_build(ip_adapter, regions, self.prompt_chunks, cfg_split, hires_hw, controlnet, adapter, tiling, inpaint_unet, model, quant_ip):
            self.ip_tokens, self.ip_proj_dim, ip_vision = IP.ip_sources(state_dicts, models_dir)
        up_args = upscaler_check_build(upscaler, tiling, hires_hw if hires_hw is not None else latent_hw, state_dicts, models_dir)
        if hires_hw is not None:
            check_latent_hw(hires_hw, 'hires_hw')
            if cfg_split or inpaint_unet:
                raise ValueError('hires_hw cannot be combined with cfg_split or inpaint_unet')
        self.device = torch.device(device)
        torch.cuda.set_device(self.device)
        self.n = images_per_gpu
        self.model = model
        self.v_prediction = model == 'sd21'
        self.cfg = E.sd21_config(latent_h, latent_w) if model == 'sd21' else E.sd14_config(latent_h, latent_w)
        self.inpaint_unet = bool(inpaint_unet)
        if self.inpaint_unet:
            self.cfg.concat_channels = 5
        self._cond_staged = False
        if weight_quant is None:
            weight_quant = state_dicts is not None and any(hasattr(v, 'payload') and len(v.shape) >= 2 for v in state_dicts['unet'].values())
        self.cfg.weight_quant = 2 if weight_quant in ('auto', 2) else 1 if weight_quant else 0
        self.cfg_split = bool(cfg_split)
        self._pair = None
        if self.cfg_split:
            import torch.distributed as dist
            if not (dist.is_available() and dist.is_initialized() and dist.get_world_size() % 2 == 0):
                raise RuntimeError('cfg_split needs torch.distributed initialised with an even world size')
            rank = dist.get_rank()
            self._half = rank % 2
            for a in range(0, dist.get_world_size(), 2):
                grp = dist.new_group([a, a + 1])
                if a == rank - self._half:
                    self._pair = grp
            self._pair_staged = dist.get_backend() == 'gloo'
        self.use_hip_graph = use_hip_graph
        self.tokenizer = tokenizer
        unet_cfg = self.cfg
        if self.prompt_chunks > 1:
            unet_cfg = E.copy_config(self.cfg)
            unet_cfg.context_len = PR.CHUNK_LEN * self.prompt_chunks
        if adapter:
            unet_cfg = E.copy_config(unet_cfg)
            unet_cfg.adapter_reps = 2
            self.adapter_channels = int(adapter_channels)
        if controlnet:
            unet_cfg = E.copy_config(unet_cfg)
            unet_cfg.control_inputs = 1
        if self.regions:
            unet_cfg = E.copy_config(unet_cfg)
            unet_cfg.context_len = PR.CHUNK_LEN * self.regions
            unet_cfg.regions = self.regions
        if self.ip_tokens:
            unet_cfg = E.copy_config(unet_cfg)
            unet_cfg.ip_tokens = self.ip_tokens
        if self.freeu:
            unet_cfg = E.copy_config(unet_cfg)
            unet_cfg.freeu = 1
        vae_cfg = self.cfg
        if self.tiling:
            unet_cfg, vae_cfg = E.copy_config(unet_cfg), E.copy_config(self.cfg)
            unet_cfg.tiling = vae_cfg.tiling = self.tiling
        self.unet = E.UNet(unet_cfg, self.n if cfg_split else 2 * self.n, device)
        self.vae = E.VaeDecoder(vae_cfg, 1, device) if with_vae else None
        self.text = E.TextEncoder(self.cfg, 2 * (self.regions or self.prompt_chunks), device) if with_text_encoder else None
        self.encoder = E.VaeEncoder(self.cfg, 1, device) if with_vae_encoder else None
        self.masked_encoder = E.MaskedVaeEncoder(self.cfg, 1, device) if self.inpaint_unet else None
        if adapter:
            acfg = E.copy_config(self.cfg)
            acfg.adapter_hint_channels = self.adapter_channels
            self.adapter = E.Adapter(acfg, 1, device)
        if self.canvas_hw is not None:
            ccfg = E.sd21_config(*self.canvas_hw) if model == 'sd21' else E.sd14_config(*self.canvas_hw)
            if self.canvas_wrap:
                ccfg.tiling = 1
            self.canvas_vae = E.VaeDecoder(ccfg, 1, device) if with_vae else None
        self._temb_graphs = {}
        self._sd = state_dicts
        self._dir = models_dir
        for g, key, stem in ((self.unet, 'unet', 'unet'), (self.vae, 'vae', 'vae_decoder'), (self.text, 'text', 'text_encoder'),
                             (self.encoder, 'vae_enc', 'vae_encoder'), (self.masked_encoder, 'vae_enc', 'vae_encoder'),
                             (self.adapter, 'adapter', 'adapter'), (self.canvas_vae, 'vae', 'vae_decoder')):
            if g is None:
                continue
            self._load(g, key, stem)
            if loras and (g is self.unet or g is self.text):
                g.keep_base()
            g.finalize()
        if controlnet:
            ccfg = E.copy_config(unet_cfg)
            ccfg.control_inputs, ccfg.weight_quant = 0, 0
            self.controlnet = E.ControlNet(ccfg, 2 * self.n, device)
            self.control_hint = E.ControlHint(ccfg, 1, device)
            for g in (self.controlnet, self.control_hint):
                self._load(g, 'controlnet', 'controlnet')
            for k, slot in enumerate(self.unet.control_res):
                self.controlnet.bind_output(k, slot)
            self.controlnet.finalize()
            self.control_hint.finalize()
            self._temb_stage = torch.zeros((self.unet.batch, self.unet.temb_width + self.controlnet.temb_width), dtype=torch.float16,
                                           device=self.device)
        if self.ip_tokens:
            self.image_proj = E.ImageProj(self.cfg, self.ip_proj_dim, self.ip_tokens, 2 * self.n, device)
            self._load(self.image_proj, 'ip_adapter', 'ip_adapter')
            self.image_proj.bind_output(0, self.unet.ip_ctx)
            self.image_proj.finalize()
            if ip_vision is not None:
                self.image_encoder = E.ImageEncoder(E.VisionConfig(*ip_vision), self.n, device)
                self._load(self.image_encoder, 'image_encoder', 'image_encoder')
                self.image_encoder.finalize()
                self.ip_image_size = int(ip_vision[0])
        if up_args is not None:
            self.upscaler = UP.Upscaler(device=device, use_hip_graph=use_hip_graph, **up_args)
        self._loras = bool(loras)
        self._temb_cache = {}
        self._ctx_fresh = True
        if hires_hw is not None:
            self.hires = Txt2Img(state_dicts=state_dicts, models_dir=models_dir, images_per_gpu=images_per_gpu, latent_hw=hires_hw,
                                 device=device, use_hip_graph=use_hip_graph, tokenizer=None, with_text_encoder=False, model=model,
                                 with_vae=with_vae, cfg_split=False, weight_quant=weight_quant, with_vae_encoder=False, inpaint_unet=False,
                                 prompt_chunks=prompt_chunks, loras=loras, freeu=freeu)

    def _load(self, g, key, stem):
        ip_unet = g is self.unet and self.ip_tokens
        if self._sd is not None:
            g.load_state_dict({**self._sd[key], **self._sd['ip_adapter']} if ip_unet else self._sd[key])
        else:
            g.load_file(f'{self._dir}/{stem}.sdodw')
            if ip_unet:
                g.load_file(f'{self._dir}/ip_adapter.sdodw')

    def set_loras(self, adapters, strict=True):
        from . import lora as L
        if not self._loras:
            raise RuntimeError('this pipeline was built without loras=True: merge on the host (lora.merged_state_dict) and build a new one')
        parsed = []
        for a in adapters:
            if not isinstance(a, (tuple, list)) or len(a) not in (2, 3):
                raise ValueError('an adapter is (path_or_dict, strength) or (path_or_dict, strength_unet, strength_text)')
            strengths = [a[1], a[1] if len(a) == 2 else a[2]]
            for v in strengths:
# ... 1032 lines not shown
```

Measured before the change: 10.67 images/s.

## Compute first self-attention once for identical guidance halves and mirror output

In the first transformer block (input_blocks.1.1), the cond and uncond halves of the batch are identical up to that point: same latent, same timestep, no text context yet. A new pair_shared UNet mode runs the QKV GEMM and self-attention only on the first half. The attention kernel then writes each output tile a second time at a mirror row offset, so the second half is filled without being computed. The GEMM tile plan is still chosen at the full row count, and a check verifies it carries over to the half-size launch. The mode is turned on by default for plain SD1.x txt2img, guarded against configurations where the halves could differ, and adds an extra output write plus new API surface.

```diff
diff --git a/include/sdod_engine.h b/include/sdod_engine.h
--- a/include/sdod_engine.h
+++ b/include/sdod_engine.h
@@ -66,6 +66,11 @@
     int ip_tokens;
 } sdod_ip_config;
 SDOD_API int sdod_graph_create_ip(void** graph, int kind, const sdod_model_config* cfg, const sdod_ip_config* ip, int batch);
+typedef struct sdod_pair_config {
+    int pair_shared;
+} sdod_pair_config;
+SDOD_API int sdod_graph_create_pair(void** graph, int kind, const sdod_model_config* cfg, const sdod_pair_config* pair,
+                                    const sdod_adapter_config* adapter, const sdod_region_config* regions, int batch);
 typedef struct sdod_vision_config {
     int image_size;
     int patch;
diff --git a/include/sdod_hip.h b/include/sdod_hip.h
--- a/include/sdod_hip.h
+++ b/include/sdod_hip.h
@@ -125,6 +125,9 @@
 SDOD_API int sdod_attention_f16(const void* q, const void* k, const void* v, void* out, int batch, int heads,
                                 int lq, int lk, int d, int ldq, int ldk, int ldv, int ldo, float scale, int causal,
                                 void* stream);
+SDOD_API int sdod_attention_mirror_f16(const void* q, const void* k, const void* v, void* out, int batch, int heads,
+                                       int lq, int lk, int d, int ldq, int ldk, int ldv, int ldo, float scale, int causal,
+                                       long long mirror_rows, int variant_batch, void* stream);
 SDOD_API int sdod_attention_head_dim_ok(int d);
 
 SDOD_API int sdod_xattn_fold_f16(const void* kv, int ld_kv, int k_off, int v_off, int n_img, int L, const void* wq, int ldq,
diff --git a/stable-diffusion-on-device_amd/csrc/attention.hip b/stable-diffusion-on-device_amd/csrc/attention.hip
--- a/stable-diffusion-on-device_amd/csrc/attention.hip
+++ b/stable-diffusion-on-device_amd/csrc/attention.hip
@@ -18,6 +18,7 @@
     int ldq, ldk, ldv, ldo;
     float scale_log2;
     int causal;
+    int mirror_rows;
 };
 
 typedef short short4v __attribute__((__vector_size__(4 * sizeof(short))));
@@ -420,6 +421,7 @@
 #pragma unroll
                     for (int r = 0; r < 4; ++r) hv[r] = (f16)(o[a][dt][r] * inv);
                     *reinterpret_cast<f16x4*>(op + dv0) = hv;
+                    if (p.mirror_rows > 0) *reinterpret_cast<f16x4*>(op + (size_t)p.mirror_rows * p.ldo + dv0) = hv;
                 }
             }
         }
@@ -570,12 +572,14 @@
     return rows_per_image > 0 && rows_per_image % 32 == 0 && NK % 320 == 0 && C % 64 == 0 ? 1 : 0;
 }
 
-extern "C" int sdod_attention_f16(const void* q, const void* k, const void* v, void* out, int batch, int heads, int lq,
-                                  int lk, int d, int ldq, int ldk, int ldv, int ldo, float scale, int causal,
-                                  void* stream) {
+namespace {
+int attention_launch(const void* q, const void* k, const void* v, void* out, int batch, int heads, int lq, int lk, int d, int ldq, int ldk,
+                     int ldv, int ldo, float scale, int causal, long long mirror_rows, int variant_batch, void* stream) {
     SDOD_TRY
     SDOD_REQUIRE(q && k && v && out, "null pointer");
     SDOD_REQUIRE(batch > 0 && heads > 0 && lq > 0 && lk > 0, "bad shape");
+    SDOD_REQUIRE(variant_batch >= batch, "variant_batch must be at least batch");
+    SDOD_REQUIRE(mirror_rows == 0 || (mirror_rows >= (long long)batch * lq && mirror_rows <= INT_MAX), "mirror_rows must be 0 or in [batch * lq, 2^31)");
     SDOD_REQUIRE(sdod_attention_head_dim_ok(d), "head dim must be one of 40, 64, 80, 160");
     SDOD_REQUIRE(ldq % 8 == 0 && ldk % 8 == 0 && ldv % 8 == 0 && ldo % 4 == 0, "row strides must keep 16-byte alignment");
     SDOD_REQUIRE(ldq >= heads * d && ldk >= heads * d && ldv >= heads * d && ldo >= heads * d, "row stride < heads*d");
@@ -587,6 +591,7 @@
     p.ldq = ldq; p.ldk = ldk; p.ldv = ldv; p.ldo = ldo;
     p.scale_log2 = scale * 1.4426950408889634f;
     p.causal = causal;
+    p.mirror_rows = (int)mirror_rows;
     const bool no_tr = std::getenv("SDOD_ATTN_NO_TR") != nullptr;
     const bool tr = !no_tr;
     bool big = lq >= 2048 && d != 160;
@@ -598,7 +603,7 @@
     case 64: e = attn_dispatch<64>(p, big, tr, st); break;
     case 80: {
         static const bool kvs_off = [] { const char* e2 = std::getenv("SDOD_ATTN_KVS"); return e2 && e2[0] == '0'; }();
-        const long long wgs = (long long)((lq + 63) / 64) * heads * batch;
+        const long long wgs = (long long)((lq + 63) / 64) * heads * variant_batch;
         if (!big && tr && !kvs_off && !causal && wgs <= 512 && lk >= 256) e = attn_launch<80, 1, true, 2>(p, st);
         else e = attn_dispatch<80>(p, big, tr, st);
         break;
@@ -608,6 +613,19 @@
     SDOD_HIP_CHECK(e);
     return 0;
     SDOD_CATCH
+}
+}
+
+extern "C" int sdod_attention_f16(const void* q, const void* k, const void* v, void* out, int batch, int heads, int lq,
+                                  int lk, int d, int ldq, int ldk, int ldv, int ldo, float scale, int causal,
+                                  void* stream) {
+    return attention_launch(q, k, v, out, batch, heads, lq, lk, d, ldq, ldk, ldv, ldo, scale, causal, 0, batch, stream);
+}
+
+extern "C" int sdod_attention_mirror_f16(const void* q, const void* k, const void* v, void* out, int batch, int heads, int lq,
+                                         int lk, int d, int ldq, int ldk, int ldv, int ldo, float scale, int causal,
+                                         long long mirror_rows, int variant_batch, void* stream) {
+    return attention_launch(q, k, v, out, batch, heads, lq, lk, d, ldq, ldk, ldv, ldo, scale, causal, mirror_rows, variant_batch, stream);
 }
 
 namespace {
diff --git a/stable-diffusion-on-device_amd/csrc/engine.h b/stable-diffusion-on-device_amd/csrc/engine.h
--- a/stable-diffusion-on-device_amd/csrc/engine.h
+++ b/stable-diffusion-on-device_amd/csrc/engine.h
@@ -66,7 +66,7 @@
 public:
     Graph(int kind, const sdod_model_config& cfg, int batch, const sdod_adapter_config& acfg = sdod_adapter_config{0, 0, 0}, int wrap = 0,
           const sdod_upscaler_config& ucfg = sdod_upscaler_config{0, 0, 0}, const sdod_control_config* ccfg = nullptr, int regions = 0,
-          int ip_tokens = 0, const sdod_vision_config* vcfg = nullptr);
+          int ip_tokens = 0, const sdod_vision_config* vcfg = nullptr, int pair_shared = 0);
     ~Graph();
     Graph(const Graph&) = delete;
 
@@ -99,6 +99,7 @@
     int ip_tokens_ = 0;
     const float* ip_w_[4] = {};
     f16* ip_kv_all_ = nullptr;
+    bool pair_shared_ = false;
     bool freeu_ = false;
     int freeu_input_ = -1;
     void freeu_site(const Act& h, const Act& skip, const float* params, int stage);
@@ -213,6 +214,7 @@
         int regions = 0;
         int pad_mode = 0;
         int split_k = 0;
+        int plan_rows = 0;
     };
     struct LnVecs { float* s; float* t; };
     LnVecs ln_fold_vectors(f16* w, int N, int K, int ldw, int ln_w, int ln_b, const float* bias);
@@ -233,7 +235,7 @@
     char* base_copy_ = nullptr;
     bool static_stale_ = false;
     std::vector<void*> derived_;
-    void emit_gemm(sdod_gemm_desc d, const float* region_w = nullptr, int regions = 0);
+    void emit_gemm(sdod_gemm_desc d, const float* region_w = nullptr, int regions = 0, int plan_M = 0);
     void linear(const f16* x, int rows, int K, int w, int N, f16* out, const GemmOpt& o);
     void linear_raw(const f16* x, int rows, int K, const f16* w, int ldw, int N, f16* out, const GemmOpt& o);
     Act conv(const Act& x, const Act* x2, int w, int cout, int ksize, int stride, bool upsample, const GemmOpt& o);
@@ -241,7 +243,7 @@
     Act layer_norm(const Act& x, int lw, int lb, float eps);
     void dense_conv(sdod_dense_conv_desc d, int w, int bias);
     void attention(const f16* q, const f16* k, const f16* v, f16* out, int B, int heads, int lq, int lk, int d, int ldq,
-                   int ldk, int ldv, int ldo, bool causal);
+                   int ldk, int ldv, int ldo, bool causal, int mirror_rows = 0, int variant_B = 0);
 
     Act res_block(const std::string& pfx, const Act& x, const Act* x2, int cout, const f16* emb_all, int emb_ld, int& emb_off);
     std::vector<Op>& sink() { return to_static_ ? static_ops_ : ops_; }
diff --git a/stable-diffusion-on-device_amd/csrc/engine.hip b/stable-diffusion-on-device_amd/csrc/engine.hip
--- a/stable-diffusion-on-device_amd/csrc/engine.hip
+++ b/stable-diffusion-on-device_amd/csrc/engine.hip
@@ -36,8 +36,16 @@
 }
 
 Graph::Graph(int kind, const sdod_model_config& cfg, int batch, const sdod_adapter_config& acfg, int wrap, const sdod_upscaler_config& ucfg,
-             const sdod_control_config* ccfg, int regions, int ip_tokens, const sdod_vision_config* vcfg)
-    : kind_(kind), cfg_(cfg), acfg_(acfg), ucfg_(ucfg), regions_(regions), ip_tokens_(ip_tokens), batch_(batch), wrap_(wrap) {
+             const sdod_control_config* ccfg, int regions, int ip_tokens, const sdod_vision_config* vcfg, int pair_shared)
+    : kind_(kind), cfg_(cfg), acfg_(acfg), ucfg_(ucfg), regions_(regions), ip_tokens_(ip_tokens), pair_shared_(pair_shared != 0), batch_(batch),
+      wrap_(wrap) {
+    SDOD_REQUIRE(pair_shared == 0 || pair_shared == 1, "pair_shared must be 0 or 1");
+    if (pair_shared_) {
+        SDOD_REQUIRE(kind == SDOD_GRAPH_UNET, "pair_shared applies to the UNET graph only");
+        SDOD_REQUIRE(batch % 2 == 0, "pair_shared needs an even batch (the two guidance halves)");
+        SDOD_REQUIRE(cfg.weight_quant == 0 && cfg.concat_channels == 0 && wrap == 0 && ip_tokens == 0 && (!ccfg || ccfg->control_inputs == 0),
+                     "pair_shared excludes weight_quant, concat_channels, wrap, image prompts and control inputs");
+    }
     SDOD_REQUIRE(ip_tokens == 0 || ((kind == SDOD_GRAPH_UNET || kind == SDOD_GRAPH_IMAGE_PROJ) && ip_tokens >= 1 && ip_tokens <= 16 && regions == 0),
                  "ip_tokens: the UNET and IMAGE_PROJ graphs only, 1 .. 16, not with regions");
     const bool vision_kind = kind == SDOD_GRAPH_IMAGE_ENCODER || kind == SDOD_GRAPH_IMAGE_PROJ;
@@ -87,6 +95,9 @@
     SDOD_REQUIRE(cfg.model_channels > 0 && cfg.model_channels % 64 == 0, "model_channels must be a multiple of 64");
     SDOD_REQUIRE(cfg.context_dim % 64 == 0, "context_dim must be a multiple of 64");
     if (kind == SDOD_GRAPH_UNET || kind == SDOD_GRAPH_CONTROLNET) check_head_geometry();
+    if (pair_shared_)
+        SDOD_REQUIRE(cfg.model_channels == 320 && head_geometry(320).d == 40,
+                     "pair_shared needs model_channels 320 and 40-wide heads at the first level (the SD 1.x geometry)");
     SDOD_REQUIRE(cfg.context_len >= 1 && cfg.context_len <= 4096, "context_len must be in [1, 4096]");
     SDOD_REQUIRE(cfg.concat_channels >= 0, "concat_channels must not be negative");
     SDOD_REQUIRE(acfg.adapter_reps >= 0 && acfg.adapter_reps <= 2, "adapter_reps must be 0, 1 or 2");
@@ -685,9 +696,14 @@
     sink().push_back(Op{[d2](hipStream_t st) { check_rc(sdod_gemm_f16(&d2, st)); }, "splitk_reduce", 0.0, pending_.bytes, pending_.detail});
 }
 
-void Graph::emit_gemm(sdod_gemm_desc d, const float* region_w, int regions) {
+void Graph::emit_gemm(sdod_gemm_desc d, const float* region_w, int regions, int plan_M) {
     settle();
     if (mode_ == DECLARE) return;
+    const int run_M = d.M;
+    if (plan_M > run_M) {
+        if (d.a_mode != SDOD_A_ROWS) throw Error(INTERNAL_ERROR, "a GEMM planned at another row count must be a rows GEMM");
+        d.M = plan_M;
+    }
     const bool tune = autotune_enabled() && (d.N > 16 || (d.a_mode == SDOD_A_CONV3X3 && d.ksize != 1 && d.N % 4 == 0));
     if (tune) {
         for (int t : kCandidates) {
@@ -768,6 +784,16 @@
         d.tile = pick % 1000;
         d.split_k = pick / 1000;
     }
+    if (d.M != run_M) {
+        int t_full = 0, s_full = 1, t_run = 0, s_run = 1;
+        (void)sdod_gemm_plan(&d, &t_full, &s_full);
+        d.M = run_M;
+        d.tile = t_full;
+        (void)sdod_gemm_plan(&d, &t_run, &s_run);
+        if (t_run != t_full || s_run != s_full || !pick_runs(d, t_full + 1000 * d.split_k))
+            throw Error(INTERNAL_ERROR, "the full-batch GEMM plan (tile " + std::to_string(t_full) + " x" + std::to_string(s_full) +
+                                            ") does not carry over to the half-batch launch");
+    }
     const double fl = 2.0 * d.M * d.N * d.K;
     flops_ += fl;
     d.workspace = ws_;
@@ -863,7 +889,7 @@
         d.ln_s = o.ln_s_raw;
     }
     d.w_img_stride = o.w_img_stride; d.vec_img_stride = o.vec_img_stride; d.softmax_cols = o.softmax_cols;
-    emit_gemm(d, o.region_w, o.regions);
+    emit_gemm(d, o.region_w, o.regions, o.plan_rows);
 }
 
 Graph::LnVecs Graph::ln_fold_vectors(f16* w, int N, int K, int ldw, int ln_w, int ln_b, const float* bias) {
@@ -976,12 +1002,14 @@
 }
 
 void Graph::attention(const f16* q, const f16* k, const f16* v, f16* out, int B, int heads, int lq, int lk, int d, int ldq,
-                      int ldk, int ldv, int ldo, bool causal) {
+                      int ldk, int ldv, int ldo, bool causal, int mirror_rows, int variant_B) {
     const float scale = 1.0f / sqrtf((float)d);
     const int ca = causal ? 1 : 0;
-    emit([=](hipStream_t st) { check_rc(sdod_attention_f16(q, k, v, out, B, heads, lq, lk, d, ldq, ldk, ldv, ldo, scale, ca, st)); },
-         "attn_d" + std::to_string(d), 4.0 * B * heads * (double)lq * lk * d, 2.0 * B * heads * d * (2.0 * lq + 2.0 * lk),
-         "B" + std::to_string(B) + " h" + std::to_string(heads) + " lq" + std::to_string(lq) + " lk" + std::to_string(lk));
+    const int vb = variant_B > 0 ? variant_B : B;
+    emit([=](hipStream_t st) { check_rc(sdod_attention_mirror_f16(q, k, v, out, B, heads, lq, lk, d, ldq, ldk, ldv, ldo, scale, ca, mirror_rows, vb, st)); },
+         "attn_d" + std::to_string(d), 4.0 * B * heads * (double)lq * lk * d, 2.0 * B * heads * d * ((mirror_rows > 0 ? 3.0 : 2.0) * lq + 2.0 * lk),
+         "B" + std::to_string(B) + " h" + std::to_string(heads) + " lq" + std::to_string(lq) + " lk" + std::to_string(lk) +
+             (mirror_rows > 0 ? " mirror" : ""));
 }
 
 void Graph::build() {
@@ -1078,6 +1106,7 @@
 void Graph::enable_freeu() {
     SDOD_REQUIRE(kind_ == SDOD_GRAPH_UNET, "FreeU applies to the UNET graph only");
     SDOD_REQUIRE(!finalized_, "enable_freeu() must be called before finalize()");
+    SDOD_REQUIRE(!pair_shared_, "FreeU is not among the configurations a pair_shared graph is proven bit-equal for: create the graph without the flag");
     SDOD_REQUIRE(cfg_.latent_h <= 2048 && cfg_.latent_w <= 2048, "FreeU needs latent_h and latent_w <= 2048 (sdod_freeu_f16 takes sides up to 1024)");
     freeu_ = true;
 }
@@ -1384,6 +1413,25 @@
     SDOD_CATCH
 }
 
+extern "C" int sdod_graph_create_pair(void** graph, int kind, const sdod_model_config* cfg, const sdod_pair_config* pair,
+                                      const sdod_adapter_config* adapter, const sdod_region_config* regions, int batch) {
+    SDOD_TRY
+    SDOD_REQUIRE(graph && cfg, "null argument");
+    *graph = nullptr;
+    SDOD_REQUIRE(kind != SDOD_GRAPH_UPSCALER && kind != SDOD_GRAPH_ADAPTER && kind != SDOD_GRAPH_CONTROLNET && kind != SDOD_GRAPH_CONTROL_HINT,
+                 "this graph kind has a create function of its own");
+    const int R = regions ? regions->regions : 0;
+    if (R != 0) {
+        SDOD_REQUIRE(kind == SDOD_GRAPH_UNET, "regional prompts: kind SDOD_GRAPH_UNET");
+        SDOD_REQUIRE(R >= 2 && R <= 4, "regions must be in [2, 4]");
+        SDOD_REQUIRE(cfg->context_len == 77 * R, "regional prompts: context_len must be 77 * regions");
+    }
+    *graph = new Graph(kind, *cfg, batch, adapter ? *adapter : sdod_adapter_config{0, 0, 0}, 0, sdod_upscaler_config{0, 0, 0}, nullptr, R, 0, nullptr,
+                       pair ? pair->pair_shared : 0);
+    return 0;
+    SDOD_CATCH
+}
+
 extern "C" int sdod_graph_create_ip(void** graph, int kind, const sdod_model_config* cfg, const sdod_ip_config* ip, int batch) {
     SDOD_TRY
     SDOD_REQUIRE(graph && cfg, "null argument");
diff --git a/stable-diffusion-on-device_amd/csrc/graphs.hip b/stable-diffusion-on-device_amd/csrc/graphs.hip
--- a/stable-diffusion-on-device_amd/csrc/graphs.hip
+++ b/stable-diffusion-on-device_amd/csrc/graphs.hip
@@ -160,12 +160,15 @@
             release(nrm);
         }
     };
+    const bool pair = pair_shared_ && fold && pfx == "input_blocks.1.1";
+    const int srows = pair ? rows / 2 : rows, sB = pair ? B / 2 : B;
     f16* qkv = alloc((size_t)rows * 3 * C);
     { GemmOpt o; o.wq_scale = qscale_of(group_first(gq)); o.wq_off = qoff_of(group_first(gq));
+      o.plan_rows = pair ? rows : 0;
       behind_ln(t0, l1w, l1b, o, [&](const f16* a, const GemmOpt& og) {
-          linear_raw(a, rows, C, reinterpret_cast<const f16*>(group_base(gq)), C, 3 * C, qkv, og); }); }
+          linear_raw(a, srows, C, reinterpret_cast<const f16*>(group_base(gq)), C, 3 * C, qkv, og); }); }
     f16* a1 = alloc((size_t)rows * C);
-    attention(qkv, qkv + C, qkv + 2 * C, a1, B, heads, L, L, d, 3 * C, 3 * C, 3 * C, C, false);
+    attention(qkv, qkv + C, qkv + 2 * C, a1, sB, heads, L, L, d, 3 * C, 3 * C, 3 * C, C, false, pair ? srows : 0, pair ? B : 0);
     release(qkv);
     Act t1 = act(B, 1, L, C);
     { GemmOpt o; o.bias = o1b; o.residual = t0.p; linear(a1, rows, C, o1w, C, t1.p, o); }
diff --git a/stable-diffusion-on-device_amd/sdod/amd/_lib.py b/stable-diffusion-on-device_amd/sdod/amd/_lib.py
--- a/stable-diffusion-on-device_amd/sdod/amd/_lib.py
+++ b/stable-diffusion-on-device_amd/sdod/amd/_lib.py
@@ -143,6 +143,8 @@
         'sdod_compose_linear_f16': (c_int, [P, c_int, P, c_int, P, c_int, c_int, c_int, c_int, P, P, P, P]),
         'sdod_lora_merge_f16': (c_int, [P, c_int, c_int, c_int, P, P, c_int, c_float, c_int, c_int, P]),
         'sdod_attention_f16': (c_int, [P, P, P, P, c_int, c_int, c_int, c_int, c_int, c_int, c_int, c_int, c_int, c_float, c_int, P]),
+        'sdod_attention_mirror_f16': (c_int, [P, P, P, P, c_int, c_int, c_int, c_int, c_int, c_int, c_int, c_int, c_int, c_float, c_int,
+                                              ctypes.c_longlong, c_int, P]),
         'sdod_attention_head_dim_ok': (c_int, [c_int]),
         'sdod_xattn_fold_ok': (c_int, [c_int, c_int, c_int, c_int]),
         'sdod_xattn_fold_f16': (c_int, [P, c_int, c_int, c_int, c_int, c_int, P, c_int, P, P, P, c_int, c_int, c_int, c_float, P, P, P, P, P]),
@@ -222,6 +224,7 @@
     'sdod_attention_head_dim_ok', 'sdod_xattn_fold_ok',
     'sdod_k_step_windows',
     'sdod_freeu_f16',
+    'sdod_attention_mirror_f16',
 ]
 
 
diff --git a/stable-diffusion-on-device_amd/sdod/amd/engine.py b/stable-diffusion-on-device_amd/sdod/amd/engine.py
--- a/stable-diffusion-on-device_amd/sdod/amd/engine.py
+++ b/stable-diffusion-on-device_amd/sdod/amd/engine.py
@@ -25,8 +25,9 @@
     regions = 0
     ip_tokens = 0
     freeu = 0
+    pair_shared = 0
     _ADAPTER_FIELDS = ('adapter_reps', 'adapter_hint_channels', 'adapter_res_blocks', 'tiling', 'control_inputs', 'control_temb', 'regions',
-                       'ip_tokens', 'freeu')
+                       'ip_tokens', 'freeu', 'pair_shared')
 
     @classmethod
     def from_buffer_copy(cls, source, offset=0):
@@ -50,6 +51,10 @@
     _fields_ = [('regions', ctypes.c_int)]
 
 
+class PairConfig(ctypes.Structure):
+    _fields_ = [('pair_shared', ctypes.c_int)]
+
+
 class IpConfig(ctypes.Structure):
     _fields_ = [('ip_tokens', ctypes.c_int)]
 
@@ -92,6 +97,7 @@
     'sdod_graph_create_control', 'sdod_graph_bind_output', 'sdod_graph_create_regions',
     'sdod_graph_create_ip', 'sdod_graph_create_vision',
     'sdod_graph_enable_freeu', 'sdod_graph_freeu_input',
+    'sdod_graph_create_pair',
 ]
 
 
@@ -109,6 +115,8 @@
         lib.sdod_graph_create_upscaler.argtypes = [ctypes.POINTER(P), ctypes.POINTER(UpscalerConfig), I]
         lib.sdod_graph_create_control.argtypes = [ctypes.POINTER(P), I, ctypes.POINTER(ModelConfig), ctypes.POINTER(ControlConfig), I]
         lib.sdod_graph_create_regions.argtypes = [ctypes.POINTER(P), I, ctypes.POINTER(ModelConfig), ctypes.POINTER(RegionConfig), I]
+        lib.sdod_graph_create_pair.argtypes = [ctypes.POINTER(P), I, ctypes.POINTER(ModelConfig), ctypes.POINTER(PairConfig), ctypes.POINTER(AdapterConfig),
+                                               ctypes.POINTER(RegionConfig), I]
         lib.sdod_graph_create_ip.argtypes = [ctypes.POINTER(P), I, ctypes.POINTER(ModelConfig), ctypes.POINTER(IpConfig), I]
         lib.sdod_graph_create_vision.argtypes = [ctypes.POINTER(P), I, ctypes.POINTER(ModelConfig), ctypes.POINTER(VisionConfig), ctypes.POINTER(IpConfig), I]
         lib.sdod_graph_bind_output.argtypes = [P, I, P, ctypes.c_size_t]
@@ -182,8 +190,14 @@
         ip_tokens = int(getattr(cfg, 'ip_tokens', 0)) if kind == UNET else 0
         if ip_tokens and (regions or control or wrap or any(getattr(acfg, n) for n, _ in AdapterConfig._fields_)):
             raise ValueError('a UNet with an image prompt takes no regions, no control inputs, no tiling and no T2I-Adapter configuration')
+        pair = int(getattr(cfg, 'pair_shared', 0))
+        if pair and (kind != UNET or control or wrap or ip_tokens or int(getattr(cfg, 'freeu', 0))):
+            raise ValueError('pair_shared: a UNet only, with no control inputs, no tiling, no image prompt and no FreeU')
         with self._on_device():
-            if kind in (IMAGE_ENCODER, IMAGE_PROJ):
+            if pair:
+                check(self._lib.sdod_graph_create_pair(ctypes.byref(self._h), kind, ctypes.byref(cfg), ctypes.byref(PairConfig(pair)), ctypes.byref(acfg),
+                                                       ctypes.byref(RegionConfig(regions)) if regions else None, batch))
+            elif kind in (IMAGE_ENCODER, IMAGE_PROJ):
                 icfg = IpConfig(int(getattr(cfg, 'ip_tokens', 0)))
                 check(self._lib.sdod_graph_create_vision(ctypes.byref(self._h), kind, ctypes.byref(cfg), ctypes.byref(cfg.vision), ctypes.byref(icfg), batch))
             elif ip_tokens:
diff --git a/stable-diffusion-on-device_amd/sdod/amd/ops.py b/stable-diffusion-on-device_amd/sdod/amd/ops.py
--- a/stable-diffusion-on-device_amd/sdod/amd/ops.py
+++ b/stable-diffusion-on-device_amd/sdod/amd/ops.py
@@ -359,6 +359,12 @@
                                  _stream()))
 
 
+def attention_mirror(q, k, v, out, batch, heads, lq, lk, d, ldq, ldk, ldv, ldo, scale, mirror_rows, variant_batch=None, causal=False):
+    lib = _lib.hip()
+    check(lib.sdod_attention_mirror_f16(q, k, v, out, batch, heads, lq, lk, d, ldq, ldk, ldv, ldo, scale, 1 if causal else 0, int(mirror_rows),
+                                        int(batch if variant_batch is None else variant_batch), _stream()))
+
+
 def softmax_rows(x, out=None):
     if out is not None:
         _req_out(out, x, x.numel())
diff --git a/stable-diffusion-on-device_amd/sdod/amd/pipeline.py b/stable-diffusion-on-device_amd/sdod/amd/pipeline.py
--- a/stable-diffusion-on-device_amd/sdod/amd/pipeline.py
+++ b/stable-diffusion-on-device_amd/sdod/amd/pipeline.py
@@ -123,6 +123,11 @@
         if self.freeu:
             unet_cfg = E.copy_config(unet_cfg)
             unet_cfg.freeu = 1
+        self.pair_shared = not (cfg_split or self.inpaint_unet or controlnet or self.regions or self.ip_tokens or self.freeu or self.tiling
+                                or self.cfg.weight_quant or model == 'sd21' or self.canvas_hw is not None)
+        if self.pair_shared:
+            unet_cfg = E.copy_config(unet_cfg)
+            unet_cfg.pair_shared = 1
         vae_cfg = self.cfg
         if self.tiling:
             unet_cfg, vae_cfg = E.copy_config(unet_cfg), E.copy_config(self.cfg)
```

Measured after the change: 10.73 images/s, median of 6. No clear change (+0.5%).
